# Boese0601/Dyadic-Interaction-Modeling

Hardware: AMD Instinct MI355X
Metric: listener clips/sec (T=300, EMOCA-56) (higher is better)
Workload: dtype bf16; 1 GPU; C3: B=256/GPU synthetic dyad clips, T=300, SLMFT.forward(mode='val'): listener VQ encode + encoder + 299-step AR decode (top-k 52 sampling) + VQ decode; global_batch=256, seq_len=300, gather=tokens+coeffs, gather_bytes_per_rank=17452032

## Files before the change

dyadic-interaction-modeling_amd/csrc/common.hpp:

```cpp
#pragma once
#include <hip/hip_runtime.h>
#include <stdint.h>
#include <stdio.h>
#include <string.h>
#include <string>

#include "../../include/dimx.h"

namespace dimx {

void set_error(const char* fmt, ...);
const char* get_error();

#define DIMX_HIP(expr)                                                                       \
    do {                                                                                     \
        hipError_t _e = (expr);                                                              \
        if (_e != hipSuccess) {                                                              \
            dimx::set_error("%s:%d: %s -> %s", __FILE__, __LINE__, #expr, hipGetErrorString(_e)); \
            return DIMX_ERR_HIP;                                                             \
        }                                                                                    \
    } while (0)

#define DIMX_REQUIRE(cond, code, ...)       \
    do {                                    \
// ... 352 lines not shown
    int force_nsplit;
};
int launch_decode_attn_self_kv8(const Kv8SelfArgs& a, hipStream_t s);

int launch_vq_argmin(const float* z, int N, const float* Et , const float* ee ,
                     int32_t* idx, float* best_d, float* margin, hipStream_t s);

struct ChainGemmDesc {
    const void* W;
    int N, K, ldw;
    int cols, rows_pad, ncb, nkt;
};
struct ChainArgs {
    int B;
    ChainGemmDesc g1;
    const void* A1;
    int lda1;
    float* xr;
    float* x;
    int C;
    const float* slabs;
    int nslab;
    long slab_stride;
    void* y;
    const float* gamma;
    ChainGemmDesc g2;
    float* out2;
    int ld_out2;
    unsigned* counters;
    unsigned* seen;
    const int32_t* step;
    unsigned* err;
    int defer;
    float* stats;
    const float* colsum2;
    int nbar;
    int fault;
    int offA1, offW1, offRed1, offA2, offW2, offRed2;
};
struct SampleHeadArgs {
    int on;
    const float* logits;
    int ld_logits, nslab;
    long slab_stride;
    int top_k;
    const float* noise;
    int row0, rows_total;
    int32_t* tokens;
    int tok_ld;
    float* logits_out;
    int logits_out_ld;
    const float* emb_table;
    const float* qkv0;
    int qkv0_N;
    int32_t* hist;
    int hist_ld;
    int32_t* params;
};
struct LayerChainArgs {
    int B, C;
    DecodeAttnArgs sa, ca;
    ChainGemmDesc g_so, g_cq, g_co;
    const void* o;
    int ld_o;
    float* x;
    void* y;
    float* stats;
    const float* colsum_cq;
    float* qc;
    int ld_qc;
    unsigned* counters;
    unsigned* seen;
    const int32_t* step;
    int epoch_add;
    unsigned* err;
    int fault;
    unsigned long long* prof;
    SampleHeadArgs head;
    int sc_stride;
    int off_base, off_A1, off_W1, off_A2, off_W2, off_W3, off_A3;
};
bool layer_chain_supported(const LayerChainArgs& a, int cu_count);
int launch_layer_chain(const LayerChainArgs& a, hipStream_t s);
size_t chain_plan(ChainArgs& a);
bool chain_supported(const ChainArgs& a, int cu_count);
int launch_chain(const ChainArgs& a, hipStream_t s);

int launch_cast_pad(int out_dtype, const float* x, int ldx, const float* coladd, void* y, int ldy, int M, int K,
                    hipStream_t s, const uint8_t* zero_rows = nullptr);
int launch_gather_rows(int out_dtype, const float* table, int ld_table, int rows, const int32_t* idx, void* y,
                       int ldy, int M, int C, hipStream_t s);
constexpr int kLstmSave = 6;
size_t lstm_scratch_bytes(int B, int T, int In);
int lstm_layer_run(const float* x, int B, int T, int In, int H, const float* const* w_ih, const float* const* w_hh,
                   const float* const* b_ih, const float* const* b_hh, float* y, void* scratch, size_t scratch_bytes, int flags,
                   int cu_count, int* fault_count, hipStream_t st, float* save = nullptr);
size_t lstm_bwd_scratch_bytes(int B, int T);
int lstm_bwd_run(const float* dy, const float* save, const float* const* w_hh, int B, int T, float* dgates, void* scratch,
                 size_t scratch_bytes, int flags, int cu_count, int* fault_count, hipStream_t st);
int launch_context_concat(int out_dtype, const float* x_s, const float* patch, const float* audio, void* ctx,
                          int M, int dim, int dim_a, hipStream_t s);
int launch_finalize_idx(int32_t* idx, const int32_t* lens, int B, int T, int32_t pad_value, hipStream_t s,
                        int fqn = 1);
int launch_shift_tokens(const int32_t* z, int32_t* inp, int32_t* tgt, int B, int T, hipStream_t s);
int launch_ce_argmax(const float* logits, const int32_t* target, float* row_loss, int32_t* argmax_tok, int R,
                     int V, hipStream_t s);
struct SampleFilter {
    int kind = 0;
    float a = 0.f, b = 0.f;
    uint8_t* keep_out = nullptr;
};
struct SampleArgs {
    const float* logits = nullptr;
    int ld_logits = 0, R = 0, top_k = 0;
    float temperature = 0.f;
    const float* noise = nullptr;
    uint64_t seed = 0;
    const int32_t* step_dev = nullptr;
    uint64_t step_host = 0;
    int32_t* tokens = nullptr;
    int tok_ld = 0, tok_col_from_step = 0, nslab = 0;
    long slab_stride = 0;
    float* logits_out = nullptr;
    int logits_out_ld = 0, row0 = 0, rows_total = 0;
    const float* emb_table = nullptr;
    int emb_C = 0;
    float* x_next = nullptr;
    int32_t* step_rw = nullptr;
    unsigned* done_ctr = nullptr;
    const float* pos_table = nullptr;
    float pos_scale = 0.f;
    int pos_rows = 0;
    const int32_t* dev_params = nullptr;
    void* y_next = nullptr;
    const float* y_gamma = nullptr;
    int y_dtype = DIMX_F32;
    const float* qkv0_table = nullptr;
    float* qkv0_out = nullptr;
    int qkv0_N = 0;
    const int32_t* prompt = nullptr;
    int prompt_ld = 0, prompt_max = 0;
    const int32_t* prompt_len = nullptr;
    int prompt_div = 1;
    int32_t* epoch_rw = nullptr;
    SampleFilter filt;
    int32_t* hist = nullptr;
    int hist_ld = 0;
};
int launch_sample(const SampleArgs& a, hipStream_t s);
struct GuidedArgs {
    const float* logits_u = nullptr;
    float scale = 1.f;
    float* branch_out = nullptr;
    int32_t* tokens_u = nullptr;
};
int launch_sample_guided(const SampleArgs& a, const GuidedArgs& g, hipStream_t s);
struct BeamSelectArgs {
    const float* logits = nullptr;
    int nslab = 1;
    long slab_stride = 0;
    int nclip = 0, W = 0;
    const int32_t* step_dev = nullptr;
    int step_host = 0;
    int32_t* step_rw = nullptr;
    unsigned* done_ctr = nullptr;
    int32_t* epoch_rw = nullptr;
// ... 62 lines not shown
```

dyadic-interaction-modeling_amd/csrc/gemm.hip:

```cpp
#include "common.hpp"

namespace dimx {

static bool gemm_use_ws72(const GemmArgs& a);

void gemm_args_init(GemmArgs& a) {
    memset(&a, 0, sizeof(a));
    a.in_dtype = DIMX_F32;
    a.out_dtype = DIMX_F32;
    a.rowadd_scale = 1.f;
    a.nseg = 1;
    a.rowT = 1;
    a.splitk = 1;
    a.rowadd_div = 1;
}

void gemm_set_plain_out(GemmArgs& a, void* C, int ldc) {
    a.nseg = 1;
    a.seg_width = a.N;
    a.seg[0].ptr = C;
    a.seg[0].sb = (long)ldc * a.rowT;
    a.seg[0].st = ldc;
    a.seg[0].sh = 0;
    a.seg[0].sd = 1;
// ... 790 lines not shown
            if (it + STAGES - 1 < nk) issue(it + STAGES - 1, (it + STAGES - 1) % STAGES);
            if (a.ln_stats && it == nk - 2) {
                float s1 = 0.f;
#pragma unroll
                for (int i = 0; i < 8; ++i) s1 += lp[i].x;
                s1 += xor_lane_f32<16>(s1);
                s1 += xor_lane_f32<32>(s1);
                const float inv_c = 1.0f / (float)a.ln_C;
                const float mean = s1 * inv_c;
                const float ncs = (float)a.ln_C * (1.0f / 32.0f), inv_n = 32.0f * inv_c;
                float s2 = 0.f;
#pragma unroll
                for (int i = 0; i < 8; ++i) {
                    const float d = lp[i].x * inv_n - mean;
                    s2 += lp[i].y + ncs * d * d;
                }
                s2 += xor_lane_f32<16>(s2);
                s2 += xor_lane_f32<32>(s2);
                const float var = s2 * inv_c;
                const float rstd = rsqrtf(var + 1e-5f);
                if (a.ln_err && lane < 16 && m0 + lw * 16 + lane < a.M && mean * mean > 64.0f * var)
                    atomicOr(a.ln_err, 4u);
                if (lane < 16) {
                    ln_sm[lw * 16 + lane] = mean;
                    ln_sm[64 + lw * 16 + lane] = rstd;
                }
                asm volatile("s_waitcnt lgkmcnt(0)" ::: "memory");
            }
        }
        return;
    }

    const int wm = wave >> 1, wn = wave & 1;
    const int half = lane >> 5, l31 = lane & 31;
    const unsigned lds0 = (unsigned)(size_t)(lds_void_t*)smem;
    unsigned aoff[4], woff[4];
#pragma unroll
    for (int ks = 0; ks < 4; ++ks) {
        aoff[ks] = lds0 + lds_off(wm * 32 + l31, 2 * ks + half);
        woff[ks] = lds0 + BM * 128 + lds_off(wn * 32 + l31, 2 * ks + half);
    }
    f32x16_t acc[1][1];
#pragma unroll
    for (int r = 0; r < 16; ++r) acc[0][0][r] = 0.f;
    float ln_cs = 0.f;
    for (int it = 0; it < nk; ++it) {
        const unsigned boff = (unsigned)((it % STAGES) * TILE_BYTES);
        __builtin_amdgcn_s_barrier();
        if (it == 0 && a.ln_stats) {
            const int n = n0 + wn * 32 + l31;
            ln_cs = a.ln_colsum[n < a.N ? n : a.N - 1];
        }
        u32x4_t fa[4][1], fw[4][1];
#pragma unroll
        for (int q = 0; q < 4; ++q) {
            ds_read128<0>(fa[q][0], aoff[q] + boff);
            ds_read128<0>(fw[q][0], woff[q] + boff);
        }
#pragma unroll
        for (int q = 0; q < 4; ++q) {
            if (q == 0) wait_lgkm<6>();
            if (q == 1) wait_lgkm<4>();
            if (q == 2) wait_lgkm<2>();
            if (q == 3) wait_lgkm<0>();
            __builtin_amdgcn_sched_barrier(0);
            FragMma<T, 1, 1>::run(acc, fa[q], fw[q]);
        }
    }
    if (a.ln_stats) {
        const float* strip = ln_sm + wm * 32;
#pragma unroll
        for (int q = 0; q < 4; ++q) {
            const float4 mq = *(const float4*)(strip + 8 * q + 4 * half);
            const float4 rq = *(const float4*)(strip + 64 + 8 * q + 4 * half);
            acc[0][0][4 * q + 0] = rq.x * (acc[0][0][4 * q + 0] - mq.x * ln_cs);
            acc[0][0][4 * q + 1] = rq.y * (acc[0][0][4 * q + 1] - mq.y * ln_cs);
            acc[0][0][4 * q + 2] = rq.z * (acc[0][0][4 * q + 2] - mq.z * ln_cs);
            acc[0][0][4 * q + 3] = rq.w * (acc[0][0][4 * q + 3] - mq.w * ln_cs);
        }
    }
    epilogue<T, OutT, 1, 1>(a, acc, m0 + wm * 32, n0 + wn * 32, half, l31, split);
}

template <typename OutT>
struct Ws72 {
    static constexpr int BM = 64, BN = 72, BK = 64, STAGES = 4, NLOAD = 4, NCONS = 6;
    static constexpr int TILE_BYTES = (BM + BN) * 128;
    static constexpr int RING_BYTES = STAGES * TILE_BYTES + 24 * 128;
    static constexpr int SMEM_BYTES = RING_BYTES > 84 * 1024 ? RING_BYTES : 84 * 1024;
    static_assert(STAGES - 2 == 2, "the loaders' counted waits below are written for two k-tiles in flight behind the current slot");

    template <int LW>
    static __device__ __forceinline__ void loader(const GemmArgs& a, int lw, int lane, int m0, int n0, int kt0, int nk, unsigned char* smem,
                                                  float* ln_sm) {
        constexpr int LA = 2, LPT = LA + LW;
        static_assert((STAGES - 1) * LPT < 56, "ring depth");
        const bf16* __restrict__ A = (const bf16*)a.A;
        const bf16* __restrict__ W = (const bf16*)a.W;
        const bf16* gA[LA];
        const bf16* gW[LW];
        int pA[LA], pW[LW];
#pragma unroll
        for (int j = 0; j < LA; ++j) {
            pA[j] = lw * LA + j;
            const int row = pA[j] * 8 + (lane >> 3);
            const int c = (lane & 7) ^ ((row >> 1) & 7);
            int m = m0 + row;
            m = m < a.M ? m : a.M - 1;
            gA[j] = A + (size_t)m * a.lda + c * 8 + (size_t)kt0 * BK;
        }
#pragma unroll
        for (int j = 0; j < LW; ++j) {
            pW[j] = (lw == 0 ? 0 : 1 + 2 * lw) + j;
            const int row = pW[j] * 8 + (lane >> 3);
            const int c = (lane & 7) ^ ((row >> 1) & 7);
            int n = n0 + row;
            n = n < a.N ? n : a.N - 1;
            gW[j] = W + (size_t)n * a.ldw + c * 8 + (size_t)kt0 * BK;
        }
        auto issue = [&](int kt, int slot) {
            unsigned char* base = smem + slot * TILE_BYTES;
#pragma unroll
            for (int j = 0; j < LA; ++j)
                __builtin_amdgcn_global_load_lds((glb_void_t*)(gA[j] + (size_t)kt * BK), (lds_void_t*)(base + pA[j] * 1024), 16, 0, 0);
#pragma unroll
            for (int j = 0; j < LW; ++j)
                __builtin_amdgcn_global_load_lds((glb_void_t*)(gW[j] + (size_t)kt * BK), (lds_void_t*)(base + BM * 128 + pW[j] * 1024), 16, 0, 0);
        };
        float2 lp[8];
        if (a.ln_stats) {
            int m = m0 + lw * 16 + (lane & 15);
            m = m < a.M ? m : a.M - 1;
            const float2* sp = (const float2*)a.ln_stats + ((size_t)(m >> 5) * 32 + (lane >> 4) * 8) * 32 + (m & 31);
#pragma unroll
            for (int i = 0; i < 8; ++i) lp[i] = sp[(size_t)i * 32];
        }
        int issued = 0;
        for (; issued < STAGES - 1 && issued < nk; ++issued) issue(issued, issued);
        int slot_next = issued % STAGES;
        const int st_ln = nk >= 2 ? nk - 2 : 0;
        for (int st = 0; st < nk; ++st) {
            {
                int done = st + 1, all = issued;
                done = done < nk ? done : nk;
                all = all < nk ? all : nk;
                const int y = all - done;
                if (y <= 0) wait_vmcnt<0>();
                else if (y == 1) wait_vmcnt<LPT>();
                else wait_vmcnt<2 * LPT>();
            }
            __builtin_amdgcn_s_barrier();
            if (issued < nk) {
                issue(issued, slot_next);
                ++issued;
                slot_next = slot_next + 1 == STAGES ? 0 : slot_next + 1;
            }
            if (a.ln_stats && st == st_ln) {
                float s1 = 0.f;
#pragma unroll
                for (int i = 0; i < 8; ++i) s1 += lp[i].x;
                s1 += xor_lane_f32<16>(s1);
                s1 += xor_lane_f32<32>(s1);
                const float inv_c = 1.0f / (float)a.ln_C;
                const float mean = s1 * inv_c;
                const float ncs = (float)a.ln_C * (1.0f / 32.0f), inv_n = 32.0f * inv_c;
                float s2 = 0.f;
#pragma unroll
                for (int i = 0; i < 8; ++i) {
                    const float d = lp[i].x * inv_n - mean;
                    s2 += lp[i].y + ncs * d * d;
                }
                s2 += xor_lane_f32<16>(s2);
                s2 += xor_lane_f32<32>(s2);
                const float var = s2 * inv_c;
                const float rstd = rsqrtf(var + 1e-5f);
                if (a.ln_err && lane < 16 && m0 + lw * 16 + lane < a.M && mean * mean > 64.0f * var) atomicOr(a.ln_err, 4u);
                if (lane < 16) {
                    ln_sm[lw * 16 + lane] = mean;
                    ln_sm[64 + lw * 16 + lane] = rstd;
                }
                asm volatile("s_waitcnt lgkmcnt(0)" ::: "memory");
            }
        }
    }

    static __device__ __forceinline__ void body(const GemmArgs& a, int block_id, int nblocks, unsigned char* smem, float* ln_sm) {
        const int tid = threadIdx.x, lane = tid & 63;
        const int wave = __builtin_amdgcn_readfirstlane(tid >> 6);
        const int tiles_n = (a.N + BN - 1) / BN, tiles_m = (a.M + BM - 1) / BM;
        const int ntiles = tiles_m * tiles_n;
        int bid = block_id;
        {
            const int q = nblocks >> 3, r = nblocks & 7, x = bid & 7, i = bid >> 3;
            bid = (x < r ? x * (q + 1) : r * (q + 1) + (x - r) * q) + i;
        }
        const int split = bid / ntiles, tile = bid - split * ntiles;
        const int tile_n = tile / tiles_m, tile_m = tile - tile_n * tiles_m;
        const int m0 = tile_m * BM, n0 = tile_n * BN;
        const int nk_all = (a.kloop ? a.kloop : a.ldw) / BK;
        const int per = (nk_all + a.splitk - 1) / a.splitk;
        const int kt0 = split * per;
        int nk = nk_all - kt0;
        nk = nk > per ? per : nk;
        if (nk <= 0) return;
        if (wave >= NCONS) {
            const int lw = wave - NCONS;
            if (lw == 0)
                loader<3>(a, lw, lane, m0, n0, kt0, nk, smem, ln_sm);
            else
                loader<2>(a, lw, lane, m0, n0, kt0, nk, smem, ln_sm);
            return;
        }
        const int wm = wave / 3, wn = wave - 3 * wm;
        const int half = lane >> 5, l31 = lane & 31;
        const unsigned lds0 = (unsigned)(size_t)(lds_void_t*)smem;
        unsigned aoff[4], woff[4];
#pragma unroll
        for (int ks = 0; ks < 4; ++ks) {
            aoff[ks] = lds0 + lds_off(wm * 32 + l31, 2 * ks + half);
            woff[ks] = lds0 + BM * 128 + lds_off(wn * 32 + l31, 2 * ks + half);
        }
        f32x16_t acc[1][1];
#pragma unroll
        for (int r = 0; r < 16; ++r) acc[0][0][r] = 0.f;
        const int n_lim = n0 + BN < a.N ? n0 + BN : a.N;
        const int ncol = n0 + wn * 32 + l31;
        const bool col_ok = ncol < n_lim;
        const int ncl = col_ok ? ncol : n_lim - 1;
        const float bias_v = (a.bias && split == 0) ? a.bias[ncl] : 0.f;
        const float ln_cs = a.ln_stats ? a.ln_colsum[ncl] : 0.f;
        const int ldc = (int)a.seg[0].st;
        const int row_base = m0 + wm * 32 + 4 * half;
        OutT* cptr = (OutT*)a.seg[0].ptr + (a.out_slabs ? (size_t)split * a.slab_stride : 0) + (size_t)row_base * ldc + ncl;
        const float* rptr = a.residual ? a.residual + (size_t)row_base * a.ldr + ncl : nullptr;
        const int ldr = a.ldr;
        const int mrem = a.M - row_base;
        const int act = a.act;
        const bool has_ln = a.ln_stats != nullptr;
        unsigned boff = 0;
        for (int st = 0; st < nk; ++st) {
            __builtin_amdgcn_s_barrier();
            u32x4_t fa[4][1], fw[4][1];
#pragma unroll
            for (int q = 0; q < 4; ++q) {
                ds_read128<0>(fa[q][0], aoff[q] + boff);
                ds_read128<0>(fw[q][0], woff[q] + boff);
            }
#pragma unroll
            for (int q = 0; q < 4; ++q) {
                if (q == 0) wait_lgkm<6>();
                if (q == 1) wait_lgkm<4>();
                if (q == 2) wait_lgkm<2>();
                if (q == 3) wait_lgkm<0>();
                __builtin_amdgcn_sched_barrier(0);
                FragMma<bf16, 1, 1>::run(acc, fa[q], fw[q]);
            }
            boff = boff + TILE_BYTES == STAGES * TILE_BYTES ? 0u : boff + TILE_BYTES;
        }
        if (has_ln) {
            const float* strip = ln_sm + wm * 32;
#pragma unroll
            for (int q = 0; q < 4; ++q) {
                const float4 mq = *(const float4*)(strip + 8 * q + 4 * half);
                const float4 rq = *(const float4*)(strip + 64 + 8 * q + 4 * half);
                acc[0][0][4 * q + 0] = rq.x * (acc[0][0][4 * q + 0] - mq.x * ln_cs);
                acc[0][0][4 * q + 1] = rq.y * (acc[0][0][4 * q + 1] - mq.y * ln_cs);
                acc[0][0][4 * q + 2] = rq.z * (acc[0][0][4 * q + 2] - mq.z * ln_cs);
                acc[0][0][4 * q + 3] = rq.w * (acc[0][0][4 * q + 3] - mq.w * ln_cs);
            }
        }
        float v[16];
        switch (act) {
            case ACT_GELU_ERF:
#pragma unroll
                for (int r = 0; r < 16; ++r) v[r] = act_fn<ACT_GELU_ERF, true>(acc[0][0][r] + bias_v);
                break;
            case ACT_GELU_TANH:
#pragma unroll
                for (int r = 0; r < 16; ++r) v[r] = act_fn<ACT_GELU_TANH, true>(acc[0][0][r] + bias_v);
                break;
            case ACT_LEAKY:
#pragma unroll
                for (int r = 0; r < 16; ++r) v[r] = act_fn<ACT_LEAKY, true>(acc[0][0][r] + bias_v);
                break;
            default:
#pragma unroll
                for (int r = 0; r < 16; ++r) v[r] = acc[0][0][r] + bias_v;
                break;
        }
        if (col_ok) {
            if (rptr) {
                float rv[16];
#pragma unroll
                for (int r = 0; r < 16; ++r) {
                    int off = (r & 3) + 8 * (r >> 2);
                    off = off < mrem ? off : mrem - 1;
                    rv[r] = rptr[(size_t)off * ldr];
                }
#pragma unroll
                for (int r = 0; r < 16; ++r) v[r] += rv[r];
            }
            if (mrem > 27) {
#pragma unroll
                for (int r = 0; r < 16; ++r) store_from_f32<OutT>(cptr + (size_t)((r & 3) + 8 * (r >> 2)) * ldc, v[r]);
            } else {
#pragma unroll
                for (int r = 0; r < 16; ++r) {
                    const int off = (r & 3) + 8 * (r >> 2);
                    if (off < mrem) store_from_f32<OutT>(cptr + (size_t)off * ldc, v[r]);
                }
            }
        }
    }
};

template <typename OutT>
__global__ __launch_bounds__(640) void gemm_ws72_kernel(const GemmArgs a) {
    __shared__ __attribute__((aligned(16))) unsigned char smem[Ws72<OutT>::SMEM_BYTES];
    __shared__ __attribute__((aligned(16))) float ln_sm[128];
    Ws72<OutT>::body(a, blockIdx.x, gridDim.x, smem, ln_sm);
}

template <typename OutT> static int launch_ws72(const GemmArgs& a, hipStream_t s) {
    const int tiles = ceil_div(a.M, 64) * ceil_div(a.N, 72);
    hipLaunchKernelGGL((gemm_ws72_kernel<OutT>), dim3(tiles * a.splitk), dim3(640), 0, s, a);
    DIMX_HIP(hipGetLastError());
    return DIMX_OK;
}

template <typename T, typename OutT, int STAGES> static int launch_ws(const GemmArgs& a, hipStream_t s) {
    const int tiles = ceil_div(a.M, 64) * ceil_div(a.N, 64);
    hipLaunchKernelGGL((gemm_ws_kernel<T, OutT, STAGES>), dim3(tiles * a.splitk), dim3(512), 0, s, a);
    DIMX_HIP(hipGetLastError());
    return DIMX_OK;
}

template <int BM, int BN, int WM> constexpr bool glds_stages() { return BM * BN >= 128 * 128 && BM / (WM * 32) == 1; }
static inline bool cfg_stages(int cfg) { return cfg == 14; }
static_assert(glds_stages<128, 128, 4>() && !glds_stages<128, 128, 2>() && !glds_stages<64, 64, 2>(), "cfg_stages() names the staged tiles");

template <typename T, typename OutT, int BM, int BN, int WM, int WN, int STAGES>
static int launch_glds(const GemmArgs& a, hipStream_t s) {
    const int tiles = ceil_div(a.M, BM) * ceil_div(a.N, BN);
    dim3 grid(tiles * a.splitk), block(WM * WN * 64);
    if constexpr (glds_stages<BM, BN, WM>()) {
        if (a.stage_out) {
            hipLaunchKernelGGL((gemm_glds_kernel<T, OutT, BM, BN, WM, WN, STAGES, true>), grid, block, 0, s, a);
            DIMX_HIP(hipGetLastError());
            return DIMX_OK;
        }
    }
    hipLaunchKernelGGL((gemm_glds_kernel<T, OutT, BM, BN, WM, WN, STAGES>), grid, block, 0, s, a);
    DIMX_HIP(hipGetLastError());
    return DIMX_OK;
}

template <typename T, typename OutT, int BM, int BN, int WM, int WN>
static int launch_cfg(const GemmArgs& a, hipStream_t s) {
    const int tiles = ceil_div(a.M, BM) * ceil_div(a.N, BN);
    dim3 grid(tiles), block(WM * WN * 64);
    if (a.conv_T > 0)
        hipLaunchKernelGGL((gemm_kernel<T, OutT, BM, BN, WM, WN, true>), grid, block, 0, s, a);
    else
        hipLaunchKernelGGL((gemm_kernel<T, OutT, BM, BN, WM, WN, false>), grid, block, 0, s, a);
    DIMX_HIP(hipGetLastError());
    return DIMX_OK;
}

template <typename T, typename OutT> static int launch_by_cfg(const GemmArgs& a, int cfg, hipStream_t s) {
    DIMX_REQUIRE(!a.w_tiled || cfg == 34 || cfg == 35, DIMX_ERR_ARG, "gemm: block-tiled W is read by the decode kernel only (cfg %d)", cfg);
    DIMX_REQUIRE(!a.ln_stats || ((cfg == 34 || cfg == 35 || cfg == 72) && a.splitk == 1 && a.ln_colsum && a.ln_C > 0 &&
                                 a.K >= 16 * Elem<T>::kPerChunk),
                 DIMX_ERR_ARG, "gemm: the deferred-LayerNorm epilogue exists in the decode kernel only, without split-K, from two "
                               "k-tiles up (cfg %d, K %d)", cfg, a.K);
    switch (cfg) {
        case 1: return launch_glds<T, OutT, 128, 128, 2, 2, 2>(a, s);
        case 3: return launch_glds<T, OutT, 64, 64, 2, 2, 4>(a, s);
        case 4: return launch_glds<T, OutT, 64, 64, 2, 2, 3>(a, s);
        case 14: return launch_glds<T, OutT, 128, 128, 4, 2, 2>(a, s);
        case 72:
            if constexpr (sizeof(T) == 2) return launch_ws72<OutT>(a, s);
            break;
        case 34: return launch_ws<T, OutT, 4>(a, s);
        case 35: return launch_ws<T, OutT, 6>(a, s);
        default: break;
    }
    set_error("gemm: unknown cfg %d", cfg);
    return DIMX_ERR_ARG;
}

static inline void cfg_tile(int cfg, int& bm, int& bn) {
    switch (cfg) {
        case 1: case 14: bm = 128; bn = 128; break;
        case 72: bm = 64; bn = 72; break;
        default: bm = 64; bn = 64; break;
    }
}

struct TypedPlan {
    int simple, cfg;
};

static int plan_typed(const GemmArgs& a0, GemmArgs& a, int in_es, int out_es, TypedPlan& p) {
// ... 106 lines not shown
        return splitk_nonempty(nk, best);
    }
    if (tiles >= 256) return 1;
    if (cfg == 72) {
        constexpr int min_nk72 = 6;
        int sp = 256 / tiles;
        const int max_sp = nk / min_nk72 > 0 ? nk / min_nk72 : 1;
        sp = sp > max_sp ? max_sp : sp;
        sp = sp > 8 ? 8 : sp;
        return splitk_nonempty(nk, sp);
    }
    constexpr int target = 288;
    constexpr int min_nk = 6;
    int sp = (target + tiles / 2) / tiles;
    const int max_sp = nk / min_nk > 0 ? nk / min_nk : 1;
    sp = sp > max_sp ? max_sp : sp;
    sp = sp > 8 ? 8 : sp;
    return splitk_nonempty(nk, sp);
}

static bool gemm_use_ws72(const GemmArgs& a) {
    if (a.in_dtype != DIMX_BF16) return false;
    const int kext = a.kloop ? a.kloop : a.ldw;
    if (a.conv_T != 0 || a.K % 64 != 0 || a.K != kext || a.force_simple || a.w_tiled) return false;
    if (a.M > 256 || a.N % 72 != 0) return false;
    if (a.nseg != 1 || a.seg[0].sd != 1 || a.seg[0].sh != 0 || a.seg[0].sb != a.seg[0].st * (long)a.rowT || a.rowadd_mode != 0) return false;
    return ceil_div(a.M, 64) * (a.N / 72) <= 256;
}

static int gemm_dispatch(const GemmArgs& a, hipStream_t s, int* route) {
    const int epc = a.in_dtype == DIMX_BF16 ? 8 : 4;
    const int bk = 8 * epc;
    const size_t es = dtype_size(a.in_dtype);
    DIMX_REQUIRE(a.A && a.W && a.M > 0 && a.N > 0 && a.K > 0, DIMX_ERR_ARG, "gemm: null operand or empty shape");
    DIMX_REQUIRE(a.ldw % epc == 0 && a.ldw >= a.K && (a.kloop ? a.kloop : a.ldw) % bk == 0 &&
                     (a.kloop == 0 || (a.kloop >= a.K && a.kloop <= a.ldw)),
                 DIMX_ERR_ARG, "gemm: W must be K-padded to %d (ldw=%d kloop=%d K=%d)", bk, a.ldw, a.kloop, a.K);
    DIMX_REQUIRE((a.lda * es) % 16 == 0 && ((uintptr_t)a.A % 16) == 0 && ((uintptr_t)a.W % 16) == 0, DIMX_ERR_ARG,
                 "gemm: A/W rows must be 16-byte aligned (lda=%d)", a.lda);
    DIMX_REQUIRE(a.K % epc == 0, DIMX_ERR_ARG, "gemm: K=%d must be a multiple of %d", a.K, epc);
    DIMX_REQUIRE(a.rowT >= 1 && a.nseg >= 1 && a.nseg <= 3 && a.seg_width > 0, DIMX_ERR_ARG, "gemm: bad output map");
    if (a.conv_T > 0) {
        DIMX_REQUIRE(a.conv_C % bk == 0 && a.K == 5 * a.conv_C && a.M % a.conv_T == 0, DIMX_ERR_ARG,
                     "gemm(conv5): C=%d must be a multiple of %d, K=5C, M %% T == 0", a.conv_C, bk);
    }
    for (int i = 0; i < a.nseg; ++i)
        DIMX_REQUIRE(a.seg[i].ptr && a.seg[i].D > 0, DIMX_ERR_ARG, "gemm: output segment %d unset", i);
    if (a.out_slabs)
        DIMX_REQUIRE(a.out_dtype == DIMX_F32 && a.act == ACT_NONE && !a.residual && a.rowadd_mode == 0 && a.nseg == 1 &&
                         a.conv_T == 0 && a.K == (a.kloop ? a.kloop : a.ldw),
                     DIMX_ERR_ARG, "gemm: slab output needs a plain f32 GEMM without activation/residual");
    if (a.w_tiled)
        DIMX_REQUIRE(a.N % 8 == 0 && a.conv_T == 0 && !a.force_simple && a.K % bk == 0 && a.M < 4096 && a.kloop == 0, DIMX_ERR_ARG,
                     "gemm: block-tiled W needs N %% 8 == 0, K %% %d == 0 and a decode-sized M (N=%d K=%d M=%d)", bk, a.N, a.K, a.M);
    {
        static const bool log = getenv("DIMX_GEMM_LOG") != nullptr;
        if (log && !route)
            fprintf(stderr, "dimx-gemm M=%d N=%d K=%d in=%d out=%d bias=%d res=%d act=%d rowadd=%d nseg=%d slabs=%d big=%d\n", a.M, a.N, a.K,
                    a.in_dtype, a.out_dtype, a.bias ? 1 : 0, a.residual ? 1 : 0, a.act, a.rowadd_mode, a.nseg, a.out_slabs ? 1 : 0,
                    (a.in_dtype == DIMX_BF16 && a.cfg == 0 && gemm256_eligible(a)) ? 1 : 0);
    }
    if (a.in_dtype == DIMX_BF16) {
        if (a.cfg == 0 && gemm256_eligible(a)) {
            if (route) {
                *route = ROUTE_GEMM256;
                return DIMX_OK;
            }
            return launch_gemm256(a, s);
        }
        if (a.out_dtype == DIMX_BF16) return launch_typed<bf16, bf16>(a, s, route);
        return launch_typed<bf16, float>(a, s, route);
    }
    DIMX_REQUIRE(a.out_dtype == DIMX_F32, DIMX_ERR_ARG, "gemm: f32 inputs produce f32 outputs");
    if (gemm_use_x3(a)) {
        if (route) {
            *route = ROUTE_X3;
            return DIMX_OK;
        }
        return launch_gemm_x3(a, s);
    }
    return launch_typed<float, float>(a, s, route);
}

int launch_gemm(const GemmArgs& a, hipStream_t s) { return gemm_dispatch(a, s, nullptr); }

int gemm_route(const GemmArgs& a, int* route) {
    *route = 0;
    return gemm_dispatch(a, nullptr, route);
}

}
```

dyadic-interaction-modeling_amd/csrc/generate.hip:

```cpp
#include <stdlib.h>

#include "stages.hpp"

namespace dimx {

static void chain_desc(ChainGemmDesc& d, const Linear& L) { d.W = L.w; d.N = L.N; d.K = L.K; d.ldw = L.Kp; }

static bool gen_use_chain(dimx_handle h, int B, int S) {
    if (!h->use_chain || h->at != DIMX_BF16 || S != 1 || h->gen_groups > 1 || !h->chain_err_dev) return false;
    const DecGeom& dg = h->decg;
    ChainArgs c;
    memset(&c, 0, sizeof(c));
    c.B = B;
    c.C = dg.dim;
    const XAttn& sa = h->dec.self_[0];
    const XAttn& ca = h->dec.cross[0];
    chain_desc(c.g1, sa.out);
    c.lda1 = dg.heads * dg.dim_head;
    chain_desc(c.g2, ca.qkv);
    if (!chain_supported(c, h->cu_count)) return false;
    chain_desc(c.g2, h->dec.logits);
    c.g1.W = nullptr;
    return chain_supported(c, h->cu_count) && 3 * dg.depth + 1 <= kChainSites;
}

static bool gen_multi_tr(dimx_handle h, int S) {
    return S > 1 && h->multi_tr && h->at == DIMX_BF16 && h->decg.dim_head == 64;
}

static int slab_gemm_rows(dimx_handle h, int B, hipStream_t st, const void* A, int lda, const Linear& L, float* out, long stride,
                          int* nsl) {
    GemmArgs g;
    gemm_lin(h, A, lda, L, B, g);
    g.x3_decode = 1;
    g.out_dtype = DIMX_F32;
    g.out_slabs = 1;
    static const bool f32_split = getenv("DIMX_F32_NO_SPLIT") == nullptr;
    if (f32_split) g.allow_splitk = 1;
    g.slab_stride = stride;
    gemm_set_plain_out(g, out, L.N);
    *nsl = gemm_plan_splits(g);
    g.force_splitk = *nsl;
    return launch_gemm(g, st);
}

static bool qkv0_table_supported(dimx_handle h) {
    const DecGeom& dg = h->decg;
    const int N = 3 * dg.heads * dg.dim_head;
    return h->use_qkv0_table && !dg.abs_pos && h->dec.self_[0].qkv.N == N && N % 4 == 0 && N <= 12 * 256 && dg.dim % 4 == 0 &&
           dg.dim / 2 <= 16 * 64;
}

static int qkv0_table_alloc(dimx_handle h) {
    const int V = h->decg.num_tokens, N = h->dec.self_[0].qkv.N;
    if (!h->qkv0_table) {
        DIMX_HIP(hipMalloc((void**)&h->qkv0_table, (size_t)V * N * sizeof(float)));
        h->qkv0_epoch = 0;
        h->graph_valid = false;
    }
    if (h->use_kv0_table && h->at == DIMX_BF16 && !h->kv0_image) {
        DIMX_HIP(hipMalloc(&h->kv0_image, (size_t)V * 2 * (N / 3) * sizeof(bf16)));
        h->qkv0_epoch = 0;
        h->graph_valid = false;
    }
    return DIMX_OK;
}

static int qkv0_table_build(dimx_handle h, const GenScratch& s, int M, hipStream_t st, int step0 = 0) {
    const DecGeom& dg = h->decg;
    const int DD = dg.dim, V = dg.num_tokens, N = h->dec.self_[0].qkv.N;
    if (h->qkv0_M == M && h->qkv0_at == h->at && h->qkv0_epoch == h->dec_epoch) return DIMX_OK;
    h->qkv0_epoch = 0;
    const int rounds = (V + M - 1) / M;
    int32_t* ids = (int32_t*)s.logits;
    DIMX_TRY(launch_iota_clamp(ids, rounds * M, V, st));
    for (int r = 0; r < rounds; ++r) {
        int ns = 0;
        DIMX_TRY(launch_embed_step(h->dec.tok_emb, DD, V, ids + (size_t)r * M, nullptr, 0, s.step, s.x, M, 1, st, nullptr, 0.f, 1, step0));
        DIMX_TRY(launch_add_slabs_layernorm(h->at, s.x, s.xr, 0, s.st_xr, s.y, h->dec.self_[0].ln_g, M, DD, st));
        DIMX_TRY(slab_gemm_rows(h, M, st, s.y, DD, h->dec.self_[0].qkv, s.qkv, s.st_qkv, &ns));
        DIMX_TRY(launch_sum_slabs_rows(s.qkv, ns, s.st_qkv, h->qkv0_table, r * M, V, M, N, st));
    }
    if (h->kv0_image) DIMX_TRY(launch_kv0_image(h->qkv0_table, N, V, N / 3, 2 * (N / 3), h->kv0_image, st));
    h->qkv0_M = M;
    h->qkv0_at = h->at;
    h->qkv0_epoch = h->dec_epoch;
    ++h->qkv0_builds;
    return DIMX_OK;
}

struct Kv8Layer {
    uint8_t *kcodes, *vcodes;
    float *kscale, *vscale;
};
static size_t kv8_codes_bytes(dimx_handle h, int B, int T) { return align_up((size_t)B * h->decg.heads * tpad(T) * 64, 256); }
static size_t kv8_scale_bytes(dimx_handle h, int B, int T) { return align_up((size_t)B * h->decg.heads * tpad(T) * sizeof(float), 256); }
static size_t kv8_bytes(dimx_handle h, int B, int T) {
    if (!h || h->variant != 0 || h->decg.dim_head != 64 || B < 1 || T < 2 || T > h->d.max_seq_len || tpad(T) > 2048) return 0;
    return (size_t)h->decg.depth * 2 * (kv8_codes_bytes(h, B, T) + kv8_scale_bytes(h, B, T));
}
static Kv8Layer kv8_layer_of(dimx_handle h, void* buf, int B, int T, int l) {
    const size_t cb = kv8_codes_bytes(h, B, T), sb = kv8_scale_bytes(h, B, T);
    uint8_t* p = (uint8_t*)buf + (size_t)l * 2 * (cb + sb);
    return Kv8Layer{p, p + cb, (float*)(p + 2 * cb), (float*)(p + 2 * cb + sb)};
}
static Kv8Layer kv8_layer(dimx_handle h, int B, int T, int l) { return kv8_layer_of(h, h->kv8_buf, B, T, l); }
static Kv8Layer self_kv8_layer(dimx_handle h, int R, int T, int l) { return kv8_layer_of(h, h->self_kv8_buf, R, T, l); }

struct GenRequest {
    GenPrompt pr;
    const uint8_t* ctx_mask;
    int B, T, S;
    float temperature;
    int top_k;
    const float* noise;
    uint64_t seed;
    int32_t* tokens;
    float* logits_out;
    void* ws;
    size_t ws_bytes;
    hipStream_t st;
    const BeamCall* beam;
    bool guided = false;
    float scale = 1.f;
    float* branch_out = nullptr;
// ... 246 lines not shown
    ta.kwords_ready = 1;
    return launch_attention_tr(ta, c.st);
}

static void head_args(const StepCtx& c, SampleHeadArgs& hd) {
    const GenScratch& s = c.s;
    const GenRequest& q = c.gc->req;
    memset(&hd, 0, sizeof(hd));
    hd.on = 1;
    hd.logits = s.logits; hd.ld_logits = c.V; hd.nslab = 1; hd.slab_stride = s.st_lg;
    hd.top_k = c.gc->top_k; hd.noise = q.noise; hd.row0 = c.row0; hd.rows_total = c.gc->R;
    hd.tokens = c.tokens; hd.tok_ld = c.n; hd.logits_out = c.logits_out; hd.logits_out_ld = c.n;
    hd.emb_table = c.h->dec.tok_emb; hd.qkv0 = c.r->qkv0; hd.qkv0_N = 3 * c.inner;
    hd.hist = s.hist; hd.hist_ld = c.T;
    hd.params = s.step;
}

static int attention_half(const StepCtx& c, int l, int* pending) {
    dimx_handle h = c.h;
    const GenScratch& s = c.s;
    const StepRoute& r = *c.r;
    const int B = c.B, DD = c.DD, inner = c.inner;
    int ns = 0;
    if (l > 0) DIMX_TRY(launch_add_slabs_layernorm(h->at, s.x, s.xr, *pending, s.st_xr, s.y, h->dec.self_[l].ln_g, B, DD, c.st));
    if (l == 0 && r.qkv0)
        ns = 1;
    else
        DIMX_TRY(slab_gemm(c, s.y, DD, h->dec.self_[l].qkv, s.qkv, s.st_qkv, &ns));
    const DecodeAttnArgs sa = self_args(c, l, ns);
    DecodeAttnArgs ca = cross_args(c, l);
    if (r.layer_kernel[l]) {
        LayerChainArgs lc;
        memset(&lc, 0, sizeof(lc));
        DIMX_REQUIRE(layer_args(c, l, sa, ca, lc), DIMX_ERR_STATE, "generate: layer %d lost its layer-kernel weights after the route was resolved", l);
        if (l == 0 && r.sample_head) head_args(c, lc.head);
        DIMX_TRY(launch_layer_chain(lc, c.st));
    } else if (r.chain) {
        DIMX_TRY(self_attention(c, l, sa));
        if (r.defer)
            DIMX_TRY(chain_site(c, 3 * l, s.o, inner, &h->dec.self_[l].out, 0, h->dec.cross[l].ln_g, &h->dec.cross[l].q_ln, s.qc, inner,
                                h->dec.cross[l].q_ln_colsum));
        else
            DIMX_TRY(chain_site(c, 3 * l, s.o, inner, &h->dec.self_[l].out, 0, h->dec.cross[l].ln_g, &h->dec.cross[l].qkv, s.qc, inner));
        ca.nslab = 1;
        DIMX_TRY(cross_attention(c, l, ca));
        DIMX_TRY(chain_site(c, 3 * l + 1, s.o, inner, &h->dec.cross[l].out, 0, h->dec.ff[l].ln_g, nullptr, nullptr, 0));
    } else if (r.guided) {
        const int Bc = c.Bc;
        const size_t es = c.es;
        DIMX_TRY(launch_decode_attn(sa, c.st));
        DIMX_TRY(slab_gemm(c, s.o, inner, h->dec.self_[l].out, s.xr, s.st_xr, pending));
        DIMX_TRY(launch_add_slabs_layernorm(h->at, s.x, s.xr, *pending, s.st_xr, s.y, h->dec.cross[l].ln_g, B, DD, c.st));
        DIMX_TRY(slab_gemm_rows(h, Bc, c.st, s.y, DD, h->dec.cross[l].qkv, s.qc, s.st_qc, &ns));
        ca.nslab = ns;
        DIMX_TRY(cross_attention(c, l, ca));
        DIMX_TRY(slab_gemm_rows(h, Bc, c.st, s.o, inner, h->dec.cross[l].out, s.xr, s.st_xr, pending));
        DIMX_TRY(launch_add_slabs_layernorm(h->at, s.x, s.xr, *pending, s.st_xr, s.y, h->dec.ff[l].ln_g, Bc, DD, c.st));
        DIMX_TRY(launch_add_slabs_layernorm(h->at, s.x + (size_t)Bc * DD, s.xr + (size_t)Bc * DD, 0, s.st_xr, (unsigned char*)s.y + (size_t)Bc * DD * es,
                                            h->dec.ff[l].ln_g, B - Bc, DD, c.st));
    } else {
        DIMX_TRY(self_attention(c, l, sa));
        DIMX_TRY(slab_gemm(c, s.o, inner, h->dec.self_[l].out, s.xr, s.st_xr, pending));
        DIMX_TRY(launch_add_slabs_layernorm(h->at, s.x, s.xr, *pending, s.st_xr, s.y, h->dec.cross[l].ln_g, B, DD, c.st));
        if (r.multi_tr && !r.win && r.kv8_samples) {
            GemmArgs g;
            gemm_lin(h, s.y, DD, h->dec.cross[l].qkv, B, g);
            g.out_dtype = h->at;
            gemm_set_plain_out(g, s.qcb, inner);
            DIMX_TRY(launch_gemm(g, c.st));
            DIMX_TRY(cross_attention(c, l, ca, s.qcb));
        } else if (r.multi_tr && !r.win) {
            DIMX_TRY(cross_attention_multi(c, l, ca));
        } else {
            DIMX_TRY(slab_gemm(c, s.y, DD, h->dec.cross[l].qkv, s.qc, s.st_qc, &ns));
            ca.nslab = ns;
            DIMX_TRY(cross_attention(c, l, ca));
        }
        DIMX_TRY(slab_gemm(c, s.o, inner, h->dec.cross[l].out, s.xr, s.st_xr, pending));
        DIMX_TRY(launch_add_slabs_layernorm(h->at, s.x, s.xr, *pending, s.st_xr, s.y, h->dec.ff[l].ln_g, B, DD, c.st));
    }
    return DIMX_OK;
}

static int feed_forward(const StepCtx& c, int l, int* pending) {
    dimx_handle h = c.h;
    const GenScratch& s = c.s;
    const bool defer = c.r->defer;
    const int F = c.DD * h->decg.ff_mult;
    GemmArgs g;
    gemm_lin(h, s.y, c.DD, defer ? h->dec.ff[l].f1_ln : h->dec.ff[l].f1, c.B, g);
    g.x3_decode = 1;
    if (defer) {
        g.ln_stats = h->chain_stats_dev;
        g.ln_err = h->chain_err_dev;
        g.ln_colsum = h->dec.ff[l].f1_ln_colsum;
        g.ln_C = c.DD;
    }
    g.out_dtype = h->at;
    g.act = ACT_GELU_ERF;
    gemm_set_plain_out(g, s.f, F);
    DIMX_TRY(launch_gemm(g, c.st));
    return slab_gemm(c, s.f, F, h->dec.ff[l].f2, s.xr, s.st_xr, pending);
}

static int logits(const StepCtx& c, int pending, int* nlg) {
    dimx_handle h = c.h;
    const GenScratch& s = c.s;
    if (c.r->logits_chain) {
        *nlg = 1;
        return chain_site(c, 3 * h->decg.depth, nullptr, 0, nullptr, pending, h->dec.final_g, &h->dec.logits, s.logits, c.V);
    }
    DIMX_TRY(launch_add_slabs_layernorm(h->at, s.x, s.xr, pending, s.st_xr, s.y, h->dec.final_g, c.B, c.DD, c.st));
    return slab_gemm(c, s.y, c.DD, h->dec.logits, s.logits, s.st_lg, nlg);
}

static int finish_beam(const StepCtx& c, int nlg) {
    dimx_handle h = c.h;
    const GenScratch& s = c.s;
    const GenPrompt& pr = c.gc->req.pr;
    const BeamCall& bm = *c.r->beam;
    const int row0 = c.row0, n = c.n, depth = h->decg.depth;
    BeamSelectArgs bs;
    bs.logits = s.logits; bs.nslab = nlg; bs.slab_stride = s.st_lg; bs.nclip = c.nclip; bs.W = c.S;
    bs.step_dev = s.step; bs.step_rw = s.step; bs.done_ctr = (unsigned*)(s.step + 8); bs.epoch_rw = s.step + 9; bs.dev_params = s.step + 2;
    bs.prompt = c.forced; bs.prompt_ld = pr.ld; bs.prompt_max = pr.Pmax; bs.prompt_len = c.forced_len;
    bs.lens = bm.lens ? bm.lens + c.clip0 : nullptr; bs.len_off = c.T - n;
    bs.cum_in = bm.cum + row0; bs.cum_out = bm.cum + row0; bs.parent = bm.parent + row0;
    bs.tokens = c.tokens; bs.backptr = bm.backptr ? bm.backptr + (size_t)row0 * n : nullptr; bs.tok_ld = n; bs.logits_out = c.logits_out;
    bs.emb_table = h->dec.tok_emb; bs.emb_C = c.DD; bs.x_next = s.x;
    bs.qkv0_table = c.r->qkv0; bs.qkv0_out = s.qkv; bs.qkv0_N = 3 * c.inner;
    DIMX_TRY(launch_beam_select(bs, c.st));
    if (!c.r->qkv0) DIMX_TRY(launch_add_slabs_layernorm(h->at, s.x, s.xr, 0, s.st_xr, s.y, h->dec.self_[0].ln_g, c.B, c.DD, c.st));
    BeamReorderArgs br;
    for (int l = 0; l < depth; ++l) {
        br.buf[2 * l] = s.sk[l];
        br.buf[2 * l + 1] = s.sv[l];
    }
    br.nbuf = 2 * depth; br.es = (int)c.es; br.nclip = c.nclip; br.W = c.S; br.H = c.heads; br.T = c.T;
    br.parent = bs.parent; br.step_dev = s.step; br.step_back = 1;
    br.tokens = c.tokens; br.backptr = bs.backptr; br.tok_ld = n;
    return launch_beam_reorder(br, c.st);
}

static int finish_sample(const StepCtx& c, int nlg) {
    dimx_handle h = c.h;
    const GenScratch& s = c.s;
    const GenRequest& q = c.gc->req;
    const GenPrompt& pr = q.pr;
    const float* qkv0 = c.r->qkv0;
    SampleArgs sm;
    sm.logits = s.logits; sm.ld_logits = c.V; sm.R = c.B; sm.nslab = nlg; sm.slab_stride = s.st_lg; sm.row0 = c.row0; sm.rows_total = c.gc->R;
    sm.top_k = c.gc->top_k; sm.noise = q.noise; sm.filt.kind = h->filter_kind;
    sm.temperature = q.temperature; sm.seed = q.seed;
    sm.step_dev = s.step; sm.step_rw = s.step; sm.dev_params = s.step + 2; sm.done_ctr = (unsigned*)(s.step + 8); sm.epoch_rw = s.step + 9;
    sm.tokens = c.tokens; sm.tok_ld = c.n; sm.tok_col_from_step = 1; sm.logits_out = c.logits_out; sm.logits_out_ld = c.n;
    sm.emb_table = h->dec.tok_emb; sm.emb_C = c.DD; sm.x_next = s.x; sm.pos_table = c.pos; sm.pos_scale = c.pos_scale; sm.pos_rows = c.n;
    sm.y_next = qkv0 ? nullptr : s.y; sm.y_gamma = qkv0 ? nullptr : h->dec.self_[0].ln_g; sm.y_dtype = h->at;
    sm.qkv0_table = qkv0; sm.qkv0_out = s.qkv; sm.qkv0_N = 3 * c.inner;
    if (c.r->kv0) { sm.hist = s.hist; sm.hist_ld = c.T; }
    sm.prompt = c.forced; sm.prompt_ld = pr.ld; sm.prompt_max = pr.Pmax; sm.prompt_len = c.forced_len; sm.prompt_div = c.S;
    return launch_sample(sm, c.st);
}

static int finish_guided(const StepCtx& c, int nlg) {
    dimx_handle h = c.h;
    const GenScratch& s = c.s;
    const GenRequest& q = c.gc->req;
    const GenPrompt& pr = q.pr;
    const float* qkv0 = c.r->qkv0;
    SampleArgs sm;
    sm.logits = s.logits; sm.ld_logits = c.V; sm.R = c.Bc; sm.nslab = nlg; sm.slab_stride = s.st_lg; sm.row0 = 0; sm.rows_total = c.Bc;
    sm.top_k = c.gc->top_k; sm.noise = q.noise; sm.filt.kind = h->filter_kind;
    sm.temperature = q.temperature; sm.seed = q.seed;
    sm.step_dev = s.step; sm.step_rw = s.step; sm.dev_params = s.step + 2; sm.done_ctr = (unsigned*)(s.step + 8); sm.epoch_rw = s.step + 9;
    sm.tokens = c.tokens; sm.tok_ld = c.n; sm.tok_col_from_step = 1; sm.logits_out = c.logits_out; sm.logits_out_ld = c.n;
    sm.emb_table = h->dec.tok_emb; sm.emb_C = c.DD; sm.x_next = s.x; sm.pos_table = c.pos; sm.pos_scale = c.pos_scale; sm.pos_rows = c.n;
    sm.y_next = qkv0 ? nullptr : s.y; sm.y_gamma = qkv0 ? nullptr : h->dec.self_[0].ln_g; sm.y_dtype = h->at;
    sm.qkv0_table = qkv0; sm.qkv0_out = s.qkv; sm.qkv0_N = 3 * c.inner;
    if (c.r->kv0) { sm.hist = s.hist; sm.hist_ld = c.T; }
    sm.prompt = c.forced; sm.prompt_ld = pr.ld; sm.prompt_max = pr.Pmax; sm.prompt_len = c.forced_len; sm.prompt_div = 1;
    GuidedArgs g;
    g.logits_u = s.logits + (size_t)c.Bc * c.V; g.scale = q.scale; g.branch_out = q.branch_out;
    return launch_sample_guided(sm, g, c.st);
}

static int gen_step(const StepCtx& c) {
    int pending = 0;
    for (int l = 0; l < c.h->decg.depth; ++l) {
        DIMX_TRY(attention_half(c, l, &pending));
        DIMX_TRY(feed_forward(c, l, &pending));
    }
    int nlg = 0;
    DIMX_TRY(logits(c, pending, &nlg));
    if (c.r->sample_head) return DIMX_OK;
    return c.r->beam ? finish_beam(c, nlg) : c.r->guided ? finish_guided(c, nlg) : finish_sample(c, nlg);
}

static int resolve_route(dimx_handle h, const GenCall& gc, int G, int rows, StepRoute& r) {
    const GenRequest& q = gc.req;
    const DecGeom& dg = h->decg;
    r = StepRoute{};
    r.G = G;
    r.S = q.S;
    r.beam = q.beam;
    r.fault_inject = h->chain_fault_inject > 0;
    r.chain = gen_use_chain(h, rows, q.S);
    r.defer = r.chain && h->defer_ln && h->chain_stats_dev && h->dec.cross[0].q_ln.w && h->dec.ff[0].f1_ln.w;
    r.logits_chain = r.chain && !h->dec.logits.bias;
    r.multi_tr = gen_multi_tr(h, q.S);
    r.win = h->xwin_on != 0;
    r.lookahead = r.win ? h->xwin_lookahead : 0;
    r.kv8 = h->kv8_buf != nullptr;
    r.kv8_samples = r.kv8 && q.S > 1;
    r.self_kv8 = h->self_kv8_buf != nullptr;
    r.guided = q.guided;
    if (r.guided) r.chain = r.defer = r.logits_chain = r.multi_tr = false;
    if (G == 1 && qkv0_table_supported(h)) {
        DIMX_TRY(qkv0_table_alloc(h));
        r.qkv0 = h->qkv0_table;
    }
    if (r.qkv0 && h->use_kv0_table && !q.beam && q.pr.step0 == 0 && q.pr.Pmax <= 1 && dg.dim_head == 64 && dg.num_tokens <= 512)
        r.kv0 = h->at == DIMX_BF16 ? h->kv0_image : (const void*)h->qkv0_table;
    if (h->use_layer_chain && r.chain && r.defer && q.S == 1 && 4 * dg.depth + 1 <= kChainSites && !r.win && !r.kv8 && !r.self_kv8) {
        const StepCtx c = step_ctx(h, gc, r, 0, rows, 0, q.st);
        for (int l = 0; l < dg.depth; ++l) {
            LayerChainArgs lc;
            memset(&lc, 0, sizeof(lc));
            r.layer_kernel[l] = layer_args(c, l, self_args(c, l, 1), cross_args(c, l), lc) && layer_chain_supported(lc, h->cu_count);
        }
    }
    r.sample_head = h->use_sample_head && r.kv0 && r.layer_kernel[0] && r.logits_chain && h->filter_kind == DIMX_FILTER_TOP_K && !q.beam &&
                    !r.guided && q.pr.step0 == 0 && q.pr.Pmax <= 1 && G == 1 && q.S == 1 && dg.num_tokens == 512 && dg.dim % 4 == 0;
    return DIMX_OK;
}

static GraphKey graph_key(dimx_handle h, const GenCall& gc, const StepRoute& r) {
    const GenRequest& q = gc.req;
    GraphKey k{};
    k.ws = q.ws; k.B = q.B; k.T = q.T; k.top_k = gc.top_k;
    k.noise = q.noise; k.start = q.pr.tok; k.mask = q.ctx_mask; k.tokens = q.tokens; k.logits_out = q.logits_out;
    k.G = r.G; k.S = r.S;
    k.chain = r.chain; k.defer = r.defer; k.logits_chain = r.logits_chain; k.multi_tr = r.multi_tr; k.fault_inject = r.fault_inject;
    for (int l = 0; l < 8; ++l) k.layer_kernel |= r.layer_kernel[l] ? 1u << l : 0u;
    k.qkv0 = r.qkv0; k.kv0 = r.kv0; k.sample_head = r.sample_head;
    k.prompt_len = q.pr.len; k.ld_prompt = q.pr.ld; k.Pmax = q.pr.Pmax;
    k.filter_kind = h->filter_kind;
    k.beam = q.beam ? *q.beam : BeamCall{};
    k.xwin_on = r.win ? 1 : 0; k.xwin_lookahead = r.lookahead;
    k.guided = r.guided; k.branch_out = q.branch_out;
    k.kv8 = r.kv8 ? h->kv8_buf : nullptr;
    k.kv8_samples = r.kv8_samples;
    k.self_kv8 = r.self_kv8 ? h->self_kv8_buf : nullptr;
    return k;
}

static int gen_prefill(dimx_handle h, const CtxPersist& cp, const GenScratch& gs, const PrefillScratch& s, const GenPrompt& pr,
                       const uint8_t* ctx_mask, int B, int T, int S, int32_t* tokens, hipStream_t st, const int* win = nullptr,
                       int n_keys = 0) {
    const DecGeom& dg = h->decg;
    const int n0 = pr.step0, M = B * n0, DD = dg.dim, heads = dg.heads, D = dg.dim_head;
    const int np = tpad(n0), Tp = tpad(T), V = dg.num_tokens;
    DIMX_TRY(launch_prompt_rows(pr.tok, pr.ld, B, n0, V, S, s.inp, tokens, gen_steps(h, T), st));
    DIMX_TRY(launch_gather_rows(DIMX_F32, h->dec.tok_emb, DD, V, s.inp, s.h, DD, M, DD, st));
    const bool rowv = qkv_row_v(h->at, D);
    for (int l = 0; l < dg.depth; ++l) {
        AttnArgs a;
        DIMX_TRY(self_attn_qkv(h, s, h->dec.self_[l].ln_g, nullptr, h->dec.self_[l].qkv, B, n0, DD, heads, D, a, st));
        DIMX_TRY(launch_kv_rows_to_cache(h->at, s.k, gs.sk[l], B, n0, heads, T, S, st));
        if (rowv)
            DIMX_TRY(launch_kv_rows_to_cache(h->at, s.vt, gs.sv[l], B, n0, heads, T, S, st));
        else
            DIMX_TRY(launch_kv_vt_to_cache((const float*)s.vt, np, (float*)gs.sv[l], B, n0, heads, T, S, st));
        if (l == dg.depth - 1) break;
        a.scale = 1.0f / sqrtf((float)D); a.causal = 1;
        DIMX_TRY(attn_out(h, s, a, h->dec.self_[l].out, DD, st));
        if (win) {
            const XAttn& x = h->dec.cross[l];
            float* qf = win_q_rows(s, B, n0, heads * D, es_of(h));
            DIMX_REQUIRE(qf, DIMX_ERR_WORKSPACE, "generate: no room for the windowed prefill's f32 queries");
            DIMX_TRY(launch_layernorm(h->at, s.h, s.y, x.ln_g, nullptr, M, DD, st));
            DIMX_TRY(linear(h, s.y, DD, x.qkv, M, DIMX_F32, qf, heads * D, st));
            WinAttnArgs w;
            w.dtype = h->at;
            w.q = qf; w.ld = heads * D;
            w.kcache = cp.ck[l]; w.vcache = cp.cv[l]; w.Tp = Tp;
            w.out = s.o; w.o_ld = heads * D;
            w.B = B; w.H = heads; w.Lq = n0; w.t0 = 0; w.n_keys = n_keys; w.lookahead = *win;
            w.kmask = ctx_mask; w.kmask_ld = T;
            w.scale = 1.0f / sqrtf((float)D);
            DIMX_TRY(launch_win_attn(w, st));
            DIMX_TRY(residual_linear(h, s.o, heads * D, x.out, M, s.h, DD, st));
            DIMX_TRY(ff_sublayer(h, s, h->dec.ff[l].ln_g, nullptr, h->dec.ff[l].f1, h->dec.ff[l].f2, nullptr, ACT_GELU_ERF, M, DD, st));
            continue;
        }
        set_attn_packed(a, h->at, s.q, cp.ck[l], rowv ? cp.cv[l] : s.cvt, s.o, B, heads, n0, T, D, Tp, rowv);
        a.k_sb = (long)heads * Tp * D; a.k_sh = (long)Tp * D; a.k_st = D;
        if (rowv) { a.v_sb = a.k_sb; a.v_sh = a.k_sh; a.v_st = D; }
        DIMX_TRY(cross_attn_sublayer(h, s, h->dec.cross[l], a, ctx_mask, DD, st, rowv ? nullptr : (const float*)cp.cv[l]));
        DIMX_TRY(ff_sublayer(h, s, h->dec.ff[l].ln_g, nullptr, h->dec.ff[l].f1, h->dec.ff[l].f2, nullptr, ACT_GELU_ERF, M, DD, st));
    }
    return DIMX_OK;
}

static int chain_state_ensure(dimx_handle h) {
    if (!(h->use_chain && h->at == DIMX_BF16 && !h->chain_err_dev)) return DIMX_OK;
    DIMX_HIP(hipMalloc((void**)&h->chain_err_dev, 64));
    DIMX_HIP(hipMemset(h->chain_err_dev, 0, 64));
    DIMX_HIP(hipMalloc((void**)&h->chain_stats_dev, 8 * 32 * 32 * 2 * sizeof(float)));
    DIMX_HIP(hipMemset(h->chain_stats_dev, 0, 8 * 32 * 32 * 2 * sizeof(float)));
    DIMX_HIP(hipHostMalloc((void**)&h->chain_err_host, 64, hipHostMallocDefault));
    *h->chain_err_host = 0;
    DIMX_HIP(hipEventCreateWithFlags(&h->chain_err_ev, hipEventDisableTiming));
    return DIMX_OK;
}

static int gen_groups_fork(dimx_handle h, int G, hipStream_t st, hipStream_t* gs) {
    if (G == 1) {
        gs[0] = st;
        return DIMX_OK;
    }
    if (!h->ev_fork) DIMX_HIP(hipEventCreateWithFlags(&h->ev_fork, hipEventDisableTiming));
    DIMX_HIP(hipEventRecord(h->ev_fork, st));
    for (int g = 0; g < G; ++g) {
        if (!h->grp_stream[g]) DIMX_HIP(hipStreamCreateWithFlags(&h->grp_stream[g], hipStreamNonBlocking));
        if (!h->ev_join[g]) DIMX_HIP(hipEventCreateWithFlags(&h->ev_join[g], hipEventDisableTiming));
        gs[g] = h->grp_stream[g];
        DIMX_HIP(hipStreamWaitEvent(gs[g], h->ev_fork, 0));
// ... 78 lines not shown
        DIMX_HIP(hipMemset2DAsync(q.beam->backptr, (size_t)n * 4, 0xFF, (size_t)q.pr.step0 * 4, gc.R, st));
    return DIMX_OK;
}

struct GenRun {
    GenRequest q;
    CtxPersist cp;
    GenScratch s;
    GenCall gc;
    StepRoute route;
    StepCtx ctx[dimx_ctx::kMaxGroups];
    hipStream_t gs[dimx_ctx::kMaxGroups];
    int G = 1, n = 0, nrun = 0;
    bool graphs = true;
    explicit GenRun(const GenRequest& r) : q(r), cp{}, s{}, gc{q, cp, s, 0, 0} {}
    GenRun(const GenRun&) = delete;
};

int gen_open(dimx_handle h, GenRun& run, bool keep_prefill, bool prefill_only, const GenSessionSpec* sess) {
    const GenRequest& q = run.q;
    const GenPrompt& pr = q.pr;
    const int B = q.B, T = q.T, S = q.S;
    hipStream_t st = q.st;
    const int top_k = h && h->filter_kind != DIMX_FILTER_TOP_K ? 0 : q.top_k;
    DIMX_REQUIRE(S == 1 || S == 2 || S == 4 || S == 5 || S == 8 || S == 10, DIMX_ERR_ARG,
                 "generate: n_samples %d not in {1,2,4,5,8,10}", S);
    if (h && h->kv8_buf && !sess) {
        DIMX_REQUIRE((S == 1 || (h->kv8_samples_on && !q.guided)) && !q.beam, DIMX_ERR_ARG,
                     "generate: n_samples > 1 and beam search are not available with dimx_set_cross_kv8");
        DIMX_REQUIRE(kv8_bytes(h, B, T) != 0, DIMX_ERR_ARG, "generate: B=%d T=%d is not supported with dimx_set_cross_kv8", B, T);
        DIMX_REQUIRE(h->kv8_bytes >= kv8_bytes(h, B, T), DIMX_ERR_WORKSPACE, "generate: the FP8 cross K/V buffer holds %zu bytes, B=%d T=%d needs %zu (dimx_cross_kv8_bytes)",
                     h->kv8_bytes, B, T, kv8_bytes(h, B, T));
    }
    if (h && h->self_kv8_buf && !sess) {
        DIMX_REQUIRE(!q.beam && !q.guided, DIMX_ERR_ARG, "generate: beam search and guidance are not available with dimx_set_self_kv8");
        DIMX_REQUIRE(kv8_bytes(h, B * S, T) != 0, DIMX_ERR_ARG, "generate: B=%d n_samples=%d T=%d is not supported with dimx_set_self_kv8", B, S, T);
        DIMX_REQUIRE(h->self_kv8_bytes >= kv8_bytes(h, B * S, T), DIMX_ERR_WORKSPACE,
                     "generate: the FP8 self K/V buffer holds %zu bytes, B=%d n_samples=%d T=%d needs %zu (dimx_self_kv8_bytes)", h->self_kv8_bytes, B, S, T,
                     kv8_bytes(h, B * S, T));
    }
    const int halves = q.guided ? 2 : 1;
    DIMX_TRY(check_common(h, B, T, q.ws, q.ws_bytes, COMP_DEC, S * halves));
    DIMX_REQUIRE(pr.tok && q.ctx_mask && q.tokens && T >= 2, DIMX_ERR_ARG, "generate: null argument or T < 2");
    DIMX_REQUIRE(sess || (h->ctx_ready && h->ctx_B == B && h->ctx_T == T && h->ctx_ws == q.ws && h->ctx_for_generate),
                 DIMX_ERR_STATE, "generate: call dimx_encode_ctx(for_generate=1) with the same B, T, ws first");
    CtxPersist& cp = run.cp;
    Arena ar = scratch_arena(h, q.ws, q.ws_bytes, B, T, &cp);
    GenScratch& s = run.s;
    const int R = B * S * halves;
    plan_gen(h, ar, R, T, s);
    PrefillScratch ps;
    if (pr.step0 > 0) plan_prefill(h, ar, B, pr.step0, T, ps);
    DIMX_REQUIRE(!ar.overflow, DIMX_ERR_WORKSPACE, "generate: workspace overflow");
    const int n = gen_steps(h, T);
    run.n = n;
    run.nrun = n - pr.step0;
    DIMX_TRY(chain_state_ensure(h));
    int G = h->gen_groups < 1 ? 1 : h->gen_groups;
    if (G > B) G = B;
    if (S > 1 || q.beam || sess || q.guided) G = 1;
    run.G = G;
    int lo[dimx_ctx::kMaxGroups + 1];
    for (int g = 0; g <= G; ++g) lo[g] = (int)((long)R * g / G);
    run.gc.R = R;
    run.gc.top_k = top_k;
    const GenCall& gc = run.gc;
    StepRoute& route = run.route;
    DIMX_TRY(resolve_route(h, gc, G, lo[1] - lo[0], route));
    if (sess) {
        route.chain = route.defer = route.logits_chain = route.multi_tr = false;
        for (bool& lk : route.layer_kernel) lk = false;
        route.sample_head = false;
        route.win = true;
        route.lookahead = sess->lookahead;
        route.kv8 = false;
        route.kv8_samples = false;
        route.self_kv8 = false;
        run.graphs = false;
    }
    DIMX_TRY(gen_parameters(h, gc, route, n));
    if (route.qkv0) DIMX_TRY(qkv0_table_build(h, s, R, st, pr.step0));
    if (route.kv0) ++h->kv0_generations;
    if (route.sample_head) ++h->sample_head_generations;
    if (pr.step0 > 0 && !keep_prefill) {
        if (q.logits_out)
            DIMX_HIP(hipMemset2DAsync(q.logits_out, (size_t)n * h->decg.num_tokens * 4, 0, (size_t)pr.step0 * h->decg.num_tokens * 4, R, st));
        DIMX_REQUIRE(!pr.win || route.win, DIMX_ERR_STATE, "generate: a windowed prefill without the cross-attention window");
        DIMX_TRY(gen_prefill(h, cp, s, ps, pr, q.ctx_mask, B, T, S, q.tokens, st, pr.win ? &route.lookahead : nullptr, sess ? sess->n_keys : T));
    }
    if (route.self_kv8 && pr.step0 > 0 && !keep_prefill && !prefill_only) {
        for (int l = 0; l < h->decg.depth; ++l) {
            const Kv8Layer kl = self_kv8_layer(h, R, T, l);
            DIMX_TRY(launch_kv8_quant(h->at, s.sk[l], R, h->decg.heads, tpad(T), pr.step0, kl.kcodes, kl.kscale, st, T));
            DIMX_TRY(launch_kv8_quant(h->at, s.sv[l], R, h->decg.heads, tpad(T), pr.step0, kl.vcodes, kl.vscale, st, T));
        }
    }
    if (prefill_only) return DIMX_OK;
    if (route.kv8 && !keep_prefill) {
        const int Tp = tpad(T), heads = h->decg.heads;
        for (int l = 0; l < h->decg.depth; ++l) {
            const Kv8Layer kl = kv8_layer(h, B, T, l);
            DIMX_TRY(launch_kv8_quant(h->at, cp.ck[l], B, heads, Tp, T, kl.kcodes, kl.kscale, st));
            DIMX_TRY(launch_kv8_quant(h->at, cp.cv[l], B, heads, Tp, T, kl.vcodes, kl.vscale, st));
        }
    }
    DIMX_TRY(gen_groups_fork(h, G, st, run.gs));
    for (int g = 0; g < G; ++g) {
        run.ctx[g] = step_ctx(h, gc, route, lo[g], lo[g + 1] - lo[g], g, run.gs[g]);
        if (sess) run.ctx[g].n_keys = sess->n_keys;
        DIMX_TRY(gen_start(run.ctx[g]));
    }
    return DIMX_OK;
}

int gen_run_steps(dimx_handle h, GenRun& run, int nsteps) {
    const int G = run.G;
    if (!h->use_graph || !run.graphs) {
        for (int t = 0; t < nsteps; ++t)
            for (int g = 0; g < G; ++g) DIMX_TRY(gen_step(run.ctx[g]));
    } else {
        DIMX_TRY(step_graphs_ensure(h, graph_key(h, run.gc, run.route), run.ctx, G, run.n));
        DIMX_TRY(step_graphs_replay(h, nsteps, G, run.gs));
    }
    return DIMX_OK;
}

void gen_run_set_keys(GenRun& run, int n_keys, hipStream_t st) {
    run.ctx[0].n_keys = n_keys;
    run.ctx[0].st = run.gs[0] = st;
}

GenRun* gen_run_new(const int32_t* start, const uint8_t* ctx_mask, int B, int T, float temperature, int top_k, const float* noise,
                    uint64_t seed, int32_t* tokens, float* logits_out, void* ws, size_t ws_bytes, hipStream_t st, int ld_prompt, int P) {
    const GenRequest q{{start, ld_prompt, P, nullptr, P - 1, P > 1}, ctx_mask, B, T, 1, temperature, top_k, noise, seed, tokens, logits_out, ws, ws_bytes, st, nullptr};
    return new GenRun(q);
}
void gen_run_free(GenRun* r) { delete r; }

static int generate_impl(dimx_handle h, const GenRequest& q, bool keep_prefill, bool prefill_only, StepRoute* ran) {
    *ran = StepRoute{};
    GenRun run(q);
    DIMX_TRY(gen_open(h, run, keep_prefill, prefill_only, nullptr));
    if (prefill_only) return DIMX_OK;
    DIMX_TRY(gen_run_steps(h, run, run.nrun));
    if (run.route.sample_head && run.nrun > 0) DIMX_TRY(finish_sample(run.ctx[0], 1));
    DIMX_TRY(gen_groups_join(h, run.G, q.st, run.gs));
    if (run.route.chain && run.G == 1) {
        DIMX_HIP(hipMemcpyAsync(h->chain_err_host, h->chain_err_dev, 4, hipMemcpyDeviceToHost, q.st));
        DIMX_HIP(hipEventRecord(h->chain_err_ev, q.st));
    }
    *ran = run.route;
    return DIMX_OK;
}

int check_sampler_filter(int kind, float a, float b) {
    DIMX_REQUIRE(kind >= DIMX_FILTER_TOP_K && kind <= DIMX_FILTER_TOP_A, DIMX_ERR_ARG, "sampler filter: unknown kind %d", kind);
    if (kind == DIMX_FILTER_TOP_K) return DIMX_OK;
    DIMX_REQUIRE(a == a && (kind != DIMX_FILTER_TOP_A || b == b), DIMX_ERR_ARG, "sampler filter: NaN parameter");
    if (kind == DIMX_FILTER_TOP_P) DIMX_REQUIRE(a >= 0.f, DIMX_ERR_ARG, "sampler filter: top_p thres %g < 0", (double)a);
    if (kind == DIMX_FILTER_MIN_P) DIMX_REQUIRE(a >= 0.f && a <= 1.f, DIMX_ERR_ARG, "sampler filter: min_p %g outside [0, 1]", (double)a);
    if (kind == DIMX_FILTER_TOP_A)
        DIMX_REQUIRE(a >= 0.f && b >= 0.f, DIMX_ERR_ARG, "sampler filter: top_a min_p_pow %g or min_p_ratio %g < 0", (double)a, (double)b);
    return DIMX_OK;
}

}

using namespace dimx;

extern "C" {

static int print_layer_prof(dimx_handle h) {
    DIMX_HIP(hipEventSynchronize(h->chain_err_ev));
    static const char* names[14] = {"start", "self attention done", "barrier 1", "rows + W1 landed", "out-proj stored", "barrier 2",
                                    "y rows + W2 landed", "cross-q stored", "barrier 3", "cross attention done", "barrier 4",
                                    "rows + W3 landed", "out-proj stored", "head done"};
    static const int order[14] = {0, 13, 1, 2, 3, 4, 5, 6, 7, 8, 9, 10, 11, 12};
    std::vector<unsigned long long> hp((size_t)8 * 256 * 16);
    DIMX_HIP(hipMemcpy(hp.data(), h->layer_prof_dev, hp.size() * 8, hipMemcpyDeviceToHost));
    for (int l = 0; l < h->decg.depth; ++l) {
        const unsigned long long* p = hp.data() + (size_t)l * 256 * 16;
        unsigned long long t0 = ~0ull;
        for (int b = 0; b < 256; ++b)
            if (p[b * 16] && p[b * 16] < t0) t0 = p[b * 16];
        if (t0 == ~0ull) continue;
        fprintf(stderr, "dimx layer-kernel stamps, layer %d (us after the first block's start; mean / max over blocks)\n", l);
        double prev = 0;
        for (int k = 0; k < 14; ++k) {
            const int i = order[k];
            double sum = 0, mx = 0;
            int n = 0;
            for (int b = 0; b < 256; ++b)
                if (p[b * 16 + i]) {
                    const double v = (double)(p[b * 16 + i] - t0) / 100.0;
                    sum += v;
                    mx = v > mx ? v : mx;
                    ++n;
                }
            if (!n) continue;
            fprintf(stderr, "  %-24s %7.2f / %7.2f  (+%.2f)\n", names[i], sum / n, mx, sum / n - prev);
            prev = sum / n;
        }
    }
    return DIMX_OK;
}

static int take_chain_flags(dimx_handle h, void* stream) {
    DIMX_HIP(hipEventSynchronize(h->chain_err_ev));
    const unsigned e = *h->chain_err_host;
    if (!e) return 0;
    *h->chain_err_host = 0;
    DIMX_HIP(hipMemsetAsync(h->chain_err_dev, 0, 64, (hipStream_t)stream));
    h->graph_valid = false;
    ++h->chain_faults;
    return (int)e;
}

static int generate_checked(dimx_handle h, const GenRequest& q) {
    StepRoute route;
    auto chain_ran = [&] { return route.chain && route.G == 1; };
    DIMX_TRY(generate_impl(h, q, false, false, &route));
    if (h->chain_fault_inject > 0) --h->chain_fault_inject;
    if (!chain_ran()) return DIMX_OK;
    if (h->layer_prof_dev) DIMX_TRY(print_layer_prof(h));
    const int e = take_chain_flags(h, q.st);
    if (e <= 0) return e;
    if (e & 3) {
        h->use_chain = 0;
        fprintf(stderr, "dimx: the XCD-local chain kernels reported %s%s; this batch is regenerated on the one-kernel-per-op "
                        "step and the chain path stays off for this handle (DIMX_NO_CHAIN=1 avoids it from the start)\n",
                (e & 1) ? "two blocks on one (XCD, CU slot) " : "", (e & 2) ? "a group-barrier timeout" : "");
    } else {
        h->defer_ln = 0;
        fprintf(stderr, "dimx: a residual row's mean exceeds 8 standard deviations; this batch is regenerated with the row-phase "
                        "LayerNorm and the deferred form stays off for this handle\n");
    }
    DIMX_TRY(generate_impl(h, q, true, false, &route));
    if (!chain_ran()) return DIMX_OK;
    const int e2 = take_chain_flags(h, q.st);
    if (e2 <= 0) return e2;
    h->use_chain = 0;
    fprintf(stderr, "dimx: the regenerated batch reported chain flags 0x%x again; regenerating on the one-kernel-per-op step, the "
                    "chain path stays off for this handle\n", e2);
    DIMX_TRY(generate_impl(h, q, true, false, &route));
    DIMX_REQUIRE(!chain_ran(), DIMX_ERR_STATE, "generate: the chain path is still active after it was switched off");
    return DIMX_OK;
}

int dimx_generate(dimx_handle h, const int32_t* start, const uint8_t* ctx_mask, int B, int T, int n_samples,
                  float temperature, int top_k, const float* exp_noise, uint64_t seed, int32_t* tokens, float* logits_out,
                  void* ws, size_t ws_bytes, void* stream) {
    const GenRequest q{{start, 1, 1, nullptr, 0}, ctx_mask, B, T, n_samples < 1 ? 1 : n_samples, temperature, top_k, exp_noise, seed,
                       tokens, logits_out, ws, ws_bytes, (hipStream_t)stream, nullptr};
    DIMX_NO_SESSION(h, "generate");
    return generate_checked(h, q);
}

int dimx_generate_prompted(dimx_handle h, const int32_t* prompt, int ld_prompt, const int32_t* prompt_len, int Pmax, int P0,
                           const uint8_t* ctx_mask, int B, int T, int n_samples, float temperature, int top_k,
                           const float* exp_noise, uint64_t seed, int32_t* tokens, float* logits_out, int flags, void* ws,
                           size_t ws_bytes, void* stream) {
    DIMX_REQUIRE(h, DIMX_ERR_ARG, "null handle");
    DIMX_NO_SESSION(h, "generate_prompted");
    DIMX_REQUIRE(h->variant == 0, DIMX_ERR_ARG, "generate_prompted: prompts are implemented for variant 0 (SLMFT) only; this handle is variant %d",
                 h->variant);
    DIMX_REQUIRE(prompt && T >= 2 && Pmax >= 1 && Pmax <= T - 1 && ld_prompt >= Pmax, DIMX_ERR_ARG,
                 "generate_prompted: need 1 <= Pmax <= T - 1 and ld_prompt >= Pmax (Pmax=%d T=%d ld_prompt=%d)", Pmax, T, ld_prompt);
    DIMX_REQUIRE(P0 >= 1 && P0 <= Pmax, DIMX_ERR_ARG, "generate_prompted: need 1 <= P0 <= Pmax (P0=%d Pmax=%d)", P0, Pmax);
    DIMX_REQUIRE((flags & ~7) == 0, DIMX_ERR_ARG, "generate_prompted: unknown flags 0x%x", flags);
    const int S = n_samples < 1 ? 1 : n_samples;
    const bool win_prefill = h->xwin_on && (flags & 2) && !(flags & 1);
    const int p0 = ((flags & 1) || (h->xwin_on && !win_prefill)) ? 1 : P0;
    DIMX_REQUIRE(!(flags & 4) || p0 >= 2, DIMX_ERR_ARG, "generate_prompted: flags bit 2 (the prefill stage alone) without a prefill (P0=%d, flags 0x%x)",
                 P0, flags);
    DIMX_REQUIRE(p0 == 1 || h->decg.dim_head == 64, DIMX_ERR_ARG, "generate_prompted: the prefill needs 64-wide heads");
    DIMX_REQUIRE(B >= 1 && T <= h->d.max_seq_len, DIMX_ERR_ARG, "B=%d T=%d out of range (T <= %d)", B, T, h->d.max_seq_len);
    const size_t need = workspace_bytes_prompt(h, B, T, S, p0);
    DIMX_REQUIRE(ws_bytes >= need, DIMX_ERR_WORKSPACE, "generate_prompted: workspace %zu < required %zu (dimx_workspace_bytes_prompt)",
                 ws_bytes, need);
    const GenRequest q{{prompt, ld_prompt, Pmax, prompt_len, p0 - 1, win_prefill && p0 >= 2}, ctx_mask, B, T, S, temperature, top_k, exp_noise, seed,
                       tokens, logits_out, ws, ws_bytes, (hipStream_t)stream, nullptr};
    if (flags & 4) {
        StepRoute route;
// ... 65 lines not shown
    h->filter_a = kind == DIMX_FILTER_TOP_K ? 0.f : a;
    h->filter_b = kind == DIMX_FILTER_TOP_A ? b : 0.f;
    return DIMX_OK;
}

int dimx_set_cross_lookahead(dimx_handle h, int on, int lookahead) {
    DIMX_REQUIRE(h, DIMX_ERR_ARG, "null handle");
    DIMX_NO_SESSION(h, "set_cross_lookahead");
    DIMX_REQUIRE(h->variant == 0, DIMX_ERR_ARG, "set_cross_lookahead: online generation is implemented for variant 0 (SLMFT) only; this handle is variant %d",
                 h->variant);
    h->xwin_on = on ? 1 : 0;
    h->xwin_lookahead = on ? lookahead : 0;
    return DIMX_OK;
}

int dimx_cross_lookahead(dimx_handle h, int* on, int* lookahead) {
    DIMX_REQUIRE(h, DIMX_ERR_ARG, "null handle");
    if (on) *on = h->xwin_on;
    if (lookahead) *lookahead = h->xwin_lookahead;
    return DIMX_OK;
}

size_t dimx_cross_kv8_bytes(dimx_handle h, int B, int T) { return kv8_bytes(h, B, T); }

int dimx_set_cross_kv8(dimx_handle h, void* buf, size_t bytes) {
    DIMX_REQUIRE(h, DIMX_ERR_ARG, "null handle");
    DIMX_NO_SESSION(h, "set_cross_kv8");
    DIMX_REQUIRE(h->variant == 0, DIMX_ERR_ARG, "set_cross_kv8: FP8 cross K/V is implemented for variant 0 (SLMFT) only; this handle is variant %d",
                 h->variant);
    DIMX_REQUIRE(buf == nullptr || (h->decg.dim_head == 64 && (uintptr_t)buf % 256 == 0), DIMX_ERR_ARG,
                 "set_cross_kv8: the buffer must be 256-byte aligned and the decoder's heads 64 wide");
    h->kv8_buf = buf;
    h->kv8_bytes = buf ? bytes : 0;
    return DIMX_OK;
}

int dimx_cross_kv8(dimx_handle h, void** buf, size_t* bytes) {
    DIMX_REQUIRE(h, DIMX_ERR_ARG, "null handle");
    if (buf) *buf = h->kv8_buf;
    if (bytes) *bytes = h->kv8_bytes;
    return DIMX_OK;
}

int dimx_set_cross_kv8_samples(dimx_handle h, int on) {
    DIMX_REQUIRE(h, DIMX_ERR_ARG, "set_cross_kv8_samples: null handle");
    DIMX_NO_SESSION(h, "set_cross_kv8_samples");
    DIMX_REQUIRE(h->variant == 0, DIMX_ERR_ARG, "set_cross_kv8_samples: FP8 cross K/V is implemented for variant 0 (SLMFT) only; this handle is variant %d",
                 h->variant);
    h->kv8_samples_on = on ? 1 : 0;
    return DIMX_OK;
}

int dimx_cross_kv8_samples(dimx_handle h, int* on) {
    DIMX_REQUIRE(h, DIMX_ERR_ARG, "cross_kv8_samples: null handle");
    if (on) *on = h->kv8_samples_on;
    return DIMX_OK;
}

size_t dimx_self_kv8_bytes(dimx_handle h, int R, int T) { return kv8_bytes(h, R, T); }

int dimx_set_self_kv8(dimx_handle h, void* buf, size_t bytes) {
    DIMX_REQUIRE(h, DIMX_ERR_ARG, "null handle");
    DIMX_NO_SESSION(h, "set_self_kv8");
    DIMX_REQUIRE(h->variant == 0, DIMX_ERR_ARG, "set_self_kv8: FP8 self K/V is implemented for variant 0 (SLMFT) only; this handle is variant %d",
                 h->variant);
    DIMX_REQUIRE(buf == nullptr || (h->decg.dim_head == 64 && (uintptr_t)buf % 256 == 0), DIMX_ERR_ARG,
                 "set_self_kv8: the buffer must be 256-byte aligned and the decoder's heads 64 wide");
    h->self_kv8_buf = buf;
    h->self_kv8_bytes = buf ? bytes : 0;
    return DIMX_OK;
}

int dimx_self_kv8(dimx_handle h, void** buf, size_t* bytes) {
    DIMX_REQUIRE(h, DIMX_ERR_ARG, "null handle");
    if (buf) *buf = h->self_kv8_buf;
    if (bytes) *bytes = h->self_kv8_bytes;
    return DIMX_OK;
}

int dimx_chain_faults(dimx_handle h) { return h ? h->chain_faults : 0; }
int dimx_qkv0_table_builds(dimx_handle h) { return h ? h->qkv0_builds : 0; }
int dimx_kv0_table_generations(dimx_handle h) { return h ? h->kv0_generations : 0; }
int dimx_sample_head_generations(dimx_handle h) { return h ? h->sample_head_generations : 0; }

int dimx_debug_chain_fault(dimx_handle h, int n_calls) {
    DIMX_REQUIRE(h && n_calls >= 0, DIMX_ERR_ARG, "debug_chain_fault: bad argument");
    h->chain_fault_inject = n_calls;
    h->graph_valid = false;
    return DIMX_OK;
}

}
```

dyadic-interaction-modeling_amd/csrc/model.hip:

```cpp
#include <stdarg.h>
#include <stdlib.h>
#include <set>

#include "stages.hpp"

namespace dimx {

static thread_local char g_err[1024] = "";
void set_error(const char* fmt, ...) {
    va_list ap;
    va_start(ap, fmt);
    vsnprintf(g_err, sizeof(g_err), fmt, ap);
    va_end(ap);
}
const char* get_error() { return g_err; }

static std::string vq_prefix(int which) { return which == 0 ? "speaker_vq." : "listener_vq."; }

struct KeySpec {
    std::string name;
    std::vector<int64_t> shape;
};

static void vq_keys(const dimx_dims& d, int which, std::vector<KeySpec>& out) {
// ... 763 lines not shown
}

using namespace dimx;

extern "C" {

int dimx_version(void) { return 100; }
const char* dimx_last_error(void) { return get_error(); }

void dimx_legacy_dims(dimx_dims* d) {
    if (!d) return;
    dimx_default_dims(d);
    d->variant = 1;
    d->dim_in = 1024; d->dim = 512; d->dim_a = 0; d->enc_depth = 6; d->dec_depth = 6; d->heads = 8;
    d->max_seq_len = 1024;
    d->spk_in_dim = 824; d->spk_hidden = 768; d->spk_heads = 8; d->spk_inter = 1536; d->spk_face_quan_num = 8;
}

void dimx_default_dims(dimx_dims* d) {
    if (!d) return;
    memset(d, 0, sizeof(*d));
    d->vq_in_dim = 56; d->vq_hidden = 384; d->vq_layers = 6; d->vq_heads = 8; d->vq_inter = 1536;
    d->vq_n_embed = 512; d->vq_zdim = 128;
    d->dim_in = 56; d->dim = 384; d->dim_a = 768; d->enc_depth = 4; d->dec_depth = 4; d->heads = 12;
    d->dim_head = 64; d->num_tokens = 512; d->max_seq_len = 2048; d->ff_mult = 4;
}

int dimx_create(dimx_handle* h, int device_id, const dimx_dims* dims, int numeric_mode) {
    DIMX_REQUIRE(h, DIMX_ERR_ARG, "dimx_create: null handle pointer");
    DIMX_REQUIRE(numeric_mode == DIMX_MODE_PARITY_F32 || numeric_mode == DIMX_MODE_PERF_BF16, DIMX_ERR_ARG,
                 "dimx_create: numeric_mode %d", numeric_mode);
    dimx_dims d;
    dimx_default_dims(&d);
    if (dims) d = *dims;
    DIMX_REQUIRE(d.vq_hidden == 384 && d.vq_heads == 8 && d.vq_zdim == 128 && d.vq_n_embed == 512 && d.vq_in_dim == 56,
                 DIMX_ERR_ARG, "dimx_create: only the DIM-Listener VQ geometry (56/384/8/128/512) is built");
    if (d.variant == 0 || d.variant == 2) {
        DIMX_REQUIRE(d.dim == 384 && d.dim_a == 768 && d.dim_head == 64 && d.heads == 12 && d.num_tokens == 512 &&
                         d.vq_layers <= 8 && d.enc_depth <= 8 && d.dec_depth <= 8 && d.max_seq_len <= 2048,
                     DIMX_ERR_ARG, "dimx_create: only the SLMFT geometry (384+768, 12x64, 512 tokens) is built");
    } else {
        DIMX_REQUIRE(d.variant == 1 && d.dim == 512 && d.dim_a == 0 && d.dim_head == 64 && d.heads == 8 &&
                         d.num_tokens == 512 && d.enc_depth <= 8 && d.dec_depth <= 8 && d.max_seq_len <= 2048 &&
                         d.spk_hidden == 768 && d.spk_heads == 8 && d.spk_in_dim == 824 && d.spk_face_quan_num == 8,
                     DIMX_ERR_ARG, "dimx_create: only the legacy ListenerGenerator geometry (824/768 VQ, 512, 8x64) is built");
    }
    DIMX_REQUIRE(d.mesh_dim == 0 || (d.variant == 2 && d.mesh_dim > 0), DIMX_ERR_ARG,
                 "dimx_create: the mesh head (mesh_dim %d) belongs to a handle of variant 2", d.mesh_dim);
    int ndev = 0;
    DIMX_HIP(hipGetDeviceCount(&ndev));
    DIMX_REQUIRE(device_id >= 0 && device_id < ndev, DIMX_ERR_ARG, "dimx_create: device %d of %d", device_id, ndev);
    DIMX_HIP(hipSetDevice(device_id));
    dimx_ctx* c = new dimx_ctx();
    c->device = device_id;
    c->d = d;
    c->mode = numeric_mode;
    c->at = numeric_mode == DIMX_MODE_PERF_BF16 ? DIMX_BF16 : DIMX_F32;
    c->variant = d.variant;
    const VQGeom lvq = {d.vq_in_dim, 64, d.vq_hidden, d.vq_heads, d.vq_inter, d.vq_layers, d.vq_zdim, 1, d.vq_zdim,
                        d.vq_n_embed, true};
    c->vqg[0] = c->vqg[1] = lvq;
    if (d.variant == 1) {
        c->vqg[0] = {d.spk_in_dim, (d.spk_in_dim + 63) / 64 * 64, d.spk_hidden, d.spk_heads, d.spk_inter, d.vq_layers,
                     d.spk_face_quan_num * d.vq_zdim, d.spk_face_quan_num, d.vq_zdim, d.vq_n_embed, false};
        const int din = d.spk_face_quan_num * d.vq_zdim;
        c->encg[0] = c->encg[1] = {din, din, d.dim, d.heads, d.dim_head, d.enc_depth, d.ff_mult, 0};
        c->decg = {d.dim, d.heads, d.dim_head, d.dec_depth, d.ff_mult, 1, d.num_tokens, d.dim};
    } else {
        const int causal = d.variant == 2 ? 0 : 1, abs_pos = d.variant == 2 ? 1 : 0;
        c->encg[0] = {d.dim_in, 64, d.dim, d.heads, d.dim_head, d.enc_depth, d.ff_mult, causal};
        c->encg[1] = {d.dim, d.dim, d.dim, d.heads, d.dim_head, d.enc_depth, d.ff_mult, causal};
        c->decg = {d.dim + d.dim_a, d.heads, d.dim_head, d.dec_depth, d.ff_mult, abs_pos, d.num_tokens, d.dim + d.dim_a};
    }
    for (const auto& k : all_keys(d)) c->required.push_back(k.name);
    const char* ng = getenv("DIMX_NO_GRAPH");
    c->use_graph = (ng && ng[0] == '1') ? 0 : 1;
    const char* nc = getenv("DIMX_NO_CHAIN");
    c->use_chain = (nc && nc[0] == '1') ? 0 : 1;
    c->use_layer_chain = getenv("DIMX_NO_LAYER_CHAIN") ? 0 : 1;
    c->multi_tr = getenv("DIMX_NO_MULTI_TR") ? 0 : 1;
    c->use_qkv0_table = getenv("DIMX_NO_QKV0_TABLE") ? 0 : 1;
    c->use_kv0_table = getenv("DIMX_NO_KV0_TABLE") ? 0 : 1;
    c->use_sample_head = getenv("DIMX_NO_SAMPLE_HEAD") ? 0 : 1;
    if (getenv("DIMX_LAYER_PROF")) {
        void* p = nullptr;
        if (hipMalloc(&p, (size_t)8 * 256 * 16 * 8) == hipSuccess) {
            (void)hipMemset(p, 0, (size_t)8 * 256 * 16 * 8);
            c->layer_prof_dev = (unsigned long long*)p;
        }
    }
    if (const char* pg = getenv("DIMX_PREFILL_GROUPS")) {
        const int v = atoi(pg);
        if (v >= 1 && v <= dimx_ctx::kPreGroups) c->prefill_groups = v;
    }
    {
        int cus = 0;
        if (hipDeviceGetAttribute(&cus, hipDeviceAttributeMultiprocessorCount, device_id) == hipSuccess) c->cu_count = cus;
    }
    const char* gg = getenv("DIMX_GEN_GROUPS");
    if (gg && atoi(gg) >= 1 && atoi(gg) <= dimx_ctx::kMaxGroups) c->gen_groups = atoi(gg);
    *h = c;
    return DIMX_OK;
}

int dimx_destroy(dimx_handle h) {
    if (!h) return DIMX_OK;
    (void)hipSetDevice(h->device);
    for (int g = 0; g < dimx_ctx::kMaxGroups; ++g) {
        if (h->graph_multi[g]) (void)hipGraphExecDestroy(h->graph_multi[g]);
        if (h->graph_exec[g]) (void)hipGraphExecDestroy(h->graph_exec[g]);
        if (h->grp_stream[g]) (void)hipStreamDestroy(h->grp_stream[g]);
        if (h->ev_join[g]) (void)hipEventDestroy(h->ev_join[g]);
    }
    if (h->ev_fork) (void)hipEventDestroy(h->ev_fork);
    for (int g = 0; g < dimx_ctx::kPreGroups - 1; ++g) {
        if (h->pre_stream[g]) (void)hipStreamDestroy(h->pre_stream[g]);
        if (h->pre_join[g]) (void)hipEventDestroy(h->pre_join[g]);
    }
    if (h->pre_fork) (void)hipEventDestroy(h->pre_fork);
    if (h->cap_stream) (void)hipStreamDestroy(h->cap_stream);
    if (h->chain_err_ev) (void)hipEventDestroy(h->chain_err_ev);
    if (h->chain_err_dev) (void)hipFree(h->chain_err_dev);
    if (h->chain_stats_dev) (void)hipFree(h->chain_stats_dev);
    if (h->layer_prof_dev) (void)hipFree(h->layer_prof_dev);
    if (h->qkv0_table) (void)hipFree(h->qkv0_table);
    if (h->kv0_image) (void)hipFree(h->kv0_image);
    if (h->chain_err_host) (void)hipHostFree(h->chain_err_host);
    free_packed(h);
    stream_forget(h);
    train_forget(h);
    delete h;
    return DIMX_OK;
}

int dimx_numeric_mode(dimx_handle h) { return h ? h->mode : DIMX_ERR_ARG; }

int dimx_set_shard(dimx_handle h, int row_offset, int rows_total) {
    DIMX_REQUIRE(h, DIMX_ERR_ARG, "set_shard: null handle");
    DIMX_REQUIRE(row_offset >= 0 && (rows_total == 0 || rows_total > row_offset), DIMX_ERR_ARG,
                 "set_shard: row_offset %d, rows_total %d", row_offset, rows_total);
    h->shard_row_off = row_offset;
    h->shard_rows_total = rows_total;
    return DIMX_OK;
}

int dimx_begin_checkpoint(dimx_handle h) {
    DIMX_REQUIRE(h, DIMX_ERR_ARG, "dimx_begin_checkpoint: null handle");
    std::set<std::string> spec;
    for (const auto& k : all_keys(h->d)) spec.insert(k.name);
    bool dirty = false;
    for (auto it = h->host.begin(); it != h->host.end();) {
        if (!spec.count(it->first)) {
            it = h->host.erase(it);
            dirty = true;
        } else {
            ++it;
        }
    }
    if (dirty) {
        (void)hipSetDevice(h->device);
        (void)hipDeviceSynchronize();
        free_packed(h);
        h->graph_valid = false;
        h->ctx_ready = false;
    }
    return DIMX_OK;
// ... 856 lines not shown
```

dyadic-interaction-modeling_amd/csrc/model.hpp:

```cpp
#pragma once
#include <map>
#include <string>
#include <vector>

#include "common.hpp"

namespace dimx {

struct Linear {
    void* w = nullptr;
    const float* bias = nullptr;
    int N = 0, K = 0, Kp = 0;
    void* w3 = nullptr;
};

struct VQBlock {
    const float *ln1_g, *ln1_b, *ln2_g, *ln2_b;
    Linear qkv, out, l1, l2;
    const void* mlp = nullptr;
};

struct VQNet {
    Linear vm, conv, le, post;
    VQBlock enc[8];
// ... 16 lines not shown
};
struct XFF {
    const float* ln_g;
    Linear f1, f2;
    Linear f1_ln;
    const float* f1_ln_colsum = nullptr;
    const void* mlp = nullptr;
};
struct XEnc {
    Linear proj_in;
    const float* pos_emb = nullptr;
    XAttn attn[8];
    XFF ff[8];
    const float* final_g = nullptr;
};
struct XDec {
    const float* tok_emb = nullptr;
    const float* pos_emb = nullptr;
    XAttn self_[8], cross[8];
    XFF ff[8];
    const float* final_g = nullptr;
    Linear logits;
    Linear cross_kv_all;
};

struct MeshHead {
    const float *w_ih[2][2], *w_hh[2][2], *b_ih[2][2], *b_hh[2][2];
    Linear l1, l2;
};

struct VQGeom {
    int in_dim, in_pad, hidden, heads, inter, layers, out_dim, fqn, zdim, n_embed;
    bool has_decoder;
};
struct EncGeom {
    int dim_in, in_pad, dim, heads, dim_head, depth, ff_mult, causal;
};
struct DecGeom {
    int dim, heads, dim_head, depth, ff_mult, abs_pos, num_tokens, ctx_dim;
};

struct HostTensor {
    std::vector<float> data;
    std::vector<int64_t> shape;
};

struct Arena {
    unsigned char* base;
    size_t off;
    size_t cap;
    bool overflow;
    Arena(void* b, size_t c) : base((unsigned char*)b), off(0), cap(c), overflow(false) {}
    void* take(size_t bytes) {
        off = align_up(off, 256);
        void* p = base ? base + off : nullptr;
        off += bytes;
        if (base && off > cap) overflow = true;
        return p;
    }
};

struct BeamCall {
    double* cum = nullptr;
    int32_t* parent = nullptr;
    int32_t* backptr = nullptr;
    const int32_t* lens = nullptr;
    bool operator==(const BeamCall& o) const { return cum == o.cum && parent == o.parent && backptr == o.backptr && lens == o.lens; }
};

struct StepRoute {
    bool chain = false;
    bool defer = false;
    bool layer_kernel[8] = {};
    bool logits_chain = false;
    bool multi_tr = false;
    bool win = false;
    int lookahead = 0;
    bool kv8 = false;
    bool kv8_samples = false;
    bool self_kv8 = false;
    const float* qkv0 = nullptr;
    const void* kv0 = nullptr;
    bool sample_head = false;
    const BeamCall* beam = nullptr;
    bool fault_inject = false;
    int G = 1, S = 1;
    bool guided = false;
};

struct GraphKey {
    void* ws;
    int B, T, top_k;
    const void *noise, *start, *mask, *tokens, *logits_out;
    int G, S;
    bool chain, defer, logits_chain, multi_tr, fault_inject;
    unsigned layer_kernel;
    const void *qkv0, *kv0;
    bool sample_head;
    const void* prompt_len;
    int ld_prompt, Pmax;
    int filter_kind;
    BeamCall beam;
    int xwin_on, xwin_lookahead;
    bool guided;
    const void* branch_out;
    const void* kv8;
    bool kv8_samples;
    const void* self_kv8;
    bool operator==(const GraphKey& o) const {
        return ws == o.ws && B == o.B && T == o.T && top_k == o.top_k && noise == o.noise && start == o.start && mask == o.mask &&
               tokens == o.tokens && logits_out == o.logits_out && G == o.G && S == o.S && chain == o.chain && defer == o.defer &&
               logits_chain == o.logits_chain && multi_tr == o.multi_tr && fault_inject == o.fault_inject &&
               layer_kernel == o.layer_kernel && qkv0 == o.qkv0 && kv0 == o.kv0 && sample_head == o.sample_head && prompt_len == o.prompt_len &&
               ld_prompt == o.ld_prompt && Pmax == o.Pmax && filter_kind == o.filter_kind && beam == o.beam && xwin_on == o.xwin_on &&
               xwin_lookahead == o.xwin_lookahead && guided == o.guided && branch_out == o.branch_out && kv8 == o.kv8 && kv8_samples == o.kv8_samples && self_kv8 == o.self_kv8;
    }
};

}

namespace dimx {
int vq_pe_buffers(dimx_ctx* c, int which, const float** pe_enc, const float** pe_dec);
void train_forget(dimx_ctx* h);
void stream_forget(dimx_ctx* h);
}

struct dimx_ctx {
    int device = 0;
    dimx_dims d;
    int variant = 0;
    dimx::VQGeom vqg[2];
    dimx::EncGeom encg[2];
    dimx::DecGeom decg;
    int mode = 0;
    int at = DIMX_F32;
    std::map<std::string, dimx::HostTensor> host;
    std::vector<std::string> required;
    int packed_mask = 0;
    std::vector<void*> dev_allocs;
    dimx::VQNet vq[2];
    dimx::XEnc enc_s, enc_joint, enc_l;
    dimx::XDec dec;
    const float *patch_s = nullptr, *patch_dec_s = nullptr, *norm_s_g = nullptr, *norm_s_b = nullptr;
    const float *patch_l = nullptr, *patch_dec_l = nullptr, *norm_l_g = nullptr, *norm_l_b = nullptr;
    const float *norm_j_g = nullptr, *norm_j_b = nullptr;
    bool ctx_ready = false;
    int ctx_B = 0, ctx_T = 0, ctx_for_generate = 0;
    void* ctx_ws = nullptr;
    static constexpr int kMaxGroups = 8;
    hipGraphExec_t graph_exec[kMaxGroups] = {};
    hipGraphExec_t graph_multi[kMaxGroups] = {};
    int graph_unroll = 16;
    static constexpr int kPreGroups = 4;
    int prefill_groups = 0;
    hipStream_t pre_stream[kPreGroups - 1] = {};
    hipEvent_t pre_fork = nullptr, pre_join[kPreGroups - 1] = {};
    hipStream_t grp_stream[kMaxGroups] = {};
    hipEvent_t ev_fork = nullptr, ev_join[kMaxGroups] = {};
    int gen_groups = 1;
    hipStream_t cap_stream = nullptr;
    dimx::GraphKey graph_key{};
    bool graph_valid = false;
    int use_graph = 1;
    int use_chain = 1;
    int cu_count = 0;
    float* chain_stats_dev = nullptr;
    int defer_ln = 1;
    unsigned long long* layer_prof_dev = nullptr;
    int multi_tr = 1;
    int use_layer_chain = 1;
    unsigned* chain_err_dev = nullptr;
    unsigned* chain_err_host = nullptr;
    hipEvent_t chain_err_ev = nullptr;
    int chain_faults = 0;
    int chain_fault_inject = 0;
    int use_qkv0_table = 1;
    float* qkv0_table = nullptr;
    int qkv0_M = 0, qkv0_at = -1;
    uint64_t qkv0_epoch = 0;
    uint64_t dec_epoch = 1;
    int qkv0_builds = 0;
    int use_kv0_table = 1;
    void* kv0_image = nullptr;
    int kv0_generations = 0;
    int use_sample_head = 1;
    int sample_head_generations = 0;
    int shard_row_off = 0, shard_rows_total = 0;
    int filter_kind = 0;
    float filter_a = 0.f, filter_b = 0.f;
    int xwin_on = 0, xwin_lookahead = 0;
    void* kv8_buf = nullptr;
    size_t kv8_bytes = 0;
    int kv8_samples_on = 0;
    void* self_kv8_buf = nullptr;
    size_t self_kv8_bytes = 0;
    int twin_on = 0, twin_lookahead = 0;
    const uint8_t* tcond_keep = nullptr;
    void* stream_sess = nullptr;
    dimx::MeshHead mesh;
    int lstm_faults = 0;
    int spk_embed_rows = 0;
};
```

dyadic-interaction-modeling_amd/csrc/ops.hip:

```cpp
#include "stages.hpp"

using namespace dimx;

extern "C" {

int dimx_op_lstm_layer(int dtype, const float* x, int B, int T, int In, int H, const float* const* w_ih, const float* const* w_hh,
                       const float* const* b_ih, const float* const* b_hh, float* y, int flags, int* faults_out, void* stream) {
    DIMX_REQUIRE(dtype == DIMX_F32, DIMX_ERR_ARG, "lstm_layer: only the f32 recurrence is built (dtype %d)", dtype);
    DIMX_REQUIRE(B >= 1 && T >= 1 && In >= 4, DIMX_ERR_ARG, "lstm_layer: bad shape");
    hipStream_t st = (hipStream_t)stream;
    int dev = 0, cus = 0;
    DIMX_HIP(hipGetDevice(&dev));
    DIMX_HIP(hipDeviceGetAttribute(&cus, hipDeviceAttributeMultiprocessorCount, dev));
    const size_t bytes = lstm_scratch_bytes(B, T, In);
    void* scratch = nullptr;
    DIMX_HIP(hipMalloc(&scratch, bytes));
    int faults = 0;
    const int rc = lstm_layer_run(x, B, T, In, H, w_ih, w_hh, b_ih, b_hh, y, scratch, bytes, flags, cus, &faults, st);
    const hipError_t e = hipStreamSynchronize(st);
    (void)hipFree(scratch);
    if (faults_out) *faults_out = faults;
    DIMX_TRY(rc);
    DIMX_HIP(e);
    return DIMX_OK;
// ... 572 lines not shown
    DIMX_REQUIRE(scratch && x && y && gamma, DIMX_ERR_ARG, "op_chain: null argument");
    int dev = 0, cus = 0;
    DIMX_HIP(hipGetDevice(&dev));
    DIMX_HIP(hipDeviceGetAttribute(&cus, hipDeviceAttributeMultiprocessorCount, dev));
    ChainArgs c;
    memset(&c, 0, sizeof(c));
    unsigned* u = (unsigned*)scratch;
    c.B = B;
    c.C = C;
    if (W1) {
        c.g1.W = W1; c.g1.N = C; c.g1.K = K1; c.g1.ldw = K1;
        c.A1 = A1; c.lda1 = K1;
        c.xr = (float*)(u + 512);
    }
    c.x = x;
    c.slabs = slabs;
    c.nslab = nslab;
    c.slab_stride = (long)B * C;
    c.y = y;
    c.gamma = gamma;
    if (W2) {
        c.g2.W = W2; c.g2.N = N2; c.g2.K = C; c.g2.ldw = C;
        c.out2 = out2; c.ld_out2 = N2;
    }
    c.counters = u;
    c.seen = u + 256;
    c.step = (const int32_t*)(u + 128);
    c.err = u + 129;
    DIMX_REQUIRE(chain_supported(c, cus), DIMX_ERR_ARG, "op_chain: shape not supported on this device (%d CUs)", cus);
    DIMX_HIP(hipMemsetAsync(u, 0, 512 * 4, (hipStream_t)stream));
    return launch_chain(c, (hipStream_t)stream);
}

int dimx_op_chain_ln(const void* A1, int K1, const void* W1, float* x, void* y, float* stats, const void* W2s,
                     const float* colsum2, int N2, float* out2, int B, int C, void* scratch, void* stream) {
    DIMX_REQUIRE(scratch && x && y && stats && A1 && W1, DIMX_ERR_ARG, "op_chain_ln: null argument");
    int dev = 0, cus = 0;
    DIMX_HIP(hipGetDevice(&dev));
    DIMX_HIP(hipDeviceGetAttribute(&cus, hipDeviceAttributeMultiprocessorCount, dev));
    ChainArgs c;
    memset(&c, 0, sizeof(c));
    unsigned* u = (unsigned*)scratch;
    c.B = B;
    c.C = C;
    c.g1.W = W1; c.g1.N = C; c.g1.K = K1; c.g1.ldw = K1;
    c.A1 = A1; c.lda1 = K1;
    c.xr = (float*)(u + 512);
    c.x = x;
    c.y = y;
    c.gamma = (const float*)x;
    c.defer = 1;
    c.stats = stats;
    if (W2s) {
        c.g2.W = W2s; c.g2.N = N2; c.g2.K = C; c.g2.ldw = C;
        c.out2 = out2; c.ld_out2 = N2;
        c.colsum2 = colsum2;
    }
    c.counters = u;
    c.seen = u + 256;
    c.step = (const int32_t*)(u + 128);
    c.err = u + 129;
    DIMX_REQUIRE(chain_supported(c, cus), DIMX_ERR_ARG, "op_chain_ln: shape not supported on this device (%d CUs)", cus);
    DIMX_HIP(hipMemsetAsync(u, 0, 512 * 4, (hipStream_t)stream));
    return launch_chain(c, (hipStream_t)stream);
}

int dimx_op_gemm_ln(int out_dtype, const void* A, const void* Ws, void* C, int M, int N, int K, const float* bias, int act,
                    const float* stats, const float* colsum, void* stream) {
    DIMX_REQUIRE(A && Ws && C && stats && colsum && M >= 1 && M <= 256, DIMX_ERR_ARG, "op_gemm_ln: bad argument");
    GemmArgs g;
    gemm_args_init(g);
    g.in_dtype = DIMX_BF16;
    g.out_dtype = out_dtype;
    g.A = A; g.lda = K;
    g.W = Ws; g.ldw = K;
    g.M = M; g.N = N; g.K = K;
    g.bias = bias;
    g.act = act;
    g.ln_stats = stats;
    g.ln_colsum = colsum;
    g.ln_C = K;
    gemm_set_plain_out(g, C, N);
    return launch_gemm(g, (hipStream_t)stream);
}

static int op_layer_chain(const float* qkv, int nslab, long slab_stride, void* sk, void* sv, int T, const void* ck, const void* cv,
                          int Tp, int n_keys, const uint8_t* kmask, const void* w_so, const void* w_cq, const float* colsum_cq,
                          const void* w_co, float* x, void* y, void* o, float* qc, float* stats, int B, const int32_t* step,
                          int call_index, float scale, void* scratch, void* prof, void* stream, const OpTabArgs* tab,
                          const SampleHeadArgs* head = nullptr) {
    DIMX_REQUIRE(qkv && sk && sv && ck && cv && w_so && w_cq && colsum_cq && w_co && x && y && o && qc && stats && step && scratch,
                 DIMX_ERR_ARG, "op_layer_chain: null argument");
    constexpr int H = 12, D = 64, inner = H * D, C = 1152;
    LayerChainArgs lc;
    memset(&lc, 0, sizeof(lc));
    lc.B = B;
    lc.C = C;
    DecodeAttnArgs& sa = lc.sa;
    sa.dtype = DIMX_BF16;
    sa.q = qkv; sa.q_ld = 3 * inner; sa.q_f32 = 1; sa.nslab = nslab; sa.slab_stride = slab_stride;
    sa.knew = qkv + inner; sa.vnew = qkv + 2 * inner; sa.kv_ld = 3 * inner;
    sa.kcache = sk; sa.vcache = sv; sa.Tmax = T;
    sa.out = o; sa.o_ld = inner; sa.B = B; sa.H = H; sa.step = step; sa.scale = scale;
    if (tab) set_tab(sa, *tab);
    DecodeAttnArgs& ca = lc.ca;
    ca.dtype = DIMX_BF16;
    ca.q = qc; ca.q_ld = inner; ca.q_f32 = 1; ca.nslab = 1; ca.slab_stride = (long)B * inner;
    ca.kcache = (void*)ck; ca.vcache = (void*)cv; ca.Tmax = Tp;
    ca.out = o; ca.o_ld = inner; ca.B = B; ca.H = H; ca.n_keys = n_keys; ca.kmask = kmask; ca.kmask_ld = n_keys; ca.scale = scale;
    lc.g_so.W = w_so; lc.g_so.N = C; lc.g_so.K = inner; lc.g_so.ldw = inner;
    lc.g_cq.W = w_cq; lc.g_cq.N = inner; lc.g_cq.K = C; lc.g_cq.ldw = C;
    lc.g_co.W = w_co; lc.g_co.N = C; lc.g_co.K = inner; lc.g_co.ldw = inner;
    lc.o = o; lc.ld_o = inner;
    lc.x = x; lc.y = y; lc.stats = stats; lc.colsum_cq = colsum_cq;
    lc.qc = qc; lc.ld_qc = inner;
    lc.counters = (unsigned*)scratch;
    lc.seen = lc.counters + 8 * 16;
    lc.err = lc.counters + 768;
    lc.step = nullptr;
    lc.epoch_add = call_index;
    if (head) lc.head = *head;
    lc.prof = (unsigned long long*)prof;
    lc.sc_stride = ((T > n_keys ? T : n_keys) + 15) / 16 * 16;
    int cu = 0, dev = 0;
    DIMX_HIP(hipGetDevice(&dev));
    DIMX_HIP(hipDeviceGetAttribute(&cu, hipDeviceAttributeMultiprocessorCount, dev));
    DIMX_REQUIRE(layer_chain_supported(lc, cu), DIMX_ERR_ARG, "op_layer_chain: not supported here (B = %d needs 129..256 clips, a 256-CU device)", B);
    return launch_layer_chain(lc, (hipStream_t)stream);
}

int dimx_op_layer_chain(const float* qkv, int nslab, long slab_stride, void* sk, void* sv, int T, const void* ck, const void* cv,
                        int Tp, int n_keys, const uint8_t* kmask, const void* w_so, const void* w_cq, const float* colsum_cq,
                        const void* w_co, float* x, void* y, void* o, float* qc, float* stats, int B, const int32_t* step,
                        int call_index, float scale, void* scratch, void* prof, void* stream) {
    return op_layer_chain(qkv, nslab, slab_stride, sk, sv, T, ck, cv, Tp, n_keys, kmask, w_so, w_cq, colsum_cq, w_co, x, y, o, qc, stats, B,
                          step, call_index, scale, scratch, prof, stream, nullptr);
}

int dimx_op_layer_chain_tab(const float* qkv, int nslab, long slab_stride, void* sk, void* sv, int T, const void* ck, const void* cv,
                            int Tp, int n_keys, const uint8_t* kmask, const void* w_so, const void* w_cq, const float* colsum_cq,
                            const void* w_co, float* x, void* y, void* o, float* qc, float* stats, int B, const int32_t* step,
                            int call_index, float scale, void* scratch, void* prof, const void* tab, int tab_ld, int tab_koff,
                            int tab_voff, int tab_rows, const int32_t* hist, int hist_ld, void* stream) {
    const OpTabArgs t = {tab, tab_ld, tab_koff, tab_voff, tab_rows, hist, hist_ld};
    return op_layer_chain(qkv, nslab, slab_stride, sk, sv, T, ck, cv, Tp, n_keys, kmask, w_so, w_cq, colsum_cq, w_co, x, y, o, qc, stats, B,
                          step, call_index, scale, scratch, prof, stream, &t);
}

int dimx_op_layer_chain_head(const float* qkv0, const float* logits, int top_k, const float* exp_noise, int rows_total, int32_t* tokens,
                             int tok_ld, float* logits_out, const float* emb_table, int32_t* params, void* sk, void* sv, int T, const void* ck,
                             const void* cv, int Tp, int n_keys, const uint8_t* kmask, const void* w_so, const void* w_cq,
                             const float* colsum_cq, const void* w_co, float* x, void* y, void* o, float* qc, float* stats, int B, float scale,
                             void* scratch, void* prof, const void* tab, int tab_ld, int tab_koff, int tab_voff, int tab_rows, int32_t* hist,
                             int hist_ld, void* stream) {
    DIMX_REQUIRE(qkv0 && logits && tokens && emb_table && params && hist && tab, DIMX_ERR_ARG, "op_layer_chain_head: null argument");
    const OpTabArgs t = {tab, tab_ld, tab_koff, tab_voff, tab_rows, hist, hist_ld};
    SampleHeadArgs hd;
    memset(&hd, 0, sizeof(hd));
    hd.on = 1;
    hd.logits = logits; hd.ld_logits = 512; hd.nslab = 1; hd.top_k = top_k; hd.noise = exp_noise; hd.rows_total = rows_total;
    hd.tokens = tokens; hd.tok_ld = tok_ld; hd.logits_out = logits_out; hd.logits_out_ld = tok_ld;
    hd.emb_table = emb_table; hd.qkv0 = qkv0; hd.qkv0_N = 3 * 12 * 64; hd.hist = hist; hd.hist_ld = hist_ld; hd.params = params;
    return op_layer_chain(qkv0, 1, 0, sk, sv, T, ck, cv, Tp, n_keys, kmask, w_so, w_cq, colsum_cq, w_co, x, y, o, qc, stats, B, params, 0, scale,
                          scratch, prof, stream, &t, &hd);
}

// ... 54 lines not shown
```

dyadic-interaction-modeling_amd/engine.py:

```python
import ctypes

import numpy as np
import torch

from . import lib as L
from . import sampling


class Engine:
    def __init__(self, device=None, mode=L.MODE_PARITY_F32, variant="slmft", mesh_dim=0):
        if not torch.cuda.is_available():
            raise L.DimxError("dimx needs a ROCm GPU (torch.cuda.is_available() is False); "
                              "there is no CPU fallback")
        self.device = torch.device(device if device is not None else "cuda:0")
        if self.device.index is None:
            self.device = torch.device("cuda", torch.cuda.current_device())
        self.lib = L.load()
        self.mode = mode
        assert variant in ("slmft", "legacy", "slm", "speaker")
        self.variant = variant
        if variant == "speaker":
            assert mesh_dim > 0, "the speaker variant needs mesh_dim"
            self.dims = L.speaker_dims(mesh_dim)
        else:
# ... 395 lines not shown
        prompt = prompt.to(torch.int32).contiguous()
        prompt_len = prompt_len.to(torch.int32).contiguous() if prompt_len is not None else None
        window = False
        if isinstance(prefill, str) or isinstance(prefill, tuple):
            kind, prefill = (prefill, None) if isinstance(prefill, str) else prefill
            if kind != "window":
                raise ValueError("prefill=%r: an integer P0, 'window' or ('window', P0)" % (kind,))
            window = True
        P0 = int(prefill) if prefill is not None else (Pmax if prompt_len is None else 1)
        if noise is not None:
            noise = noise.to(torch.float32).contiguous()
            assert tuple(noise.shape) == (self.n_gen(T), R, self.dims.num_tokens)
        self._chk(prompt, prompt_len, mask_u8, noise)
        n = self.n_gen(T)
        tokens = torch.empty(R, n, dtype=torch.int32, device=self.device)
        lg = torch.empty(R, n, self.dims.num_tokens, dtype=torch.float32, device=self.device) if (return_logits or return_scores) else None
        ws, wsb = self.workspace(B, T, n_samples)
        L.check(self.lib.dimx_generate_prompted(self.h, L.ptr(prompt), int(prompt.stride(0)), L.ptr(prompt_len), int(Pmax), P0,
                                                L.ptr(mask_u8), B, T, int(n_samples), float(temperature), int(top_k), L.ptr(noise),
                                                int(seed) & 0xFFFFFFFFFFFFFFFF, L.ptr(tokens), L.ptr(lg),
                                                (1 if no_prefill else 0) | (2 if window else 0), ws, wsb, self._s()), "dimx_generate_prompted")
        plen = None
        if return_scores:
            no_prefill = no_prefill or (self.cross_lookahead() is not None and not window)
            plen = prompt_len.clamp(1 if no_prefill else P0, Pmax) if prompt_len is not None \
                else torch.full((B,), Pmax, dtype=torch.int32, device=self.device)
        return self._generated(tokens, lg, mask_u8, T, n_samples, plen, return_logits, return_scores)

    def generate_beam(self, start, mask_u8, T, beam_width, prompt=None, prompt_len=None, prefill=None, return_logits=False,
                      return_backptr=False):
        W = int(beam_width)
        if prompt is None:
            prompt, prompt_len, prefill = start.reshape(-1, 1), None, 1
        B, Pmax = prompt.shape
        R = B * W
        prompt = prompt.to(torch.int32).contiguous()
        prompt_len = prompt_len.to(torch.int32).contiguous() if prompt_len is not None else None
        P0 = int(prefill) if prefill is not None else (Pmax if prompt_len is None else 1)
        lens = mask_u8.sum(1, dtype=torch.int32)
        self._chk(prompt, prompt_len, mask_u8)
        n = self.n_gen(T)
        tokens = torch.empty(R, n, dtype=torch.int32, device=self.device)
        scores = torch.empty(R, dtype=torch.float64, device=self.device)
        lg = torch.empty(R, n, self.dims.num_tokens, dtype=torch.float32, device=self.device) if return_logits else None
        bp = torch.empty(R, n, dtype=torch.int32, device=self.device) if return_backptr else None
        state = torch.empty(2 * R, dtype=torch.float64, device=self.device)
        ws, wsb = self.workspace(B, T, W)
        L.check(self.lib.dimx_generate_beam(self.h, L.ptr(prompt), int(prompt.stride(0)), L.ptr(prompt_len), int(Pmax), P0,
                                            L.ptr(mask_u8), L.ptr(lens), B, T, W, L.ptr(tokens), L.ptr(scores), L.ptr(bp), L.ptr(lg),
                                            L.ptr(state), state.numel() * 8, 0, ws, wsb, self._s()), "dimx_generate_beam")
        return (tokens, scores) + ((lg,) if return_logits else ()) + ((bp,) if return_backptr else ())

    def mesh_head(self, motion, template=None, safe=False, out=None):
        B, Lq, _ = motion.shape
        V = self.dims.mesh_dim
        motion = motion.to(torch.float32).contiguous()
        template = template.to(torch.float32).contiguous() if template is not None else None
        if template is not None:
            assert tuple(template.shape) == (B, V), "template must be [B, mesh_dim]"
        if out is None:
            out = torch.empty(B, Lq, V, dtype=torch.float32, device=self.device)
        assert tuple(out.shape) == (B, Lq, V) and out.dtype == torch.float32
        self._chk(motion, template, out)
        ws, wsb = self.workspace(B, Lq)
        L.check(self.lib.dimx_mesh_head(self.h, L.ptr(motion), L.ptr(template), B, Lq, L.ptr(out), 1 if safe else 0, ws, wsb,
                                        self._s()), "dimx_mesh_head")
        return out

    def lstm_faults(self):
        return int(self.lib.dimx_lstm_faults(self.h))

    def chain_faults(self):
        return int(self.lib.dimx_chain_faults(self.h))

    def qkv0_table_builds(self):
        return int(self.lib.dimx_qkv0_table_builds(self.h))

    def kv0_table_generations(self):
        return int(self.lib.dimx_kv0_table_generations(self.h))

    def sample_head_generations(self):
        return int(self.lib.dimx_sample_head_generations(self.h))

    def debug_chain_fault(self, n_calls=1):
        L.check(self.lib.dimx_debug_chain_fault(self.h, int(n_calls)), "dimx_debug_chain_fault")


class StreamSession:

    def __init__(self, eng, B, Tmax, start, lookahead=0, temperature=1.0, top_k=52, noise=None, seed=0, prompt=None, v_speaker=None,
                 v_audio=None):
        self.eng, self.B, self.Tmax, self.lookahead = eng, int(B), int(Tmax), int(lookahead)
        self._open = False
        lib, dev = eng.lib, eng.device
        need = lib.dimx_stream_workspace_bytes(eng.h, self.B, self.Tmax)
        if need == 0:
            raise L.DimxError("dimx_stream_workspace_bytes(%d,%d) = 0: sessions need the SLMFT variant and 2 <= Tmax <= 2048" % (B, Tmax))
        self._ws = torch.empty(need + 256, dtype=torch.uint8, device=dev)
        self._V = eng.dims.num_tokens
        self._tok = torch.zeros(self.B, self.Tmax - 1, dtype=torch.int32, device=dev)
        self._lg = None
        self.begin(start, temperature, top_k, noise, seed, prompt, v_speaker, v_audio)

    def _ws_ptr(self):
        base = self._ws.data_ptr()
        aligned = (base + 255) // 256 * 256
        return ctypes.c_void_p(aligned), self._ws.numel() - (aligned - base)

    def begin(self, start=None, temperature=1.0, top_k=52, noise=None, seed=0, prompt=None, v_speaker=None, v_audio=None):
        if self._open:
            raise L.DimxError("StreamSession.begin: the session is open (end() or close() first)")
        if noise is not None:
            noise = noise.to(torch.float32).contiguous()
            assert tuple(noise.shape) == (self.Tmax - 1, self.B, self._V)
        if prompt is not None:
            return self._begin_prompted(prompt, v_speaker, v_audio, temperature, top_k, noise, seed)
        start = start.to(torch.int32).contiguous()
        self.eng._chk(start, noise)
        assert tuple(start.shape) == (self.B,)
        self._noise = noise
        self._last = (0, 0)
        ws, wsb = self._ws_ptr()
        L.check(self.eng.lib.dimx_stream_begin(self.eng.h, L.ptr(start), self.B, self.Tmax, self.lookahead, float(temperature), int(top_k),
                                               L.ptr(self._noise), int(seed) & 0xFFFFFFFFFFFFFFFF, ws, wsb, self.eng._s()),
                "dimx_stream_begin")
        self._open = True
        self.frames = 0
        self.steps = 0

    def _begin_prompted(self, prompt, v_speaker, v_audio, temperature, top_k, noise, seed):
        from . import stream as _stream
        prompt = prompt.to(torch.int32).contiguous()
        v_speaker = v_speaker.to(torch.float32).contiguous()
        v_audio = v_audio.to(torch.float32).contiguous()
        self.eng._chk(prompt, v_speaker, v_audio, noise)
        B, P = prompt.shape
        F = v_speaker.shape[1]
        assert B == self.B and v_speaker.shape[0] == B and tuple(v_audio.shape[:2]) == (B, F)
        if not _stream.prompt_fits(P, self.lookahead, F, self.Tmax):
            raise ValueError("a session cannot start from P=%d codes and F=%d frames: need 1 <= P and P + max(lookahead, 0) = %d <= F <= Tmax = %d"
                             % (P, F, P + max(self.lookahead, 0), self.Tmax))
        need = self.eng.lib.dimx_stream_workspace_bytes_prompt(self.eng.h, self.B, self.Tmax)
        if self._ws.numel() < need + 256:
            self._ws = None
            self._ws = torch.empty(need + 256, dtype=torch.uint8, device=self.eng.device)
        self._noise = noise
        ws, wsb = self._ws_ptr()
        L.check(self.eng.lib.dimx_stream_begin_prompted(self.eng.h, L.ptr(prompt), P, P, L.ptr(v_speaker), L.ptr(v_audio), F, self.B, self.Tmax,
                                                        self.lookahead, float(temperature), int(top_k), L.ptr(self._noise),
                                                        int(seed) & 0xFFFFFFFFFFFFFFFF, ws, wsb, self.eng._s()), "dimx_stream_begin_prompted")
        self._open = True
        self.frames = F
        self.steps = P - 1
        self._last = (P - 1, P - 1)
        self._tok[:, :P - 1] = prompt[:, 1:]
        if self._lg is not None:
            self._lg[:, :P - 1] = 0

    def _logits(self):
        if self._lg is None:
            self._lg = torch.zeros(self.B, self.Tmax - 1, self._V, dtype=torch.float32, device=self.eng.device)
        return self._lg

    def _took(self, n_new, return_logits, extra=()):
        lo, hi = self.steps, self.steps + n_new
        self.steps = hi
# ... 400 lines not shown


def op_sample(logits, top_k=52, temperature=1.0, noise=None, seed=0, step=0, filter_logits_fn=None, filter_kwargs=None,
              return_keep=False):
    lib = L.load()
    R = logits.shape[0]
    tok = torch.empty(R, dtype=torch.int32, device=logits.device)
    if filter_logits_fn is not None or filter_kwargs or return_keep:
        kind, top_k, fa, fb = sampling.resolve(filter_logits_fn, filter_kwargs, top_k)
        keep = torch.empty(R, 512, dtype=torch.uint8, device=logits.device) if return_keep else None
        L.check(lib.dimx_op_sample_filtered(L.ptr(logits.contiguous()), R, kind, int(top_k), fa, fb, float(temperature),
                                            L.ptr(noise), int(seed), int(step), L.ptr(tok), L.ptr(keep),
                                            L.stream_ptr(logits.device)), "dimx_op_sample_filtered")
        return (tok, keep.bool()) if return_keep else tok
    L.check(lib.dimx_op_sample(L.ptr(logits.contiguous()), R, top_k, float(temperature), L.ptr(noise), int(seed),
                               int(step), L.ptr(tok), L.stream_ptr(logits.device)), "dimx_op_sample")
    return tok


def op_sample_guided(cond, uncond, scale, top_k=52, temperature=1.0, noise=None, seed=0, step=0, filter_logits_fn=None,
                     filter_kwargs=None, return_guided=True):
    lib = L.load()
    assert cond.shape == uncond.shape and cond.dtype == torch.float32 and uncond.dtype == torch.float32
    cond, uncond = cond.contiguous(), uncond.contiguous()
    nslab = cond.shape[0] if cond.dim() == 3 else 1
    R = cond.shape[-2]
    kind, top_k, fa, fb = sampling.resolve(filter_logits_fn, filter_kwargs, top_k)
    tok = torch.empty(2 * R, dtype=torch.int32, device=cond.device)
    g = torch.empty(R, 512, dtype=torch.float32, device=cond.device) if return_guided else None
    L.check(lib.dimx_op_sample_guided(L.ptr(cond), L.ptr(uncond), R, nslab, R * 512, float(scale), kind, int(top_k), fa, fb,
                                      float(temperature), L.ptr(noise), int(seed), int(step), L.ptr(tok), L.ptr(g),
                                      L.stream_ptr(cond.device)), "dimx_op_sample_guided")
    return (tok, g) if return_guided else tok


def op_chain(x, gamma, a1=None, w1=None, slabs=None, w2=None):
    lib = L.load()
    dev = x.device
    B, C = x.shape
    bf = lambda t: None if t is None else t.to(torch.bfloat16).contiguous()
    a1, w1, w2 = bf(a1), bf(w1), bf(w2)
    y = torch.empty(B, C, dtype=torch.bfloat16, device=dev)
    out2 = torch.empty(B, w2.shape[0], dtype=torch.float32, device=dev) if w2 is not None else None
    scratch = torch.zeros(512 + B * C, dtype=torch.int32, device=dev)
    nslab = 0 if slabs is None else slabs.shape[0]
    L.check(lib.dimx_op_chain(L.ptr(a1), a1.shape[1] if a1 is not None else 0, L.ptr(w1), L.ptr(x),
                              L.ptr(slabs.contiguous()) if slabs is not None else None, nslab, L.ptr(gamma), L.ptr(y),
                              L.ptr(w2), w2.shape[0] if w2 is not None else 0, L.ptr(out2), B, C, L.ptr(scratch),
                              L.stream_ptr(dev)), "dimx_op_chain")
    torch.cuda.synchronize(dev)
    flags = int(scratch[129].item())
    if flags:
        raise L.DimxError("chain kernel error flags 0x%x (1 = (XCD, slot) claimed twice, 2 = group barrier timeout)" % flags)
    return y, out2


def op_chain_ln(x, a1, w1, w2s=None, colsum2=None, return_flags=False):
    lib = L.load()
    dev = x.device
    B, C = x.shape
    a1, w1 = a1.to(torch.bfloat16).contiguous(), w1.to(torch.bfloat16).contiguous()
    y = torch.empty(B, C, dtype=torch.bfloat16, device=dev)
    stats = torch.zeros(8, 32, 32, 2, dtype=torch.float32, device=dev)
    out2 = torch.empty(B, w2s.shape[0], dtype=torch.float32, device=dev) if w2s is not None else None
    scratch = torch.zeros(512 + B * C, dtype=torch.int32, device=dev)
    L.check(lib.dimx_op_chain_ln(L.ptr(a1), a1.shape[1], L.ptr(w1), L.ptr(x), L.ptr(y), L.ptr(stats), L.ptr(w2s),
                                 L.ptr(colsum2), w2s.shape[0] if w2s is not None else 0, L.ptr(out2), B, C, L.ptr(scratch),
                                 L.stream_ptr(dev)), "dimx_op_chain_ln")
    torch.cuda.synchronize(dev)
    flags = int(scratch[129].item())
    if flags & 3:
        raise L.DimxError("chain kernel error flags 0x%x (1 = (XCD, slot) claimed twice, 2 = group barrier timeout)" % flags)
    return (y, stats, out2, flags) if return_flags else (y, stats, out2)


def op_gemm_ln(a, ws, stats, colsum, bias=None, act=0, out_bf16=False):
    lib = L.load()
    M, K = a.shape
    N = ws.shape[0]
    out = torch.empty(M, N, dtype=torch.bfloat16 if out_bf16 else torch.float32, device=a.device)
    L.check(lib.dimx_op_gemm_ln(L.BF16 if out_bf16 else L.F32, L.ptr(a), L.ptr(ws), L.ptr(out), M, N, K, L.ptr(bias), act,
                                L.ptr(stats), L.ptr(colsum), L.stream_ptr(a.device)), "dimx_op_gemm_ln")
    return out


def op_decode_attn(q, kcache, vcache, n_keys, scale, kmask=None, nsplit=0):
    lib = L.load()
    B, H, Tmax, _ = kcache.shape
    bf = kcache.dtype == torch.bfloat16
    q_f32 = q.dtype == torch.float32 and bf
    out = torch.empty(q.shape, dtype=kcache.dtype, device=q.device)
    L.check(lib.dimx_op_decode_attn(L.BF16 if bf else L.F32, L.ptr(q), L.ptr(kcache), L.ptr(vcache), L.ptr(out), B, H,
                                    Tmax, n_keys, float(scale), L.ptr(kmask), nsplit, 1 if q_f32 else 0,
                                    L.stream_ptr(q.device)),
            "dimx_op_decode_attn")
    return out


def op_append_attn(qkv, kcache, vcache, n0, scale):
    lib = L.load()
    B, H, Tmax, _ = kcache.shape
    Bq, c, ld = qkv.shape
    assert Bq == B and qkv.dtype == torch.float32 and qkv.is_contiguous() and kcache.is_contiguous() and vcache.is_contiguous()
    bf = kcache.dtype == torch.bfloat16
    out = torch.empty(B, c, H * 64, dtype=kcache.dtype, device=qkv.device)
    L.check(lib.dimx_op_append_attn(L.BF16 if bf else L.F32, L.ptr(qkv), ld, L.ptr(kcache), L.ptr(vcache), L.ptr(out), B, H, Tmax,
                                    int(n0), c, float(scale), L.stream_ptr(qkv.device)), "dimx_op_append_attn")
    return out


def op_cross_attn_win(q, kcache, vcache, lookahead, scale, t0=0, n_keys=None, kmask=None, out=None):
    lib = L.load()
    B, H, Tp, _ = kcache.shape
    Bq, Lq, ld = q.shape
    assert Bq == B and q.dtype == torch.float32 and q.is_contiguous() and kcache.is_contiguous() and vcache.is_contiguous()
    assert kmask is None or (kmask.dtype == torch.uint8 and kmask.is_contiguous() and kmask.shape[0] == B)
    bf = kcache.dtype == torch.bfloat16
    if out is None:
        out = torch.empty(B, Lq, H * 64, dtype=kcache.dtype, device=q.device)
    assert tuple(out.shape) == (B, Lq, H * 64) and out.dtype == kcache.dtype and out.is_contiguous()
    L.check(lib.dimx_op_cross_attn_win(L.BF16 if bf else L.F32, L.ptr(q), ld, L.ptr(kcache), L.ptr(vcache), Tp, L.ptr(out), H * 64, B, H, Lq,
                                       int(t0), Tp if n_keys is None else int(n_keys), int(lookahead), L.ptr(kmask),
                                       kmask.shape[1] if kmask is not None else 0, float(scale), L.stream_ptr(q.device)),
            "dimx_op_cross_attn_win")
    return out


def op_decode_attn_ex(q, kcache, vcache, scale, n_keys=0, step=None, kmask=None, kmask_ld=None, rows_per_clip=1, nsplit=0,
                      q_f32=None, lookahead=None, tab=None, hist=None, tab_koff=0, tab_voff=0, tab_rows=None):
    lib = L.load()
    B, H, Tmax, _ = kcache.shape
    bf = kcache.dtype == torch.bfloat16
    qs = q if q.dim() == 3 else q.unsqueeze(0)
    nslab, R, q_ld = qs.shape
    if q_f32 is None:
        q_f32 = q.dtype == torch.float32
    S = rows_per_clip if rows_per_clip > 1 else 1
    out = torch.empty(R, H * 64, dtype=kcache.dtype, device=q.device)
    kld = kmask_ld if kmask_ld is not None else (kmask.shape[1] if kmask is not None else 0)
    if tab is not None:
        L.check(lib.dimx_op_decode_attn_tab(L.BF16 if bf else L.F32, L.ptr(qs), q_ld, 1 if q_f32 else 0, nslab, qs.stride(0),
                                            L.ptr(kcache), L.ptr(vcache), L.ptr(out), H * 64, B, H, Tmax, L.ptr(step), float(scale),
                                            nsplit, L.ptr(tab), tab.stride(0), int(tab_koff), int(tab_voff),
                                            tab.shape[0] if tab_rows is None else int(tab_rows), L.ptr(hist), hist.stride(0),
                                            L.stream_ptr(q.device)), "dimx_op_decode_attn_tab")
        return out
    if lookahead is not None:
        L.check(lib.dimx_op_decode_attn_win(L.BF16 if bf else L.F32, L.ptr(qs), q_ld, 1 if q_f32 else 0, nslab, qs.stride(0),
                                            L.ptr(kcache), L.ptr(vcache), L.ptr(out), H * 64, B, H, Tmax, L.ptr(step), n_keys,
                                            L.ptr(kmask), kld, S, float(scale), nsplit, int(lookahead), L.stream_ptr(q.device)),
                "dimx_op_decode_attn_win")
        return out
    L.check(lib.dimx_op_decode_attn_ex(L.BF16 if bf else L.F32, L.ptr(qs), q_ld, 1 if q_f32 else 0, nslab, qs.stride(0),
                                       1 if step is not None else 0, L.ptr(kcache), L.ptr(vcache), L.ptr(out), H * 64, B, H, Tmax,
                                       L.ptr(step), n_keys, L.ptr(kmask), kld, S, float(scale), nsplit, L.stream_ptr(q.device)),
            "dimx_op_decode_attn_ex")
    return out


def op_kv8_quantize(cache, T=None, codes=None, scales=None):
    lib = L.load()
    B, H, Tp, _ = cache.shape
    assert cache.shape[3] == 64
    codes = torch.zeros(B, H, Tp, 64, dtype=torch.uint8, device=cache.device) if codes is None else codes
    scales = torch.zeros(B, H, Tp, dtype=torch.float32, device=cache.device) if scales is None else scales
    L.check(lib.dimx_op_kv8_quantize(L.BF16 if cache.dtype == torch.bfloat16 else L.F32, L.ptr(cache), B, H, Tp, Tp if T is None else int(T),
# ... 613 lines not shown
```

dyadic-interaction-modeling_amd/lib.py:

```python
import ctypes
import os
from ctypes import (POINTER, c_char_p, c_float, c_int, c_int32, c_int64, c_size_t, c_uint64,
                    c_void_p)

import torch

HERE = os.path.dirname(os.path.abspath(__file__))
LIB_PATH = os.environ.get("DIMX_LIB", os.path.join(HERE, "libdimx_hip.so"))

MODE_PARITY_F32 = 0
MODE_PERF_BF16 = 1
F32, BF16 = 0, 1
ACT_NONE, ACT_LEAKY, ACT_GELU_TANH, ACT_GELU_ERF = 0, 1, 2, 3


class DimxError(RuntimeError):
    pass


class Dims(ctypes.Structure):
    _fields_ = [(n, c_int) for n in (
        "vq_in_dim", "vq_hidden", "vq_layers", "vq_heads", "vq_inter", "vq_n_embed", "vq_zdim",
        "dim_in", "dim", "dim_a", "enc_depth", "dec_depth", "heads", "dim_head", "num_tokens",
        "max_seq_len", "ff_mult", "variant", "spk_in_dim", "spk_hidden", "spk_heads", "spk_inter",
# ... 55 lines not shown
                                           c_void_p, c_uint64, c_void_p, c_size_t, c_void_p]),
    "dimx_stream_push": (c_int, [c_void_p, c_void_p, c_void_p, c_int, c_void_p, c_int, c_void_p, c_void_p, POINTER(c_int), c_void_p]),
    "dimx_stream_end": (c_int, [c_void_p, c_void_p, c_int, c_void_p, POINTER(c_int), c_void_p]),
    "dimx_stream_abort": (c_int, [c_void_p]),
    "dimx_stream_state": (c_int, [c_void_p, POINTER(c_int), POINTER(c_int), POINTER(c_int)]),
    "dimx_stream_set_events": (c_int, [c_void_p, c_void_p, c_void_p, c_void_p, c_void_p]),
    "dimx_encode_ctx": (c_int, [c_void_p, c_void_p, c_void_p, c_void_p, c_int, c_int, c_int, c_void_p,
                                c_void_p, c_size_t, c_void_p]),
    "dimx_legacy_speaker_features": (c_int, [c_void_p, c_void_p, c_void_p, c_int, c_int, c_void_p, c_void_p,
                                             c_void_p, c_size_t, c_void_p]),
    "dimx_slm_encode": (c_int, [c_void_p, c_void_p, c_void_p, c_void_p, c_void_p, c_void_p, c_int, c_int, c_void_p,
                                c_void_p, c_void_p, c_void_p, c_size_t, c_void_p]),
    "dimx_set_context": (c_int, [c_void_p, c_void_p, c_int, c_int, c_void_p, c_int, c_int, c_int, c_void_p, c_size_t,
                                 c_void_p]),
    "dimx_decode_tf": (c_int, [c_void_p, c_void_p, c_void_p, c_void_p, c_int, c_int, c_void_p, c_void_p,
                               c_void_p, c_void_p, c_size_t, c_void_p]),
    "dimx_decode_tf_win": (c_int, [c_void_p, c_void_p, c_void_p, c_int, c_int, c_int, c_void_p, c_void_p, c_void_p, c_void_p,
                                   c_size_t, c_void_p]),
    "dimx_generate": (c_int, [c_void_p, c_void_p, c_void_p, c_int, c_int, c_int, c_float, c_int, c_void_p, c_uint64,
                              c_void_p, c_void_p, c_void_p, c_size_t, c_void_p]),
    "dimx_workspace_bytes_prompt": (c_size_t, [c_void_p, c_int, c_int, c_int, c_int]),
    "dimx_generate_prompted": (c_int, [c_void_p, c_void_p, c_int, c_void_p, c_int, c_int, c_void_p, c_int, c_int, c_int, c_float,
                                       c_int, c_void_p, c_uint64, c_void_p, c_void_p, c_int, c_void_p, c_size_t, c_void_p]),
    "dimx_generate_beam": (c_int, [c_void_p, c_void_p, c_int, c_void_p, c_int, c_int, c_void_p, c_void_p, c_int, c_int, c_int, c_void_p,
                                   c_void_p, c_void_p, c_void_p, c_void_p, c_size_t, c_int, c_void_p, c_size_t, c_void_p]),
    "dimx_workspace_bytes_guided": (c_size_t, [c_void_p, c_int, c_int]),
    "dimx_generate_guided": (c_int, [c_void_p, c_void_p, c_int, c_void_p, c_int, c_void_p, c_int, c_int, c_float, c_float, c_int, c_void_p,
                                     c_uint64, c_void_p, c_void_p, c_void_p, c_void_p, c_size_t, c_void_p]),
    "dimx_train_num_params": (c_int, [c_void_p]),
    "dimx_train_total": (c_int64, [c_void_p]),
    "dimx_train_param_info": (c_int, [c_void_p, c_int, POINTER(c_char_p), POINTER(c_int64), POINTER(c_int64)]),
    "dimx_train_workspace_bytes": (c_size_t, [c_void_p, c_int, c_int]),
    "dimx_train_forward_backward": (c_int, [c_void_p, c_void_p, c_void_p, c_void_p, c_void_p, c_void_p, c_void_p, c_void_p, c_int,
                                            c_int, c_void_p, c_void_p, c_void_p, c_size_t, c_void_p]),
    "dimx_train_graph_stats": (c_int, [c_void_p, c_void_p]),
    "dimx_set_train_lookahead": (c_int, [c_void_p, c_int, c_int]),
    "dimx_train_lookahead": (c_int, [c_void_p, POINTER(c_int), POINTER(c_int)]),
    "dimx_set_train_cond_keep": (c_int, [c_void_p, c_void_p]),
    "dimx_train_cond_keep": (c_int, [c_void_p, POINTER(c_void_p)]),
    "dimx_train_legacy_workspace_bytes": (c_size_t, [c_void_p, c_int, c_int]),
    "dimx_train_legacy_forward_backward": (c_int, [c_void_p, c_void_p, c_void_p, c_void_p, c_void_p, c_void_p, c_void_p, c_void_p, c_void_p,
                                                   c_void_p, c_int, c_int, c_void_p, c_void_p, c_void_p, c_void_p, c_size_t, c_void_p]),
    "dimx_train_slm_workspace_bytes": (c_size_t, [c_void_p, c_int, c_int]),
    "dimx_train_slm_forward_backward": (c_int, [c_void_p] + [c_void_p] * 14 + [c_int, c_int, c_void_p, c_void_p, c_size_t, c_void_p]),
    "dimx_train_vq_num_params": (c_int, [c_void_p, c_int]),
    "dimx_train_vq_total": (c_int64, [c_void_p, c_int]),
    "dimx_train_vq_param_info": (c_int, [c_void_p, c_int, c_int, POINTER(c_char_p), POINTER(c_int64), POINTER(c_int64)]),
    "dimx_train_vq_workspace_bytes": (c_size_t, [c_void_p, c_int, c_int]),
    "dimx_train_vq_forward_backward": (c_int, [c_void_p, c_int, c_void_p, c_void_p, c_void_p, c_int, c_int, c_float, c_float, c_float,
                                               c_uint64, c_int64, c_void_p, c_void_p, c_void_p, c_void_p, c_size_t, c_void_p]),
    "dimx_train_conv_num_params": (c_int, [c_void_p]),
    "dimx_train_conv_total": (c_int64, [c_void_p]),
    "dimx_train_conv_param_info": (c_int, [c_void_p, c_int, POINTER(c_char_p), POINTER(c_int64), POINTER(c_int64)]),
    "dimx_train_conv_workspace_bytes": (c_size_t, [c_void_p, c_int, c_int]),
    "dimx_train_conv_forward_backward": (c_int, [c_void_p, c_void_p, c_void_p, c_void_p, c_void_p, c_void_p, c_void_p, c_int, c_int, c_int,
                                                 c_int, c_void_p, c_void_p, c_void_p, c_size_t, c_void_p]),
    "dimx_train_spk_num_params": (c_int, [c_void_p]),
    "dimx_train_spk_total": (c_int64, [c_void_p]),
    "dimx_train_spk_param_info": (c_int, [c_void_p, c_int, POINTER(c_char_p), POINTER(c_int64), POINTER(c_int64)]),
    "dimx_train_spk_workspace_bytes": (c_size_t, [c_void_p, c_int, c_int]),
    "dimx_train_spk_forward_backward": (c_int, [c_void_p] + [c_void_p] * 9 + [c_int, c_int, c_void_p, c_void_p, c_void_p, c_void_p, c_void_p,
                                                c_size_t, c_void_p]),
    "dimx_op_lstm_layer_bwd": (c_int, [c_int, c_void_p, c_int, c_int, c_int, c_int, POINTER(c_void_p), POINTER(c_void_p),
                                       POINTER(c_void_p), POINTER(c_void_p), c_void_p, c_void_p, POINTER(c_void_p), POINTER(c_void_p),
                                       POINTER(c_void_p), c_int, POINTER(c_int), c_void_p]),
    "dimx_train_adamw": (c_int, [c_void_p, c_void_p, c_void_p, c_void_p, c_int64, c_float, c_float, c_float, c_float, c_float,
                                 c_int, c_float, c_void_p, c_void_p]),
    "dimx_op_train_attention": (c_int, [c_int, c_void_p, c_void_p, c_void_p, c_void_p, c_void_p, c_void_p, c_int, c_int, c_int,
                                        c_int, c_int, c_float, c_void_p, c_void_p, c_void_p, c_void_p, c_void_p, c_void_p,
                                        c_void_p]),
    "dimx_op_train_attention_win": (c_int, [c_int, c_void_p, c_void_p, c_void_p, c_void_p, c_void_p, c_void_p, c_int, c_int, c_int,
                                            c_int, c_int, c_float, c_int, c_int, c_void_p, c_void_p, c_void_p, c_void_p, c_void_p,
                                            c_void_p, c_void_p]),
    "dimx_op_train_layernorm_bwd": (c_int, [c_void_p, c_void_p, c_void_p, c_void_p, c_int, c_int, c_int, c_void_p, c_void_p, c_void_p,
                                            c_size_t, c_void_p]),
    "dimx_op_train_colsum": (c_int, [c_void_p, c_int, c_int, c_void_p, c_void_p, c_size_t, c_void_p]),
    "dimx_op_train_prep": (c_int, [c_int, c_int, c_void_p, c_int, c_void_p, c_int, c_void_p, c_void_p, c_int, c_int, c_void_p, c_size_t,
                                   c_void_p, c_size_t, c_void_p, c_size_t, POINTER(c_int), c_void_p]),
    "dimx_op_train_cross_entropy": (c_int, [c_void_p, c_void_p, c_int, c_void_p, c_void_p, c_void_p, c_void_p]),
    "dimx_chain_faults": (c_int, [c_void_p]),
    "dimx_qkv0_table_builds": (c_int, [c_void_p]),
    "dimx_kv0_table_generations": (c_int, [c_void_p]),
    "dimx_sample_head_generations": (c_int, [c_void_p]),
    "dimx_lstm_faults": (c_int, [c_void_p]),
    "dimx_mesh_head": (c_int, [c_void_p, c_void_p, c_void_p, c_int, c_int, c_void_p, c_int, c_void_p, c_size_t, c_void_p]),
    "dimx_op_lstm_layer": (c_int, [c_int, c_void_p, c_int, c_int, c_int, c_int, POINTER(c_void_p), POINTER(c_void_p),
                                   POINTER(c_void_p), POINTER(c_void_p), c_void_p, c_int, POINTER(c_int), c_void_p]),
    "dimx_debug_chain_fault": (c_int, [c_void_p, c_int]),
    "dimx_op_gemm_slabs": (c_int, [c_int, c_int, c_int, c_int, c_int]),
    "dimx_op_split_x3": (c_int, [c_void_p, c_void_p, ctypes.c_long, c_void_p]),
    "dimx_op_gemm_x3": (c_int, [c_void_p, c_int, c_void_p, c_void_p, c_int, c_int, c_int, c_int, c_void_p, c_int, c_void_p, c_int, c_int,
                                c_void_p]),
    "dimx_op_gemm": (c_int, [c_int, c_int, c_void_p, c_int, c_void_p, c_int, c_void_p, c_int, c_int, c_int,
                             c_int, c_void_p, c_int, c_void_p, c_int, c_int, c_void_p, c_int, c_void_p]),
    "dimx_op_gemm_headmajor": (c_int, [c_int, c_void_p, c_int, c_void_p, c_int, c_void_p, c_int, c_int, c_int, c_int, c_int,
                                       c_int, c_void_p]),
    "dimx_op_gemm_map": (c_int, [c_int, c_int, c_void_p, c_int, c_void_p, c_int, c_int, c_int, c_int, c_void_p, c_int, c_void_p, c_int,
                                 c_int, c_int, POINTER(c_void_p), POINTER(c_int64), POINTER(c_int32), c_void_p, c_int, c_int, c_float,
                                 c_int, c_int, c_int, c_void_p]),
    "dimx_op_gemm_route": (c_int, [c_int, c_int, c_void_p, c_int, c_void_p, c_int, c_int, c_int, c_int, c_void_p, c_int, c_void_p, c_int,
                                   c_int, c_int, POINTER(c_void_p), POINTER(c_int64), POINTER(c_int32), c_void_p, c_int, c_int, c_float,
                                   c_int, c_int, c_int]),
    "dimx_op_layernorm": (c_int, [c_int, c_void_p, c_void_p, c_void_p, c_void_p, c_int, c_int, c_void_p]),
    "dimx_op_instnorm": (c_int, [c_int, c_void_p, c_void_p, c_void_p, c_int, c_int, c_int, c_void_p]),
    "dimx_op_attention": (c_int, [c_int, c_void_p, c_void_p, c_void_p, c_void_p, c_int, c_int, c_int, c_int,
                                  c_int, c_int, c_int, c_int, c_int, c_float, c_int, c_void_p, c_void_p,
                                  c_void_p]),
    "dimx_op_attention_rowv": (c_int, [c_void_p, c_void_p, c_void_p, c_void_p, c_int, c_int, c_int, c_int, c_int, c_int, c_int,
                                       c_int, c_int, c_float, c_int, c_void_p, c_void_p, c_void_p]),
    "dimx_op_attention_strided": (c_int, [c_void_p, c_void_p, c_void_p, c_void_p, c_int, c_int, c_int, c_int, c_int,
                                          POINTER(ctypes.c_long), POINTER(ctypes.c_long), POINTER(ctypes.c_long), POINTER(ctypes.c_long),
                                          c_float, c_int, c_void_p, c_void_p, c_int, c_int, c_void_p]),
    "dimx_op_decode_attn": (c_int, [c_int, c_void_p, c_void_p, c_void_p, c_void_p, c_int, c_int, c_int, c_int,
                                    c_float, c_void_p, c_int, c_int, c_void_p]),
    "dimx_op_append_attn": (c_int, [c_int, c_void_p, c_int, c_void_p, c_void_p, c_void_p, c_int, c_int, c_int, c_int, c_int, c_float,
                                    c_void_p]),
    "dimx_op_cross_attn_win": (c_int, [c_int, c_void_p, c_int, c_void_p, c_void_p, c_int, c_void_p, c_int, c_int, c_int, c_int, c_int, c_int,
                                       c_int, c_void_p, c_int, c_float, c_void_p]),
    "dimx_op_decode_attn_self": (c_int, [c_int, c_void_p, c_int, c_void_p, c_void_p, c_void_p, c_int, c_int, c_int,
                                         c_void_p, c_float, c_int, c_void_p]),
    "dimx_op_decode_attn_ex": (c_int, [c_int, c_void_p, c_int, c_int, c_int, ctypes.c_long, c_int, c_void_p, c_void_p, c_void_p,
                                       c_int, c_int, c_int, c_int, c_void_p, c_int, c_void_p, c_int, c_int, c_float, c_int,
                                       c_void_p]),
    "dimx_op_decode_attn_win": (c_int, [c_int, c_void_p, c_int, c_int, c_int, ctypes.c_long, c_void_p, c_void_p, c_void_p,
                                        c_int, c_int, c_int, c_int, c_void_p, c_int, c_void_p, c_int, c_int, c_float, c_int,
                                        c_int, c_void_p]),
    "dimx_op_decode_attn_tab": (c_int, [c_int, c_void_p, c_int, c_int, c_int, ctypes.c_long, c_void_p, c_void_p, c_void_p, c_int, c_int,
                                        c_int, c_int, c_void_p, c_float, c_int, c_void_p, c_int, c_int, c_int, c_int, c_void_p, c_int,
                                        c_void_p]),
    "dimx_op_mlp_fused": (c_int, [c_void_p, c_void_p, c_void_p, c_void_p, c_void_p, c_void_p, c_void_p, c_int, c_int, c_int, c_int, c_void_p]),
    "dimx_mlp_fused_packed_bytes": (c_size_t, [c_int, c_int]),
    "dimx_mlp_fused_pack": (c_int, [c_void_p, c_void_p, c_void_p, c_int, c_int, c_void_p, c_size_t]),
    "dimx_op_mlp_fused_packed": (c_int, [c_void_p, c_void_p, c_void_p, c_void_p, c_void_p, c_int, c_int, c_int, c_int, c_void_p]),
    "dimx_op_add_slabs_layernorm": (c_int, [c_int, c_void_p, c_void_p, c_int, ctypes.c_long, c_void_p, c_void_p, c_int,
                                            c_int, c_void_p]),
    "dimx_op_chain": (c_int, [c_void_p, c_int, c_void_p, c_void_p, c_void_p, c_int, c_void_p, c_void_p, c_void_p, c_int,
                              c_void_p, c_int, c_int, c_void_p, c_void_p]),
    "dimx_op_chain_ln": (c_int, [c_void_p, c_int, c_void_p, c_void_p, c_void_p, c_void_p, c_void_p, c_void_p, c_int,
                                 c_void_p, c_int, c_int, c_void_p, c_void_p]),
    "dimx_op_layer_chain": (c_int, [c_void_p, c_int, ctypes.c_long, c_void_p, c_void_p, c_int, c_void_p, c_void_p, c_int, c_int, c_void_p,
                                    c_void_p, c_void_p, c_void_p, c_void_p, c_void_p, c_void_p, c_void_p, c_void_p, c_void_p, c_int,
                                    c_void_p, c_int, c_float, c_void_p, c_void_p, c_void_p]),
    "dimx_op_layer_chain_tab": (c_int, [c_void_p, c_int, ctypes.c_long, c_void_p, c_void_p, c_int, c_void_p, c_void_p, c_int, c_int, c_void_p,
                                        c_void_p, c_void_p, c_void_p, c_void_p, c_void_p, c_void_p, c_void_p, c_void_p, c_void_p, c_int,
                                        c_void_p, c_int, c_float, c_void_p, c_void_p, c_void_p, c_int, c_int, c_int, c_int, c_void_p,
                                        c_int, c_void_p]),
    "dimx_op_layer_chain_head": (c_int, [c_void_p, c_void_p, c_int, c_void_p, c_int, c_void_p, c_int, c_void_p, c_void_p, c_void_p, c_void_p,
                                         c_void_p, c_int, c_void_p, c_void_p, c_int, c_int, c_void_p, c_void_p, c_void_p, c_void_p, c_void_p,
                                         c_void_p, c_void_p, c_void_p, c_void_p, c_void_p, c_int, c_float, c_void_p, c_void_p, c_void_p, c_int,
                                         c_int, c_int, c_int, c_void_p, c_int, c_void_p]),
    "dimx_op_sample_step": (c_int, [c_void_p, c_int, c_int, c_void_p, c_int, c_void_p, c_int, c_void_p, c_void_p, c_int, c_void_p, c_void_p,
                                    c_void_p, c_int, c_void_p, c_int, c_void_p, c_void_p]),
    "dimx_op_gemm_ln": (c_int, [c_int, c_void_p, c_void_p, c_void_p, c_int, c_int, c_int, c_void_p, c_int, c_void_p,
                                c_void_p, c_void_p]),
    "dimx_op_fd_select_ws_bytes": (c_size_t, [c_int, c_int, c_int]),
    "dimx_op_fd_select": (c_int, [c_void_p, ctypes.c_long, ctypes.c_long, c_void_p, ctypes.c_long, ctypes.c_long, ctypes.c_long, c_void_p,
                                  c_int, c_int, c_int, c_int, c_int, c_int, c_void_p, c_void_p, c_void_p, c_void_p, c_void_p, c_size_t,
                                  c_void_p]),
    "dimx_op_mesh_metrics_ws_bytes": (c_size_t, [c_int, c_int, c_int, c_int]),
    "dimx_op_mesh_metrics": (c_int, [c_void_p, ctypes.c_long, ctypes.c_long, c_void_p, ctypes.c_long, ctypes.c_long, c_void_p, ctypes.c_long,
                                     POINTER(c_int32), c_int, c_int, c_int, c_void_p, c_int, c_void_p, c_int, c_void_p, c_void_p, c_void_p,
                                     c_void_p, c_size_t, c_void_p]),
    "dimx_op_listener_metrics_ws_bytes": (c_size_t, [c_int, c_int, c_int]),
    "dimx_op_listener_metrics": (c_int, [c_void_p, ctypes.c_long, ctypes.c_long, c_void_p, ctypes.c_long, ctypes.c_long, c_void_p, ctypes.c_long,
                                         ctypes.c_long, c_void_p, c_int, c_int, c_int, c_int, POINTER(c_int32), c_int, c_void_p, c_void_p,
                                         c_void_p, c_size_t, c_void_p]),
# ... 111 lines not shown
```

include/dimx.h:

```cpp
#ifndef DIMX_H
#define DIMX_H

#include <stddef.h>
#include <stdint.h>

#ifdef __cplusplus
extern "C" {
#endif

typedef struct dimx_ctx* dimx_handle;

typedef enum {
    DIMX_OK = 0,
    DIMX_ERR_ARG = -1,
    DIMX_ERR_HIP = -2,
    DIMX_ERR_WEIGHT = -3,
    DIMX_ERR_STATE = -4,
    DIMX_ERR_WORKSPACE = -5
} dimx_status;

#define DIMX_MODE_PARITY_F32 0
#define DIMX_MODE_PERF_BF16 1

#define DIMX_F32 0
// ... 47 lines not shown
                        float* x_s_out, void* ws, size_t ws_bytes, void* stream);

int dimx_set_shard(dimx_handle h, int row_offset, int rows_total);

int dimx_encode_ctx(dimx_handle h, const float* v_speaker, const float* v_audio, const uint8_t* mask,
                    int B, int T, int for_generate, float* x_s_out, void* ws, size_t ws_bytes,
                    void* stream);

int dimx_slm_encode(dimx_handle h, const float* v_speaker, const float* v_listener, const uint8_t* mask,
                    const uint8_t* mask_speaker, const uint8_t* mask_listener, int B, int T, float* x_s,
                    float* x_l, float* x_joint, void* ws, size_t ws_bytes, void* stream);

int dimx_set_context(dimx_handle h, const float* x, int ldx_rows, int which_patch, const float* v_audio, int B,
                     int T, int for_generate, void* ws, size_t ws_bytes, void* stream);

int dimx_legacy_speaker_features(dimx_handle h, const float* v_speaker, const uint8_t* mask, int B, int T,
                                 float* x_speaker_out, int32_t* idx_out, void* ws, size_t ws_bytes,
                                 void* stream);

int dimx_decode_tf(dimx_handle h, const int32_t* z_l, const uint8_t* ctx_mask, const uint8_t* kv_mask,
                   int B, int T, float* logits, float* row_loss, int32_t* argmax_tok, void* ws,
                   size_t ws_bytes, void* stream);

int dimx_decode_tf_win(dimx_handle h, const int32_t* z_l, const uint8_t* ctx_mask, int B, int T, int lookahead, float* logits,
                       float* row_loss, int32_t* argmax_tok, void* ws, size_t ws_bytes, void* stream);

int dimx_generate(dimx_handle h, const int32_t* start, const uint8_t* ctx_mask, int B, int T, int n_samples,
                  float temperature, int top_k, const float* exp_noise, uint64_t seed, int32_t* tokens,
                  float* logits_out, void* ws, size_t ws_bytes, void* stream);

size_t dimx_workspace_bytes_prompt(dimx_handle h, int B, int T, int n_samples, int P0);
int dimx_generate_prompted(dimx_handle h, const int32_t* prompt, int ld_prompt, const int32_t* prompt_len, int Pmax, int P0,
                           const uint8_t* ctx_mask, int B, int T, int n_samples, float temperature, int top_k,
                           const float* exp_noise, uint64_t seed, int32_t* tokens, float* logits_out, int flags, void* ws,
                           size_t ws_bytes, void* stream);

#define DIMX_BEAM_STATE_BYTES(B, W) ((size_t)16 * (size_t)(B) * (size_t)(W))
int dimx_generate_beam(dimx_handle h, const int32_t* prompt, int ld_prompt, const int32_t* prompt_len, int Pmax, int P0,
                       const uint8_t* ctx_mask, const int32_t* lens, int B, int T, int beam_width, int32_t* tokens, double* scores,
                       int32_t* backptr, float* logits_out, void* beam_state, size_t beam_state_bytes, int flags, void* ws, size_t ws_bytes,
                       void* stream);

size_t dimx_workspace_bytes_guided(dimx_handle h, int B, int T);
int dimx_generate_guided(dimx_handle h, const int32_t* prompt, int ld_prompt, const int32_t* prompt_len, int Pmax, const uint8_t* ctx_mask,
                         int B, int T, float scale, float temperature, int top_k, const float* exp_noise, uint64_t seed, int32_t* tokens,
                         float* logits_out, float* branch_logits_out, void* ws, size_t ws_bytes, void* stream);

int dimx_chain_faults(dimx_handle h);

typedef enum {
    DIMX_FILTER_TOP_K = 0,
    DIMX_FILTER_TOP_P = 1,
    DIMX_FILTER_MIN_P = 2,
    DIMX_FILTER_TOP_A = 3
} dimx_filter_kind;
int dimx_set_sampler_filter(dimx_handle h, int kind, float a, float b);

int dimx_set_cross_lookahead(dimx_handle h, int on, int lookahead);
int dimx_cross_lookahead(dimx_handle h, int* on, int* lookahead);
size_t dimx_cross_kv8_bytes(dimx_handle h, int B, int T);
int dimx_set_cross_kv8(dimx_handle h, void* buf, size_t bytes);
int dimx_cross_kv8(dimx_handle h, void** buf, size_t* bytes);
int dimx_set_cross_kv8_samples(dimx_handle h, int on);
int dimx_cross_kv8_samples(dimx_handle h, int* on);
size_t dimx_self_kv8_bytes(dimx_handle h, int R, int T);
int dimx_set_self_kv8(dimx_handle h, void* buf, size_t bytes);
int dimx_self_kv8(dimx_handle h, void** buf, size_t* bytes);
size_t dimx_stream_workspace_bytes(dimx_handle h, int B, int Tmax);
int dimx_stream_begin(dimx_handle h, const int32_t* start, int B, int Tmax, int lookahead, float temperature, int top_k, const float* noise,
                      uint64_t seed, void* ws, size_t ws_bytes, void* stream);
size_t dimx_stream_workspace_bytes_prompt(dimx_handle h, int B, int Tmax);
int dimx_stream_begin_prompted(dimx_handle h, const int32_t* prompt, int ld_prompt, int P, const float* v_speaker, const float* v_audio, int F,
                               int B, int Tmax, int lookahead, float temperature, int top_k, const float* noise, uint64_t seed, void* ws,
                               size_t ws_bytes, void* stream);
int dimx_stream_push(dimx_handle h, const float* v_speaker, const float* v_audio, int c, int32_t* tokens_out, int ld_tok, float* logits_out,
                     float* x_s_out, int* n_new, void* stream);
int dimx_stream_end(dimx_handle h, int32_t* tokens_out, int ld_tok, float* logits_out, int* n_new, void* stream);
int dimx_stream_abort(dimx_handle h);
int dimx_stream_state(dimx_handle h, int* frames, int* steps, int* open);
int dimx_stream_set_events(dimx_handle h, void* ev_start, void* ev_encoded, void* ev_appended, void* ev_stepped);
int dimx_qkv0_table_builds(dimx_handle h);
int dimx_kv0_table_generations(dimx_handle h);
int dimx_sample_head_generations(dimx_handle h);
int dimx_debug_chain_fault(dimx_handle h, int n_calls);

int dimx_mesh_head(dimx_handle h, const float* motion, const float* templ, int B, int L, float* mesh_out, int flags, void* ws,
                   size_t ws_bytes, void* stream);
int dimx_lstm_faults(dimx_handle h);

int dimx_train_num_params(dimx_handle h);
int64_t dimx_train_total(dimx_handle h);
int dimx_train_param_info(dimx_handle h, int i, const char** name, int64_t* offset, int64_t* numel);
size_t dimx_train_workspace_bytes(dimx_handle h, int B, int T);
int dimx_train_forward_backward(dimx_handle h, const float* params, float* grads, const float* v_speaker, const float* v_audio,
                                const uint8_t* mask, const int32_t* z_l, const uint8_t* kv_mask, int B, int T, float* loss_out,
                                float* logits_out, void* ws, size_t ws_bytes, void* stream);
int dimx_train_graph_stats(dimx_handle h, int64_t* out3);
int dimx_set_train_lookahead(dimx_handle h, int on, int lookahead);
int dimx_train_lookahead(dimx_handle h, int* on, int* lookahead);
int dimx_set_train_cond_keep(dimx_handle h, const uint8_t* keep_dev);
int dimx_train_cond_keep(dimx_handle h, const uint8_t** keep_dev);
size_t dimx_train_legacy_workspace_bytes(dimx_handle h, int B, int T);
int dimx_train_legacy_forward_backward(dimx_handle h, const float* params, float* grads, const float* x_speaker, const int32_t* z_l,
                                       const float* v_listener, const uint8_t* mask, const int32_t* listener_ids, const float* codebook,
                                       const float* pe, int B, int T, float* loss_out, float* pred_out, float* logits_out, void* ws,
                                       size_t ws_bytes, void* stream);
size_t dimx_train_slm_workspace_bytes(dimx_handle h, int B, int T);
int dimx_train_slm_forward_backward(dimx_handle h, const float* params, float* grads, const float* v_speaker, const float* v_listener,
                                    const float* v_audio, const uint8_t* mask, const uint8_t* mask_speaker, const uint8_t* mask_listener,
                                    const int32_t* z_s, const int32_t* z_l, const float* codebook_s, const float* codebook_l,
                                    const float* pe_s, const float* pe_l, int B, int T, float* loss_out, void* ws, size_t ws_bytes,
                                    void* stream);
int dimx_train_vq_num_params(dimx_handle h, int which);
int64_t dimx_train_vq_total(dimx_handle h, int which);
int dimx_train_vq_param_info(dimx_handle h, int which, int i, const char** name, int64_t* offset, int64_t* numel);
size_t dimx_train_vq_workspace_bytes(dimx_handle h, int B, int T);
int dimx_train_vq_forward_backward(dimx_handle h, int which, const float* params, float* grads, const float* x, int B, int T, float beta,
                                   float quant_loss_weight, float dropout_p, uint64_t dropout_seed, int64_t step, float* loss_out,
                                   float* pred_out, int32_t* idx_out, void* ws, size_t ws_bytes, void* stream);
int dimx_train_conv_num_params(dimx_handle h);
int64_t dimx_train_conv_total(dimx_handle h);
int dimx_train_conv_param_info(dimx_handle h, int i, const char** name, int64_t* offset, int64_t* numel);
size_t dimx_train_conv_workspace_bytes(dimx_handle h, int B, int T);
int dimx_train_conv_forward_backward(dimx_handle h, const float* params, float* grads, const float* motion, const float* templ,
                                     const float* target, const float* vert_w, int n_mouth, int B, int T, int flags, float* loss_out,
                                     float* mesh_out, void* ws, size_t ws_bytes, void* stream);
int dimx_train_spk_num_params(dimx_handle h);
int64_t dimx_train_spk_total(dimx_handle h);
int dimx_train_spk_param_info(dimx_handle h, int i, const char** name, int64_t* offset, int64_t* numel);
size_t dimx_train_spk_workspace_bytes(dimx_handle h, int B, int T);
int dimx_train_spk_forward_backward(dimx_handle h, const float* params, float* grads, const float* v_emoca, const float* v_audio,
                                    const uint8_t* mask, const int32_t* z, const int32_t* speaker_ids, const float* codebook_s,
                                    const float* pe_s, int B, int T, float* loss_out, float* logits_out, int32_t* idx_out, float* pred_out,
                                    void* ws, size_t ws_bytes, void* stream);
int dimx_op_lstm_layer_bwd(int dtype, const float* x, int B, int T, int In, int H, const float* const* w_ih, const float* const* w_hh,
                           const float* const* b_ih, const float* const* b_hh, const float* dy, float* dx, float* const* dw_ih,
                           float* const* dw_hh, float* const* db, int flags, int* faults_out, void* stream);
int dimx_train_adamw(float* params, const float* grads, float* exp_avg, float* exp_avg_sq, int64_t n, float lr, float beta1,
                     float beta2, float eps, float weight_decay, int step, float max_norm, float* scratch, void* stream);
int dimx_op_train_attention(int mfma, const float* q, const float* k, const float* v, const float* d_o, const uint8_t* kmask,
                            const uint8_t* kmask2, int B, int H, int Lq, int Lk, int causal, float scale, float* o, float* lse,
                            float* delta, float* dq, float* dk, float* dv, void* stream);
int dimx_op_train_attention_win(int mfma, const float* q, const float* k, const float* v, const float* d_o, const uint8_t* kmask,
                                const uint8_t* kmask2, int B, int H, int Lq, int Lk, int causal, float scale, int win, int lookahead,
                                float* o, float* lse, float* delta, float* dq, float* dk, float* dv, void* stream);
int dimx_op_train_layernorm_bwd(const float* x, const float* gamma, const float* dy, float* dx, int accumulate, int M, int C, float* dgamma,
                                float* dbeta, float* scratch, size_t scratch_floats, void* stream);
int dimx_op_train_colsum(const float* dy, int M, int C, float* out, float* scratch, size_t scratch_floats, void* stream);
int dimx_op_train_prep(int dtype, int mode, const float* src, int lds, const float* src2, int lds2, const float* gamma, const float* beta,
                       int rows, int cols, void* o, size_t o_elems, void* t, size_t t_elems, float* colpart, size_t colpart_floats,
                       int* dims3, void* stream);
int dimx_op_train_cross_entropy(const float* logits, const int32_t* targets, int R, float* row_loss, float* dlogits, float* loss_out2,
                                void* stream);


int dimx_op_gemm(int in_dtype, int out_dtype, const void* A, int lda, const void* W, int ldw, void* C,
                 int ldc, int M, int N, int K, const float* bias, int act, const float* residual,
                 int ldr, int conv_T, const int32_t* conv_lens, int flags, void* stream);
int dimx_op_split_x3(const float* w, void* planes, long n, void* stream);
int dimx_op_gemm_x3(const float* A, int lda, const void* planes, float* C, int ldc, int M, int N, int K, const float* bias, int act,
                    const float* residual, int ldr, int flags, void* stream);
int dimx_op_gemm_slabs(int in_dtype, int M, int N, int K, int flags);
int dimx_op_gemm_headmajor(int dtype, const void* A, int lda, const void* W, int ldw, void* out, int M, int N, int K,
                           int rowT, int Tp, int nlayers, void* stream);
int dimx_op_gemm_map(int in_dtype, int out_dtype, const void* A, int lda, const void* W, int ldw, int M, int N, int K, const float* bias,
                     int act, const float* residual, int ldr, int rowT, int nseg, void* const* seg_ptr, const int64_t* seg_strides,
                     const int32_t* seg_D, const float* rowadd, int ld_rowadd, int rowadd_mode, float rowadd_scale, int rowadd_off,
                     int rowadd_div, int flags, void* stream);
int dimx_op_gemm_route(int in_dtype, int out_dtype, const void* A, int lda, const void* W, int ldw, int M, int N, int K, const float* bias,
                       int act, const float* residual, int ldr, int rowT, int nseg, void* const* seg_ptr, const int64_t* seg_strides,
                       const int32_t* seg_D, const float* rowadd, int ld_rowadd, int rowadd_mode, float rowadd_scale, int rowadd_off,
                       int rowadd_div, int flags);
int dimx_op_lstm_layer(int dtype, const float* x, int B, int T, int In, int H, const float* const* w_ih, const float* const* w_hh,
                       const float* const* b_ih, const float* const* b_hh, float* y, int flags, int* faults_out, void* stream);
int dimx_op_layernorm(int out_dtype, const float* x, void* y, const float* gamma, const float* beta,
                      int M, int C, void* stream);
int dimx_op_instnorm(int out_dtype, const float* x, void* y, const int32_t* lens, int B, int T, int C,
                     void* stream);
int dimx_op_attention(int dtype, const void* q, const void* k, const void* vt, void* out, int B, int H,
                      int Lq, int Lk, int D, int ldq, int ldk, int ld_vt, int ldo, float scale,
                      int causal, const int32_t* lens, const uint8_t* kmask, void* stream);
int dimx_op_attention_rowv(const void* q, const void* k, const void* v, void* out, int B, int H, int Lq, int Lk, int D, int ldq,
                           int ldk, int ldv, int ldo, float scale, int causal, const int32_t* lens, const uint8_t* kmask,
                           void* stream);
int dimx_op_attention_strided(const void* q, const void* k, const void* v, void* out, int B, int H, int Lq, int Lk, int D,
                              const long* q_str, const long* k_str, const long* v_str, const long* o_str, float scale, int causal,
                              const int32_t* lens, const uint8_t* kmask, int kmask_ld, int prepacked, void* stream);
int dimx_op_decode_attn(int dtype, const void* q, const void* kcache, const void* vcache, void* out, int B, int H,
                        int Tmax, int n_keys, float scale, const uint8_t* kmask, int nsplit, int q_is_f32,
                        void* stream);
int dimx_op_decode_attn_self(int dtype, const void* qkv, int ld, void* kcache, void* vcache, void* out, int B, int H,
                             int Tmax, const int32_t* step_dev, float scale, int q_is_f32, void* stream);
int dimx_op_decode_attn_ex(int dtype, const void* q, int q_ld, int q_is_f32, int nslab, long slab_stride, int self_attn, void* kcache,
                           void* vcache, void* out, int o_ld, int B, int H, int Tmax, const int32_t* step_dev, int n_keys,
                           const uint8_t* kmask, int kmask_ld, int rows_per_clip, float scale, int nsplit, void* stream);
int dimx_op_decode_attn_tab(int dtype, const void* q, int q_ld, int q_is_f32, int nslab, long slab_stride, void* kcache, void* vcache,
                            void* out, int o_ld, int B, int H, int Tmax, const int32_t* step_dev, float scale, int nsplit, const void* tab,
                            int tab_ld, int tab_koff, int tab_voff, int tab_rows, const int32_t* hist, int hist_ld, void* stream);
int dimx_op_decode_attn_win(int dtype, const void* q, int q_ld, int q_is_f32, int nslab, long slab_stride, void* kcache, void* vcache,
                            void* out, int o_ld, int B, int H, int Tmax, const int32_t* step_dev, int n_keys, const uint8_t* kmask,
                            int kmask_ld, int rows_per_clip, float scale, int nsplit, int lookahead, void* stream);
int dimx_op_kv8_quantize(int dtype, const void* cache, int B, int H, int Tp, int T, uint8_t* codes, float* scales, void* stream);
int dimx_op_decode_attn_kv8(int out_dtype, const void* q, int q_ld, int q_is_f32, int nslab, long slab_stride, const uint8_t* kcodes,
                            const float* kscale, const uint8_t* vcodes, const float* vscale, void* out, int o_ld, int B, int H, int Tmax,
                            const int32_t* step_dev, int n_keys, const uint8_t* kmask, int kmask_ld, int rows_per_clip, float scale, int nsplit,
                            int lookahead, int win, void* stream);
int dimx_op_decode_attn_kv8_multi(int out_dtype, const void* q, int q_ld, int q_is_f32, int nslab, long slab_stride, const uint8_t* kcodes,
                                  const float* kscale, const uint8_t* vcodes, const float* vscale, void* out, int o_ld, int B, int H, int Tmax,
                                  const int32_t* step_dev, int n_keys, const uint8_t* kmask, int kmask_ld, int rows_per_clip, float scale,
                                  int nsplit, int lookahead, int win, int exact, void* stream);
int dimx_op_decode_attn_self_kv8(int out_dtype, const float* qkv, int ld, int nslab, long slab_stride, uint8_t* kcodes, float* kscale,
                                 uint8_t* vcodes, float* vscale, void* out, int o_ld, int B, int H, int Tmax, const int32_t* step_dev, int n,
                                 float scale, int nsplit, void* stream);
int dimx_op_append_attn(int dtype, const float* qkv, int ld, void* kcache, void* vcache, void* out, int B, int H, int Tmax, int n0, int c,
                        float scale, void* stream);
int dimx_op_cross_attn_win(int dtype, const float* q, int ld, const void* kcache, const void* vcache, int Tp, void* out, int o_ld, int B, int H,
                           int Lq, int t0, int n_keys, int lookahead, const uint8_t* kmask, int kmask_ld, float scale, void* stream);
int dimx_op_mlp_fused(float* x, const float* w1_host, const float* b1_host, const float* w2_host, const float* b2, const float* ln_g,
                      const float* ln_b, int M, int C, int F, int act, void* stream);
size_t dimx_mlp_fused_packed_bytes(int C, int F);
int dimx_mlp_fused_pack(const float* w1_host, const float* b1_host, const float* w2_host, int C, int F, void* out_host, size_t out_bytes);
int dimx_op_mlp_fused_packed(float* x, const void* packed, const float* b2, const float* ln_g, const float* ln_b, int M, int C, int F,
                             int act, void* stream);
int dimx_op_add_slabs_layernorm(int out_dtype, float* x, const float* slabs, int nslab, long slab_stride, void* y,
                                const float* gamma, int M, int C, void* stream);
int dimx_op_chain(const void* A1, int K1, const void* W1, float* x, const float* slabs, int nslab, const float* gamma,
                  void* y, const void* W2, int N2, float* out2, int B, int C, void* scratch, void* stream);
int dimx_op_chain_ln(const void* A1, int K1, const void* W1, float* x, void* y, float* stats, const void* W2s,
                     const float* colsum2, int N2, float* out2, int B, int C, void* scratch, void* stream);
int dimx_op_gemm_ln(int out_dtype, const void* A, const void* Ws, void* C, int M, int N, int K, const float* bias, int act,
                    const float* stats, const float* colsum, void* stream);
int dimx_op_layer_chain(const float* qkv, int nslab, long slab_stride, void* sk, void* sv, int T, const void* ck, const void* cv,
                        int Tp, int n_keys, const uint8_t* kmask, const void* w_so, const void* w_cq, const float* colsum_cq,
                        const void* w_co, float* x, void* y, void* o, float* qc, float* stats, int B, const int32_t* step,
                        int call_index, float scale, void* scratch, void* prof, void* stream);
int dimx_op_layer_chain_tab(const float* qkv, int nslab, long slab_stride, void* sk, void* sv, int T, const void* ck, const void* cv,
                            int Tp, int n_keys, const uint8_t* kmask, const void* w_so, const void* w_cq, const float* colsum_cq,
                            const void* w_co, float* x, void* y, void* o, float* qc, float* stats, int B, const int32_t* step,
                            int call_index, float scale, void* scratch, void* prof, const void* tab, int tab_ld, int tab_koff,
                            int tab_voff, int tab_rows, const int32_t* hist, int hist_ld, void* stream);
int dimx_op_layer_chain_head(const float* qkv0, const float* logits, int top_k, const float* exp_noise, int rows_total, int32_t* tokens,
                             int tok_ld, float* logits_out, const float* emb_table, int32_t* params, void* sk, void* sv, int T, const void* ck,
                             const void* cv, int Tp, int n_keys, const uint8_t* kmask, const void* w_so, const void* w_cq,
                             const float* colsum_cq, const void* w_co, float* x, void* y, void* o, float* qc, float* stats, int B, float scale,
                             void* scratch, void* prof, const void* tab, int tab_ld, int tab_koff, int tab_voff, int tab_rows, int32_t* hist,
                             int hist_ld, void* stream);
int dimx_op_sample_step(const float* logits, int R, int top_k, const float* exp_noise, int rows_total, int32_t* tokens, int tok_ld,
                        float* logits_out, const float* emb_table, int C, float* x_next, const float* qkv0, float* qkv0_out, int qkv0_N,
                        int32_t* hist, int hist_ld, int32_t* params, void* stream);
size_t dimx_op_fd_select_ws_bytes(int B, int S, int F);
int dimx_op_fd_select(const float* y_true, long yt_clip_stride, long yt_frame_stride, const float* y_pred, long yp_clip_stride,
                      long yp_sample_stride, long yp_frame_stride, const int32_t* lens, int B, int S, int L, int W, int c0, int F,
                      double* fd, int32_t* win, uint8_t* ok, float* best, void* workspace, size_t workspace_bytes, void* stream);
size_t dimx_op_mesh_metrics_ws_bytes(int B, int L, int n_mouth, int n_upper);
int dimx_op_mesh_metrics(const float* y_true, long yt_clip_stride, long yt_frame_stride, const float* y_pred, long yp_clip_stride,
                         long yp_frame_stride, const float* templ, long templ_clip_stride, const int32_t* lens, int B, int L, int n_vert,
                         const int32_t* mouth, int n_mouth, const int32_t* upper, int n_upper, double* clip_out, double* frame_max,
                         int32_t* status, void* workspace, size_t workspace_bytes, void* stream);
#define DIMX_LM_ROW 133
size_t dimx_op_listener_metrics_ws_bytes(int B, int n_win, int F);
int dimx_op_listener_metrics(const float* y_true, long yt_clip_stride, long yt_frame_stride, const float* y_pred, long yp_clip_stride,
                             long yp_frame_stride, const float* x, long x_clip_stride, long x_frame_stride, const int32_t* lens, int B,
                             int L, int Wy, int Wx, const int32_t* windows, int n_win, double* fd, double* moments, void* workspace,
                             size_t workspace_bytes, void* stream);
size_t dimx_op_kmeans_fit_ws_bytes(int N, int K, int F);
int dimx_op_kmeans_fit(const float* frames, long frame_stride, int N, int W, int c0, int F, int K, int first_index, const double* U,
                       int trials, double tol, int max_iter, double* centers, int32_t* n_iter, int32_t* status, int32_t* labels,
                       void* workspace, size_t workspace_bytes, void* stream);
int dimx_op_sid_assign(const float* frames, long frame_stride, int M, int W, int c0, int F, const double* centers, int K, int64_t* hist,
                       double* sid, int32_t* labels, void* stream);
int dimx_op_seq_logprob(const float* logits, long row_stride, long step_stride, const int32_t* tokens, long tok_row_stride,
                        const int32_t* first, const int32_t* last, int rows_per_clip, int R, int n, double* tok_logprob, double* score,
                        int32_t* count, void* stream);
int dimx_op_score_select(const double* score, const float* y_pred, long yp_clip_stride, long yp_sample_stride, long yp_frame_stride,
                         const int32_t* lens, const int32_t* tokens, long tok_row_stride, int B, int S, int L, int W, int n,
                         int32_t* win, uint8_t* ok, float* best, int32_t* best_tokens, void* stream);
size_t dimx_op_consensus_select_ws_bytes(int B, int S, int F, int kind);
int dimx_op_consensus_select(const float* y_pred, long yp_clip_stride, long yp_sample_stride, long yp_frame_stride,
                             const int32_t* lens, int B, int S, int L, int W, int c0, int F, int kind ,
                             double* dist , double* risk , int32_t* win, uint8_t* ok,
                             float* best , const int32_t* tokens, long tok_row_stride, int n_tok,
                             int32_t* best_tokens , void* workspace, size_t workspace_bytes, void* stream);
int dimx_op_pool_desc(const float* x, long clip_stride, long frame_stride, const int32_t* lens, int N, int T, int D,
                      int kind , double* desc, double* norm, void* stream);
size_t dimx_op_nn_search_ws_bytes(int Q, int N, int D, int K);
int dimx_op_nn_search(const double* q_desc, long q_row_stride, const double* q_norm, const double* x_desc, long x_row_stride,
                      const double* x_norm, int Q, int N, int D, int K, int32_t* idx, double* sim, int32_t* found,
                      double* sim_out , void* workspace, size_t workspace_bytes, void* stream);
int dimx_op_nn_gather(const int32_t* idx, const float* lib_seq, long clip_stride, long frame_stride, const int32_t* lib_lens,
                      const int32_t* q_lens, int Q, int K, int N, int Lmax, int L, int W, float* out, int32_t* out_len, void* stream);
int dimx_op_beam_step(const float* logits, const double* cum, const int32_t* mode, const int32_t* forced_tok, int B, int W,
                      int32_t* parent, int32_t* token, double* cum_out, void* stream);
int dimx_op_beam_reorder(void* cache, int dtype, const int32_t* parent, int R, int W, int H, int T, int c, void* stream);
int dimx_op_sample(const float* logits, int R, int top_k, float temperature, const float* exp_noise,
                   uint64_t seed, uint64_t step, int32_t* tokens, void* stream);
int dimx_op_sample_filtered(const float* logits, int R, int kind, int top_k, float a, float b, float temperature,
                            const float* exp_noise, uint64_t seed, uint64_t step, int32_t* tokens, uint8_t* keep_out,
                            void* stream);
int dimx_op_sample_guided(const float* cond, const float* uncond, int R, int nslab, long slab_stride, float scale, int kind, int top_k,
                          float a, float b, float temperature, const float* exp_noise, uint64_t seed, uint64_t step, int32_t* tokens,
                          float* guided_out, void* stream);

#ifdef __cplusplus
}
#endif
#endif
```

Before: 1746 clips/s.

## Fuse feed-forward GEMM pair into one kernel with XCC-local group barrier handoff

The two feed-forward GEMMs of each decoder layer (1152→4608 with GELU, then 4608→1152 split-K into slabs) now run in one 256-block launch. Each block computes its GEMM1 tile, then waits on a per-XCC group counter barrier before its GEMM2 tile. It prefetches the W2 weight panels before the barrier so weight loads overlap the wait. This removes a kernel launch and the inter-kernel drain per layer per decode step, but depends on exactly 256 CUs, co-resident blocks and spin-wait barriers with a timeout error flag.

```diff
diff --git a/dyadic-interaction-modeling_amd/csrc/common.hpp b/dyadic-interaction-modeling_amd/csrc/common.hpp
--- a/dyadic-interaction-modeling_amd/csrc/common.hpp
+++ b/dyadic-interaction-modeling_amd/csrc/common.hpp
@@ -458,6 +458,18 @@
 };
 bool layer_chain_supported(const LayerChainArgs& a, int cu_count);
 int launch_layer_chain(const LayerChainArgs& a, hipStream_t s);
+struct Ff72Args {
+    GemmArgs g1, g2;
+    unsigned* counters;
+    unsigned* seen;
+    const int32_t* step;
+    int epoch_add;
+    unsigned* err;
+    int fault;
+    unsigned long long* prof;
+};
+bool ff72_supported(const Ff72Args& a, int cu_count);
+int launch_ff72(const Ff72Args& a, hipStream_t s);
 size_t chain_plan(ChainArgs& a);
 bool chain_supported(const ChainArgs& a, int cu_count);
 int launch_chain(const ChainArgs& a, hipStream_t s);
diff --git a/dyadic-interaction-modeling_amd/csrc/gemm.hip b/dyadic-interaction-modeling_amd/csrc/gemm.hip
--- a/dyadic-interaction-modeling_amd/csrc/gemm.hip
+++ b/dyadic-interaction-modeling_amd/csrc/gemm.hip
@@ -896,6 +896,10 @@
     epilogue<T, OutT, 1, 1>(a, acc, m0 + wm * 32, n0 + wn * 32, half, l31, split);
 }
 
+struct Ws72Plain {
+    __device__ __forceinline__ void handoff() {}
+    __device__ __forceinline__ void landed() {}
+};
 template <typename OutT>
 struct Ws72 {
     static constexpr int BM = 64, BN = 72, BK = 64, STAGES = 4, NLOAD = 4, NCONS = 6;
@@ -904,9 +908,9 @@
     static constexpr int SMEM_BYTES = RING_BYTES > 84 * 1024 ? RING_BYTES : 84 * 1024;
     static_assert(STAGES - 2 == 2, "the loaders' counted waits below are written for two k-tiles in flight behind the current slot");
 
-    template <int LW>
-    static __device__ __forceinline__ void loader(const GemmArgs& a, int lw, int lane, int m0, int n0, int kt0, int nk, unsigned char* smem,
-                                                  float* ln_sm) {
+    template <int LW, int AUX_A, bool HANDOFF, typename Hook>
+    static __device__ __forceinline__ void loader(const GemmArgs& a, int lw, int lane, int m0, int n0, int kt0, int nk, int slot0,
+                                                  unsigned char* smem, float* ln_sm, Hook& hook) {
         constexpr int LA = 2, LPT = LA + LW;
         static_assert((STAGES - 1) * LPT < 56, "ring depth");
         const bf16* __restrict__ A = (const bf16*)a.A;
@@ -932,14 +936,21 @@
             n = n < a.N ? n : a.N - 1;
             gW[j] = W + (size_t)n * a.ldw + c * 8 + (size_t)kt0 * BK;
         }
-        auto issue = [&](int kt, int slot) {
+        auto issue_a = [&](int kt, int slot) {
             unsigned char* base = smem + slot * TILE_BYTES;
 #pragma unroll
             for (int j = 0; j < LA; ++j)
-                __builtin_amdgcn_global_load_lds((glb_void_t*)(gA[j] + (size_t)kt * BK), (lds_void_t*)(base + pA[j] * 1024), 16, 0, 0);
+                __builtin_amdgcn_global_load_lds((glb_void_t*)(gA[j] + (size_t)kt * BK), (lds_void_t*)(base + pA[j] * 1024), 16, 0, AUX_A);
+        };
+        auto issue_w = [&](int kt, int slot) {
+            unsigned char* base = smem + slot * TILE_BYTES;
 #pragma unroll
             for (int j = 0; j < LW; ++j)
                 __builtin_amdgcn_global_load_lds((glb_void_t*)(gW[j] + (size_t)kt * BK), (lds_void_t*)(base + BM * 128 + pW[j] * 1024), 16, 0, 0);
+        };
+        auto issue = [&](int kt, int slot) {
+            issue_a(kt, slot);
+            issue_w(kt, slot);
         };
         float2 lp[8];
         if (a.ln_stats) {
@@ -950,11 +961,22 @@
             for (int i = 0; i < 8; ++i) lp[i] = sp[(size_t)i * 32];
         }
         int issued = 0;
-        for (; issued < STAGES - 1 && issued < nk; ++issued) issue(issued, issued);
-        int slot_next = issued % STAGES;
+        if constexpr (HANDOFF) {
+            for (int i = 0; i < STAGES - 1; ++i) issue_w(i, (slot0 + i) % STAGES);
+            hook.handoff();
+            for (int i = 0; i < STAGES - 1; ++i) issue_a(i, (slot0 + i) % STAGES);
+            issued = STAGES - 1;
+        } else {
+            for (; issued < STAGES - 1 && issued < nk; ++issued) issue(issued, (slot0 + issued) % STAGES);
+        }
+        int slot_next = (slot0 + issued) % STAGES;
         const int st_ln = nk >= 2 ? nk - 2 : 0;
         for (int st = 0; st < nk; ++st) {
-            {
+            if (HANDOFF && st == 0) {
+                wait_vmcnt<2 * LA>();
+            } else if (HANDOFF && st == 1) {
+                wait_vmcnt<LA + LPT>();
+            } else {
                 int done = st + 1, all = issued;
                 done = done < nk ? done : nk;
                 all = all < nk ? all : nk;
@@ -999,8 +1021,6 @@
     }
 
     static __device__ __forceinline__ void body(const GemmArgs& a, int block_id, int nblocks, unsigned char* smem, float* ln_sm) {
-        const int tid = threadIdx.x, lane = tid & 63;
-        const int wave = __builtin_amdgcn_readfirstlane(tid >> 6);
         const int tiles_n = (a.N + BN - 1) / BN, tiles_m = (a.M + BM - 1) / BM;
         const int ntiles = tiles_m * tiles_n;
         int bid = block_id;
@@ -1008,8 +1028,17 @@
             const int q = nblocks >> 3, r = nblocks & 7, x = bid & 7, i = bid >> 3;
             bid = (x < r ? x * (q + 1) : r * (q + 1) + (x - r) * q) + i;
         }
-        const int split = bid / ntiles, tile = bid - split * ntiles;
-        const int tile_n = tile / tiles_m, tile_m = tile - tile_n * tiles_m;
+        const int split = bid / ntiles, t_in = bid - split * ntiles;
+        const int tile_n = t_in / tiles_m, tile_m = t_in - tile_n * tiles_m;
+        Ws72Plain hook;
+        tile<0, false>(a, tile_m, tile_n, split, 0, smem, ln_sm, hook);
+    }
+
+    template <int AUX_A, bool HANDOFF, typename Hook>
+    static __device__ __forceinline__ void tile(const GemmArgs& a, int tile_m, int tile_n, int split, int slot0, unsigned char* smem,
+                                                float* ln_sm, Hook& hook) {
+        const int tid = threadIdx.x, lane = tid & 63;
+        const int wave = __builtin_amdgcn_readfirstlane(tid >> 6);
         const int m0 = tile_m * BM, n0 = tile_n * BN;
         const int nk_all = (a.kloop ? a.kloop : a.ldw) / BK;
         const int per = (nk_all + a.splitk - 1) / a.splitk;
@@ -1020,9 +1049,9 @@
         if (wave >= NCONS) {
             const int lw = wave - NCONS;
             if (lw == 0)
-                loader<3>(a, lw, lane, m0, n0, kt0, nk, smem, ln_sm);
+                loader<3, AUX_A, HANDOFF>(a, lw, lane, m0, n0, kt0, nk, slot0, smem, ln_sm, hook);
             else
-                loader<2>(a, lw, lane, m0, n0, kt0, nk, smem, ln_sm);
+                loader<2, AUX_A, HANDOFF>(a, lw, lane, m0, n0, kt0, nk, slot0, smem, ln_sm, hook);
             return;
         }
         const int wm = wave / 3, wn = wave - 3 * wm;
@@ -1051,9 +1080,11 @@
         const int mrem = a.M - row_base;
         const int act = a.act;
         const bool has_ln = a.ln_stats != nullptr;
-        unsigned boff = 0;
+        unsigned boff = (unsigned)slot0 * TILE_BYTES;
+        if constexpr (HANDOFF) hook.handoff();
         for (int st = 0; st < nk; ++st) {
             __builtin_amdgcn_s_barrier();
+            if (HANDOFF && st == 0) hook.landed();
             u32x4_t fa[4][1], fw[4][1];
 #pragma unroll
             for (int q = 0; q < 4; ++q) {
@@ -1133,6 +1164,75 @@
     __shared__ __attribute__((aligned(16))) unsigned char smem[Ws72<OutT>::SMEM_BYTES];
     __shared__ __attribute__((aligned(16))) float ln_sm[128];
     Ws72<OutT>::body(a, blockIdx.x, gridDim.x, smem, ln_sm);
+}
+
+__device__ __forceinline__ unsigned ff72_xcc_id() {
+    unsigned v;
+    asm volatile("s_getreg_b32 %0, hwreg(HW_REG_XCC_ID)" : "=s"(v));
+    return v & 0xf;
+}
+__device__ __forceinline__ unsigned ff72_ld_sc1(const unsigned* p) { return __hip_atomic_load(p, __ATOMIC_RELAXED, __HIP_MEMORY_SCOPE_AGENT); }
+
+struct Ff72Hook {
+    unsigned* ctr;
+    unsigned target;
+    unsigned* err;
+    unsigned long long* prof;
+    __device__ __forceinline__ void stamp(int i) {
+        if (prof && threadIdx.x == 0) prof[i] = wall_clock64();
+    }
+    __device__ __forceinline__ void handoff() {
+        if (threadIdx.x < Ws72<float>::NCONS * 64) asm volatile("s_waitcnt vmcnt(0)" ::: "memory");
+        stamp(1);
+        __builtin_amdgcn_s_barrier();
+        if (threadIdx.x == 0) {
+            __hip_atomic_fetch_add(ctr, 1u, __ATOMIC_RELAXED, __HIP_MEMORY_SCOPE_AGENT);
+            unsigned spins = 0;
+            while ((int)(ff72_ld_sc1(ctr) - target) < 0) {
+                __builtin_amdgcn_s_sleep(1);
+                ++spins;
+                if (spins > (1u << 20) || ((spins & 1023u) == 0 && (ff72_ld_sc1(err) & 2u))) {
+                    atomicOr(err, 2u);
+                    break;
+                }
+            }
+        }
+        stamp(2);
+        __builtin_amdgcn_s_barrier();
+    }
+    __device__ __forceinline__ void landed() { stamp(3); }
+};
+
+__global__ __launch_bounds__(640) void ff72_kernel(const Ff72Args a) {
+    __shared__ __attribute__((aligned(16))) unsigned char smem[Ws72<float>::SMEM_BYTES];
+    __shared__ __attribute__((aligned(16))) float ln_sm[128];
+    constexpr int kSlots = 32, kGroup = 16;
+    const int tid = threadIdx.x;
+    const int g = (int)(ff72_xcc_id() & (a.fault ? 6u : 7u)), li = blockIdx.x >> 3;
+    const unsigned epoch = (unsigned)((a.step ? *a.step : 0) + a.epoch_add);
+    if (tid == 0) {
+        const unsigned claim = epoch + 1u;
+        if (atomicExch(a.seen + g * kSlots + li, claim) == claim) atomicOr(a.err, 1u);
+    }
+    const int s = g >> 1, r = 2 * (g & 1) + li / kGroup, c = li % kGroup;
+    Ff72Hook hook;
+    hook.ctr = a.counters + 16 * g + 8 * (li / kGroup);
+    hook.target = (epoch + 1u) * (unsigned)kGroup;
+    hook.err = a.err;
+    hook.prof = a.prof ? a.prof + (size_t)blockIdx.x * 16 : nullptr;
+    if (r * Ws72<float>::BM >= a.g1.M) {
+        if (tid == 0) __hip_atomic_fetch_add(hook.ctr, 1u, __ATOMIC_RELAXED, __HIP_MEMORY_SCOPE_AGENT);
+        return;
+    }
+    hook.stamp(0);
+    Ws72Plain plain;
+    Ws72<bf16>::tile<0, false>(a.g1, r, kGroup * s + c, 0, 0, smem, ln_sm, plain);
+    const int nk1 = (a.g1.kloop ? a.g1.kloop : a.g1.ldw) / Ws72<float>::BK;
+    Ws72<float>::tile<16, true>(a.g2, r, c, s, nk1 % Ws72<float>::STAGES, smem, ln_sm, hook);
+    if (a.prof) {
+        asm volatile("s_waitcnt vmcnt(0)" ::: "memory");
+        hook.stamp(4);
+    }
 }
 
 template <typename OutT> static int launch_ws72(const GemmArgs& a, hipStream_t s) {
@@ -1405,6 +1505,34 @@
     return launch_typed<float, float>(a, s, route);
 }
 
+static bool ff72_plan(const Ff72Args& a, Ff72Args& p) {
+    p = a;
+    const GemmArgs &u1 = a.g1, &u2 = a.g2;
+    if (!a.counters || !a.seen || !a.err) return false;
+    if (u1.in_dtype != DIMX_BF16 || u1.out_dtype != DIMX_BF16 || u2.in_dtype != DIMX_BF16 || u2.out_dtype != DIMX_F32) return false;
+    if (u1.M != u2.M || u1.M <= 128 || u1.M > 256) return false;
+    if (u1.K != 1152 || u1.N != 4608 || u2.K != 4608 || u2.N != 1152 || u1.out_slabs || !u2.out_slabs || u1.residual) return false;
+    int r1 = 0, r2 = 0;
+    if (gemm_route(u1, &r1) != DIMX_OK || gemm_route(u2, &r2) != DIMX_OK || r1 != 72 || r2 != 72) return false;
+    TypedPlan t1, t2;
+    if (plan_typed(u1, p.g1, 2, 2, t1) != DIMX_OK || plan_typed(u2, p.g2, 2, 4, t2) != DIMX_OK) return false;
+    if (p.g1.splitk != 1 || p.g2.splitk != 4) return false;
+    return u1.seg[0].ptr == u2.A && u1.seg[0].st == (long)u2.lda;
+}
+
+bool ff72_supported(const Ff72Args& a, int cu_count) {
+    Ff72Args p;
+    return cu_count == 256 && ff72_plan(a, p);
+}
+
+int launch_ff72(const Ff72Args& a, hipStream_t s) {
+    Ff72Args p;
+    DIMX_REQUIRE(ff72_plan(a, p), DIMX_ERR_ARG, "ff72: not the two 64 x 72 launches of a 1152 / 4608 feed-forward at 129..256 rows");
+    hipLaunchKernelGGL(ff72_kernel, dim3(256), dim3(640), 0, s, p);
+    DIMX_HIP(hipGetLastError());
+    return DIMX_OK;
+}
+
 int launch_gemm(const GemmArgs& a, hipStream_t s) { return gemm_dispatch(a, s, nullptr); }
 
 int gemm_route(const GemmArgs& a, int* route) {
diff --git a/dyadic-interaction-modeling_amd/csrc/generate.hip b/dyadic-interaction-modeling_amd/csrc/generate.hip
--- a/dyadic-interaction-modeling_amd/csrc/generate.hip
+++ b/dyadic-interaction-modeling_amd/csrc/generate.hip
@@ -28,9 +28,7 @@
     return S > 1 && h->multi_tr && h->at == DIMX_BF16 && h->decg.dim_head == 64;
 }
 
-static int slab_gemm_rows(dimx_handle h, int B, hipStream_t st, const void* A, int lda, const Linear& L, float* out, long stride,
-                          int* nsl) {
-    GemmArgs g;
+static void slab_gemm_args(dimx_handle h, int B, const void* A, int lda, const Linear& L, float* out, long stride, GemmArgs& g, int* nsl) {
     gemm_lin(h, A, lda, L, B, g);
     g.x3_decode = 1;
     g.out_dtype = DIMX_F32;
@@ -41,6 +39,11 @@
     gemm_set_plain_out(g, out, L.N);
     *nsl = gemm_plan_splits(g);
     g.force_splitk = *nsl;
+}
+static int slab_gemm_rows(dimx_handle h, int B, hipStream_t st, const void* A, int lda, const Linear& L, float* out, long stride,
+                          int* nsl) {
+    GemmArgs g;
+    slab_gemm_args(h, B, A, lda, L, out, stride, g, nsl);
     return launch_gemm(g, st);
 }
 
@@ -453,12 +456,11 @@
     return DIMX_OK;
 }
 
-static int feed_forward(const StepCtx& c, int l, int* pending) {
+static void ff1_args(const StepCtx& c, int l, GemmArgs& g) {
     dimx_handle h = c.h;
     const GenScratch& s = c.s;
     const bool defer = c.r->defer;
     const int F = c.DD * h->decg.ff_mult;
-    GemmArgs g;
     gemm_lin(h, s.y, c.DD, defer ? h->dec.ff[l].f1_ln : h->dec.ff[l].f1, c.B, g);
     g.x3_decode = 1;
     if (defer) {
@@ -470,8 +472,31 @@
     g.out_dtype = h->at;
     g.act = ACT_GELU_ERF;
     gemm_set_plain_out(g, s.f, F);
+}
+
+static void ff_fused_args(const StepCtx& c, int l, Ff72Args& fa, int* nsl) {
+    dimx_handle h = c.h;
+    const GenScratch& s = c.s;
+    memset(&fa, 0, sizeof(fa));
+    ff1_args(c, l, fa.g1);
+    slab_gemm_args(h, c.B, s.f, c.DD * h->decg.ff_mult, h->dec.ff[l].f2, s.xr, s.st_xr, fa.g2, nsl);
+    fa.counters = s.chain_ctr + (size_t)(4 * h->decg.depth + 1 + l) * kChainSiteWords;
+    fa.seen = fa.counters + 8 * 16; fa.step = s.step + 9; fa.err = h->chain_err_dev; fa.fault = c.r->fault_inject ? 1 : 0;
+    fa.prof = h->layer_prof_dev ? h->layer_prof_dev + (size_t)(4 + l) * 256 * 16 : nullptr;
+}
+
+static int feed_forward(const StepCtx& c, int l, int* pending) {
+    dimx_handle h = c.h;
+    const GenScratch& s = c.s;
+    if (c.r->ff_fused) {
+        Ff72Args fa;
+        ff_fused_args(c, l, fa, pending);
+        return launch_ff72(fa, c.st);
+    }
+    GemmArgs g;
+    ff1_args(c, l, g);
     DIMX_TRY(launch_gemm(g, c.st));
-    return slab_gemm(c, s.f, F, h->dec.ff[l].f2, s.xr, s.st_xr, pending);
+    return slab_gemm(c, s.f, c.DD * h->decg.ff_mult, h->dec.ff[l].f2, s.xr, s.st_xr, pending);
 }
 
 static int logits(const StepCtx& c, int pending, int* nlg) {
@@ -602,6 +627,16 @@
     }
     r.sample_head = h->use_sample_head && r.kv0 && r.layer_kernel[0] && r.logits_chain && h->filter_kind == DIMX_FILTER_TOP_K && !q.beam &&
                     !r.guided && q.pr.step0 == 0 && q.pr.Pmax <= 1 && G == 1 && q.S == 1 && dg.num_tokens == 512 && dg.dim % 4 == 0;
+    if (h->use_ff_fused && r.layer_kernel[0] && 5 * dg.depth + 1 <= kChainSites && dg.depth <= 4) {
+        const StepCtx c = step_ctx(h, gc, r, 0, rows, 0, q.st);
+        r.ff_fused = true;
+        for (int l = 0; l < dg.depth; ++l) {
+            Ff72Args fa;
+            int ns = 0;
+            ff_fused_args(c, l, fa, &ns);
+            r.ff_fused = r.ff_fused && r.layer_kernel[l] && ff72_supported(fa, h->cu_count);
+        }
+    }
     return DIMX_OK;
 }
 
@@ -613,7 +648,7 @@
     k.G = r.G; k.S = r.S;
     k.chain = r.chain; k.defer = r.defer; k.logits_chain = r.logits_chain; k.multi_tr = r.multi_tr; k.fault_inject = r.fault_inject;
     for (int l = 0; l < 8; ++l) k.layer_kernel |= r.layer_kernel[l] ? 1u << l : 0u;
-    k.qkv0 = r.qkv0; k.kv0 = r.kv0; k.sample_head = r.sample_head;
+    k.qkv0 = r.qkv0; k.kv0 = r.kv0; k.sample_head = r.sample_head; k.ff_fused = r.ff_fused;
     k.prompt_len = q.pr.len; k.ld_prompt = q.pr.ld; k.Pmax = q.pr.Pmax;
     k.filter_kind = h->filter_kind;
     k.beam = q.beam ? *q.beam : BeamCall{};
@@ -858,6 +893,7 @@
     if (route.qkv0) DIMX_TRY(qkv0_table_build(h, s, R, st, pr.step0));
     if (route.kv0) ++h->kv0_generations;
     if (route.sample_head) ++h->sample_head_generations;
+    if (route.ff_fused) ++h->ff_fused_generations;
     if (pr.step0 > 0 && !keep_prefill) {
         if (q.logits_out)
             DIMX_HIP(hipMemset2DAsync(q.logits_out, (size_t)n * h->decg.num_tokens * 4, 0, (size_t)pr.step0 * h->decg.num_tokens * 4, R, st));
@@ -975,6 +1011,30 @@
                 }
             if (!n) continue;
             fprintf(stderr, "  %-24s %7.2f / %7.2f  (+%.2f)\n", names[i], sum / n, mx, sum / n - prev);
+            prev = sum / n;
+        }
+    }
+    static const char* ff_names[5] = {"start", "f stored", "group barrier", "first f panel landed", "slabs stored"};
+    for (int l = 0; l < h->decg.depth && l < 4; ++l) {
+        const unsigned long long* p = hp.data() + (size_t)(4 + l) * 256 * 16;
+        unsigned long long t0 = ~0ull;
+        for (int b = 0; b < 256; ++b)
+            if (p[b * 16] && p[b * 16] < t0) t0 = p[b * 16];
+        if (t0 == ~0ull) continue;
+        fprintf(stderr, "dimx feed-forward launch stamps, layer %d (us after the first block's start; mean / max over blocks)\n", l);
+        double prev = 0;
+        for (int i = 0; i < 5; ++i) {
+            double sum = 0, mx = 0;
+            int n = 0;
+            for (int b = 0; b < 256; ++b)
+                if (p[b * 16 + i]) {
+                    const double v = (double)(p[b * 16 + i] - t0) / 100.0;
+                    sum += v;
+                    mx = v > mx ? v : mx;
+                    ++n;
+                }
+            if (!n) continue;
+            fprintf(stderr, "  %-24s %7.2f / %7.2f  (+%.2f)\n", ff_names[i], sum / n, mx, sum / n - prev);
             prev = sum / n;
         }
     }
@@ -1206,6 +1266,7 @@
 int dimx_qkv0_table_builds(dimx_handle h) { return h ? h->qkv0_builds : 0; }
 int dimx_kv0_table_generations(dimx_handle h) { return h ? h->kv0_generations : 0; }
 int dimx_sample_head_generations(dimx_handle h) { return h ? h->sample_head_generations : 0; }
+int dimx_ff_fused_generations(dimx_handle h) { return h ? h->ff_fused_generations : 0; }
 
 int dimx_debug_chain_fault(dimx_handle h, int n_calls) {
     DIMX_REQUIRE(h && n_calls >= 0, DIMX_ERR_ARG, "debug_chain_fault: bad argument");
diff --git a/dyadic-interaction-modeling_amd/csrc/model.hip b/dyadic-interaction-modeling_amd/csrc/model.hip
--- a/dyadic-interaction-modeling_amd/csrc/model.hip
+++ b/dyadic-interaction-modeling_amd/csrc/model.hip
@@ -869,6 +869,7 @@
     c->use_qkv0_table = getenv("DIMX_NO_QKV0_TABLE") ? 0 : 1;
     c->use_kv0_table = getenv("DIMX_NO_KV0_TABLE") ? 0 : 1;
     c->use_sample_head = getenv("DIMX_NO_SAMPLE_HEAD") ? 0 : 1;
+    c->use_ff_fused = getenv("DIMX_NO_FF_FUSED") ? 0 : 1;
     if (getenv("DIMX_LAYER_PROF")) {
         void* p = nullptr;
         if (hipMalloc(&p, (size_t)8 * 256 * 16 * 8) == hipSuccess) {
diff --git a/dyadic-interaction-modeling_amd/csrc/model.hpp b/dyadic-interaction-modeling_amd/csrc/model.hpp
--- a/dyadic-interaction-modeling_amd/csrc/model.hpp
+++ b/dyadic-interaction-modeling_amd/csrc/model.hpp
@@ -122,6 +122,7 @@
     const float* qkv0 = nullptr;
     const void* kv0 = nullptr;
     bool sample_head = false;
+    bool ff_fused = false;
     const BeamCall* beam = nullptr;
     bool fault_inject = false;
     int G = 1, S = 1;
@@ -136,7 +137,7 @@
     bool chain, defer, logits_chain, multi_tr, fault_inject;
     unsigned layer_kernel;
     const void *qkv0, *kv0;
-    bool sample_head;
+    bool sample_head, ff_fused;
     const void* prompt_len;
     int ld_prompt, Pmax;
     int filter_kind;
@@ -151,7 +152,7 @@
         return ws == o.ws && B == o.B && T == o.T && top_k == o.top_k && noise == o.noise && start == o.start && mask == o.mask &&
                tokens == o.tokens && logits_out == o.logits_out && G == o.G && S == o.S && chain == o.chain && defer == o.defer &&
                logits_chain == o.logits_chain && multi_tr == o.multi_tr && fault_inject == o.fault_inject &&
-               layer_kernel == o.layer_kernel && qkv0 == o.qkv0 && kv0 == o.kv0 && sample_head == o.sample_head && prompt_len == o.prompt_len &&
+               layer_kernel == o.layer_kernel && qkv0 == o.qkv0 && kv0 == o.kv0 && sample_head == o.sample_head && ff_fused == o.ff_fused && prompt_len == o.prompt_len &&
                ld_prompt == o.ld_prompt && Pmax == o.Pmax && filter_kind == o.filter_kind && beam == o.beam && xwin_on == o.xwin_on &&
                xwin_lookahead == o.xwin_lookahead && guided == o.guided && branch_out == o.branch_out && kv8 == o.kv8 && kv8_samples == o.kv8_samples && self_kv8 == o.self_kv8;
     }
@@ -225,6 +226,8 @@
     int kv0_generations = 0;
     int use_sample_head = 1;
     int sample_head_generations = 0;
+    int use_ff_fused = 1;
+    int ff_fused_generations = 0;
     int shard_row_off = 0, shard_rows_total = 0;
     int filter_kind = 0;
     float filter_a = 0.f, filter_b = 0.f;
diff --git a/dyadic-interaction-modeling_amd/csrc/ops.hip b/dyadic-interaction-modeling_amd/csrc/ops.hip
--- a/dyadic-interaction-modeling_amd/csrc/ops.hip
+++ b/dyadic-interaction-modeling_amd/csrc/ops.hip
@@ -678,6 +678,45 @@
     g.ln_C = K;
     gemm_set_plain_out(g, C, N);
     return launch_gemm(g, (hipStream_t)stream);
+}
+
+int dimx_op_ff_fused(const void* y, const float* stats, const void* w1s, const float* colsum1, const float* bias1, const void* w2,
+                     const float* bias2, void* f, float* slabs, long slab_stride, int M, int call_index, void* scratch, void* prof,
+                     int fault, void* stream) {
+    DIMX_REQUIRE(y && stats && w1s && colsum1 && w2 && f && slabs && scratch, DIMX_ERR_ARG, "op_ff_fused: null argument");
+    constexpr int C = 1152, F = 4608;
+    DIMX_REQUIRE(slab_stride >= (long)M * C, DIMX_ERR_ARG, "op_ff_fused: slab stride %ld below M * 1152", slab_stride);
+    Ff72Args a;
+    memset(&a, 0, sizeof(a));
+    GemmArgs& g1 = a.g1;
+    gemm_args_init(g1);
+    g1.in_dtype = DIMX_BF16; g1.out_dtype = DIMX_BF16;
+    g1.A = y; g1.lda = C; g1.W = w1s; g1.ldw = C;
+    g1.M = M; g1.N = F; g1.K = C;
+    g1.bias = bias1; g1.act = ACT_GELU_ERF;
+    g1.ln_stats = stats; g1.ln_colsum = colsum1; g1.ln_C = C;
+    unsigned* u = (unsigned*)scratch;
+    g1.ln_err = u + 768;
+    gemm_set_plain_out(g1, f, F);
+    GemmArgs& g2 = a.g2;
+    gemm_args_init(g2);
+    g2.in_dtype = DIMX_BF16; g2.out_dtype = DIMX_F32;
+    g2.A = f; g2.lda = F; g2.W = w2; g2.ldw = F;
+    g2.M = M; g2.N = C; g2.K = F;
+    g2.bias = bias2;
+    g2.allow_splitk = 1; g2.out_slabs = 1; g2.slab_stride = slab_stride;
+    gemm_set_plain_out(g2, slabs, C);
+    g2.force_splitk = 4;
+    a.counters = u; a.seen = u + 8 * 16; a.err = u + 768;
+    a.step = nullptr; a.epoch_add = call_index;
+    a.fault = fault ? 1 : 0;
+    a.prof = (unsigned long long*)prof;
+    DIMX_REQUIRE(ff72_supported(a, 256), DIMX_ERR_ARG, "op_ff_fused: M = %d needs 129..256 rows and 16-byte aligned operands", M);
+    int cu = 0, dev = 0;
+    DIMX_HIP(hipGetDevice(&dev));
+    DIMX_HIP(hipDeviceGetAttribute(&cu, hipDeviceAttributeMultiprocessorCount, dev));
+    DIMX_REQUIRE(cu == 256, DIMX_ERR_ARG, "op_ff_fused: the launch needs a 256-CU device (this one has %d)", cu);
+    return launch_ff72(a, (hipStream_t)stream);
 }
 
 static int op_layer_chain(const float* qkv, int nslab, long slab_stride, void* sk, void* sv, int T, const void* ck, const void* cv,
diff --git a/dyadic-interaction-modeling_amd/engine.py b/dyadic-interaction-modeling_amd/engine.py
--- a/dyadic-interaction-modeling_amd/engine.py
+++ b/dyadic-interaction-modeling_amd/engine.py
@@ -501,6 +501,9 @@
     def sample_head_generations(self):
         return int(self.lib.dimx_sample_head_generations(self.h))
 
+    def ff_fused_generations(self):
+        return int(self.lib.dimx_ff_fused_generations(self.h))
+
     def debug_chain_fault(self, n_calls=1):
         L.check(self.lib.dimx_debug_chain_fault(self.h, int(n_calls)), "dimx_debug_chain_fault")
 
@@ -1067,6 +1070,25 @@
     L.check(lib.dimx_op_gemm_ln(L.BF16 if out_bf16 else L.F32, L.ptr(a), L.ptr(ws), L.ptr(out), M, N, K, L.ptr(bias), act,
                                 L.ptr(stats), L.ptr(colsum), L.stream_ptr(a.device)), "dimx_op_gemm_ln")
     return out
+
+
+def op_ff_fused(y, stats, w1s, colsum1, w2, bias1=None, bias2=None, call_index=0, scratch=None, prof=None, fault=False, f=None,
+                slabs=None):
+    lib = L.load()
+    dev = y.device
+    M = y.shape[0]
+    assert y.dtype == torch.bfloat16 and y.shape[1] == 1152 and w1s.shape == (4608, 1152) and w2.shape == (1152, 4608)
+    assert w1s.dtype == torch.bfloat16 and w2.dtype == torch.bfloat16 and y.is_contiguous() and w1s.is_contiguous() and w2.is_contiguous()
+    f = torch.full((M, 4608), float("nan"), dtype=torch.bfloat16, device=dev) if f is None else f
+    slabs = torch.full((4, M, 1152), float("nan"), dtype=torch.float32, device=dev) if slabs is None else slabs
+    assert f.shape == (M, 4608) and f.is_contiguous() and slabs.shape == (4, M, 1152) and slabs.is_contiguous()
+    assert prof is None or prof.numel() >= 256 * 16
+    scratch = torch.zeros(1024, dtype=torch.int32, device=dev) if scratch is None else scratch
+    L.check(lib.dimx_op_ff_fused(L.ptr(y), L.ptr(stats), L.ptr(w1s), L.ptr(colsum1), L.ptr(bias1), L.ptr(w2), L.ptr(bias2), L.ptr(f),
+                                 L.ptr(slabs), slabs.stride(0), M, int(call_index), L.ptr(scratch), L.ptr(prof), 1 if fault else 0,
+                                 L.stream_ptr(dev)), "dimx_op_ff_fused")
+    torch.cuda.synchronize(dev)
+    return f, slabs, int(scratch[768].item())
 
 
 def op_decode_attn(q, kcache, vcache, n_keys, scale, kmask=None, nsplit=0):
diff --git a/dyadic-interaction-modeling_amd/lib.py b/dyadic-interaction-modeling_amd/lib.py
--- a/dyadic-interaction-modeling_amd/lib.py
+++ b/dyadic-interaction-modeling_amd/lib.py
@@ -161,6 +161,9 @@
     "dimx_qkv0_table_builds": (c_int, [c_void_p]),
     "dimx_kv0_table_generations": (c_int, [c_void_p]),
     "dimx_sample_head_generations": (c_int, [c_void_p]),
+    "dimx_ff_fused_generations": (c_int, [c_void_p]),
+    "dimx_op_ff_fused": (c_int, [c_void_p, c_void_p, c_void_p, c_void_p, c_void_p, c_void_p, c_void_p, c_void_p, c_void_p, ctypes.c_long,
+                                 c_int, c_int, c_void_p, c_void_p, c_int, c_void_p]),
     "dimx_lstm_faults": (c_int, [c_void_p]),
     "dimx_mesh_head": (c_int, [c_void_p, c_void_p, c_void_p, c_int, c_int, c_void_p, c_int, c_void_p, c_size_t, c_void_p]),
     "dimx_op_lstm_layer": (c_int, [c_int, c_void_p, c_int, c_int, c_int, c_int, POINTER(c_void_p), POINTER(c_void_p),
diff --git a/include/dimx.h b/include/dimx.h
--- a/include/dimx.h
+++ b/include/dimx.h
@@ -153,6 +153,7 @@
 int dimx_qkv0_table_builds(dimx_handle h);
 int dimx_kv0_table_generations(dimx_handle h);
 int dimx_sample_head_generations(dimx_handle h);
+int dimx_ff_fused_generations(dimx_handle h);
 int dimx_debug_chain_fault(dimx_handle h, int n_calls);
 
 int dimx_mesh_head(dimx_handle h, const float* motion, const float* templ, int B, int L, float* mesh_out, int flags, void* ws,
@@ -301,6 +302,9 @@
                      const float* colsum2, int N2, float* out2, int B, int C, void* scratch, void* stream);
 int dimx_op_gemm_ln(int out_dtype, const void* A, const void* Ws, void* C, int M, int N, int K, const float* bias, int act,
                     const float* stats, const float* colsum, void* stream);
+int dimx_op_ff_fused(const void* y, const float* stats, const void* w1s, const float* colsum1, const float* bias1, const void* w2,
+                     const float* bias2, void* f, float* slabs, long slab_stride, int M, int call_index, void* scratch, void* prof,
+                     int fault, void* stream);
 int dimx_op_layer_chain(const float* qkv, int nslab, long slab_stride, void* sk, void* sv, int T, const void* ck, const void* cv,
                         int Tp, int n_keys, const uint8_t* kmask, const void* w_so, const void* w_cq, const float* colsum_cq,
                         const void* w_co, float* x, void* y, void* o, float* qc, float* stats, int B, const int32_t* step,
```

Result: no change. 1740 clips/s (-0.4%).
